# kristi700/ViT-SSL

Measured on AMD Instinct MI355X. Metric: images_per_sec, higher is better.
Workload: dtype bf16; 1 GPU; ViT-B/16 SimMIM 224x224 mask 0.6 dropout 0.1 AdamW, batch 256/GPU; global_batch=256, parallelism=dp1

## Files before the change

__graft_entry__.py:

```python
import os
import subprocess
import sys
from concurrent.futures import ThreadPoolExecutor

ROOT = os.path.dirname(os.path.abspath(__file__))
PKG = os.path.join(ROOT, "vit-ssl_amd")
CSRC = os.path.join(PKG, "csrc")
OUT_DIR = os.path.join(PKG, "vitssl_hip")
LIB = os.path.join(OUT_DIR, "libvitssl_hip.so")
SOURCES = ["error.cpp", "device_state.hip", "gemm_nt.hip", "gemm_tn.hip", "layernorm.hip", "attention.hip", "attention_hd.hip", "elementwise.hip", "patch.hip", "dino.hip", "augment.hip", "transforms.hip", "metrics.hip", "classify.hip", "mixup.hip", "fp8.hip", "optim.hip", "droppath.hip", "layerscale.hip", "lamb.hip", "mae.hip"]
HIPCC = os.environ.get("HIPCC", "/opt/rocm/bin/hipcc")
PER_FILE_FLAGS = {"augment.hip": ["-ffp-contract=off"], "transforms.hip": ["-ffp-contract=off"]}
FLAGS = ["--offload-arch=gfx950", "-O3", "-fPIC", "-std=c++17", "-Wno-unused-result"] + os.environ.get("VITSSL_HIPCC_FLAGS", "").split()


def _needs_rebuild(target, deps):
    if not os.path.exists(target):
        return True
    t = os.path.getmtime(target)
    return any(os.path.getmtime(d) > t for d in deps if os.path.exists(d))


def build(force: bool = False, verbose: bool = False) -> None:
    srcs = [os.path.join(CSRC, s) for s in SOURCES if os.path.exists(os.path.join(CSRC, s))]
    hdrs = [os.path.join(CSRC, "common.h"), os.path.join(CSRC, "attention_tiles.h"), os.path.join(CSRC, "attention_bwd.h"),
            os.path.join(CSRC, "resample_taps.h"), os.path.join(CSRC, "nt_epilogue.h"),
            os.path.join(ROOT, "include", "vitssl_hip.h"), os.path.join(ROOT, "include", "vitssl_transforms.h"),
            os.path.join(ROOT, "include", "vitssl_metrics.h"), os.path.join(ROOT, "include", "vitssl_classify.h"),
            os.path.join(ROOT, "include", "vitssl_attention_hd.h"), os.path.join(ROOT, "include", "vitssl_patch.h"),
            os.path.join(ROOT, "include", "vitssl_optim.h"), os.path.join(ROOT, "include", "vitssl_mixup.h"),
            os.path.join(ROOT, "include", "vitssl_droppath.h"), os.path.join(ROOT, "include", "vitssl_layerscale.h"),
            os.path.join(ROOT, "include", "vitssl_lamb.h"), os.path.join(ROOT, "include", "vitssl_bce.h"),
            os.path.join(ROOT, "include_ext", "vitssl_mae.h")]
    objdir = os.path.join(CSRC, "build")
    os.makedirs(objdir, exist_ok=True)

    def compile_one(src):
        obj = os.path.join(objdir, os.path.basename(src) + ".o")
        if force or _needs_rebuild(obj, [src] + hdrs + [os.path.abspath(__file__)]):
            cmd = [HIPCC] + FLAGS + PER_FILE_FLAGS.get(os.path.basename(src), []) + ["-x", "hip", "-c", src, "-o", obj]
            r = subprocess.run(cmd, capture_output=True, text=True)
            if r.returncode != 0:
                raise RuntimeError(f"hipcc failed for {src}:\n{r.stderr[-4000:]}")
            if verbose and r.stderr.strip():
                print(r.stderr, file=sys.stderr)
        return obj

    with ThreadPoolExecutor(max_workers=4) as ex:
        objs = list(ex.map(compile_one, srcs))
    if force or _needs_rebuild(LIB, objs):
        cmd = [HIPCC, "--offload-arch=gfx950", "-shared", "-fPIC", "-o", LIB] + objs
        r = subprocess.run(cmd, capture_output=True, text=True)
        if r.returncode != 0:
            raise RuntimeError(f"link failed:\n{r.stderr[-4000:]}")
    if PKG not in sys.path:
        sys.path.insert(0, PKG)
    import vitssl_hip
    vitssl_hip.lib()


def smoke() -> None:
    for p in (ROOT, PKG):
        if p not in sys.path:
            sys.path.insert(0, p)
    import torch
    from vitssl_hip import smoke_check
    smoke_check.run(torch.device("cuda:0"))
    print("smoke OK")


if __name__ == "__main__":
    build(force="--force" in sys.argv, verbose=True)
    print("built", LIB)
```

vit-ssl_amd/csrc/gemm_nt.hip:

```cpp
#include "nt_epilogue.h"

namespace {

template <int BK_, int WM_, int WN_, int MI_ = 8>
struct NtCfg {
  static constexpr int BK = BK_, WM = WM_, WN = WN_;
  static constexpr int MI = MI_;
  static constexpr int WROWS = 16 * MI_;
  static constexpr int BM = WROWS * WM_, BN = 64 * WN_;
  static constexpr int WAVES = WM_ * WN_, THREADS = 64 * WM_ * WN_;
  static constexpr int ROWB = BK_ * 2;
  static constexpr int A_BYTES = BM * ROWB, B_BYTES = BN * ROWB;
  static constexpr int BUF_BYTES = A_BYTES + B_BYTES;
  static constexpr int LDS_BYTES = 2 * BUF_BYTES;
  static constexpr int MIN_WAVES_PER_SIMD = 2;
  static constexpr int WG_PER_CU = (WAVES == 8) ? 1 : 2;
};
using NtBig = NtCfg<64, 2, 4>;
using NtSmall = NtCfg<32, 2, 2>;
using NtBig224 = NtCfg<64, 2, 4, 7>;
using NtBig192 = NtCfg<64, 2, 4, 6>;

template <int BK_>
__device__ __forceinline__ int nt_swz(int r) {
  return BK_ == 64 ? ((r >> 1) & 7) : 3 * ((r >> 3) & 1);
}

template <int BK_, int ROWS, int WAVES>
__device__ __forceinline__ void stage_tile(__amdgpu_buffer_rsrc_t rsrc, char* lds_tile, long long row0, int k0,
                                           int K, int wave, int lane) {
  constexpr int ROWB = BK_ * 2;
  constexpr int RPI = 1024 / ROWB;
  constexpr int LPR = ROWB / 16;
  constexpr int SLOTS = ROWS / RPI;
  constexpr int PER = (SLOTS + WAVES - 1) / WAVES;
#pragma unroll
  for (int j = 0; j < PER; ++j) {
    const int i = wave * PER + j;
    if (SLOTS % WAVES != 0 && i >= SLOTS) break;
    const int r = i * RPI + lane / LPR;
    const int c = lane % LPR;
    const int sc = c ^ nt_swz<BK_>(r);
    const unsigned voff = (unsigned)(((row0 + r) * (long long)K + k0) * 2 + sc * 16);
    dma16_to_lds(rsrc, lds_tile + i * 1024, voff);
  }
}

template <int N>
__device__ __forceinline__ void wait_vmcnt_round_down() {
  if constexpr (N >= 16) asm volatile("s_waitcnt vmcnt(16)" ::: "memory");
  else if constexpr (N >= 8) asm volatile("s_waitcnt vmcnt(8)" ::: "memory");
  else asm volatile("s_waitcnt vmcnt(0)" ::: "memory");
}

template <int BM, int BN>
__device__ __forceinline__ bool nt_tile_of(const NtParams& p, const int ntiles, const int G, const int bid, int r, long long& m0, int& n0) {
  const int base = r * G;
  const int cnt = min(G, ntiles - base);
  if (bid >= cnt) return false;
  const int wgid = base + xcd_remap(bid, cnt);
  const int full = p.tiles_m * p.group_n;
  const int cg = wgid / full;
  const int rem = wgid - cg * full;
  const int gw = min(p.group_n, p.tiles_n - cg * p.group_n);
  const int tile_m = rem / gw;
  m0 = (long long)tile_m * BM;
  n0 = (cg * p.group_n + (rem - tile_m * gw)) * BN;
  return true;
}

template <int EPI, typename CFG>
__global__ __launch_bounds__(CFG::THREADS, CFG::MIN_WAVES_PER_SIMD) void gemm_nt_kernel(NtParams p) {
  extern __shared__ __attribute__((aligned(16))) char smem[];
  constexpr int BM = CFG::BM, BN = CFG::BN, BK = CFG::BK;

  const int lane = threadIdx.x & 63;
  const int wave = __builtin_amdgcn_readfirstlane(threadIdx.x >> 6);
  const int wm = wave / CFG::WN, wn = wave % CFG::WN;

  const int ntiles = p.tiles_m * p.tiles_n;
  const int G = gridDim.x;
  const int bid = blockIdx.x;
  auto tile_of = [&](int r, long long& m0, int& n0) { return nt_tile_of<BM, BN>(p, ntiles, G, bid, r, m0, n0); };

  const unsigned long long a_bytes = (unsigned long long)p.M * p.K * 2ull;
  const unsigned long long b_bytes = (unsigned long long)p.N * p.K * 2ull;
  __amdgpu_buffer_rsrc_t rsA = __builtin_amdgcn_make_buffer_rsrc((void*)p.A, 0, (int)a_bytes, 0x00020000);
  __amdgpu_buffer_rsrc_t rsB = __builtin_amdgcn_make_buffer_rsrc((void*)p.B, 0, (int)b_bytes, 0x00020000);

  const int kb = p.k_chunk ? (int)blockIdx.y * p.k_chunk : 0;
  const int nk = (p.k_chunk ? min(p.K - kb, p.k_chunk) : p.K) / BK;
  const int swz = nt_swz<BK>(lane & 15);
  const int frag_row = lane & 15;
  const int kq = lane >> 4;

  constexpr int MI = CFG::MI;
  f32x4 acc[4][MI];

  auto compute_half = [&](const char* bufA, const char* bufB, auto kk_c) {
    constexpr int kk = decltype(kk_c)::value;
    const int coff = ((kk * 4 + kq) ^ swz) << 4;
    bf16x8 fb[4], fa[MI];
#pragma unroll
    for (int j = 0; j < 4; ++j)
      fb[j] = *(const bf16x8*)(bufB + (wn * 64 + j * 16 + frag_row) * CFG::ROWB + coff);
#pragma unroll
    for (int i = 0; i < MI; ++i)
      fa[i] = *(const bf16x8*)(bufA + (wm * CFG::WROWS + i * 16 + frag_row) * CFG::ROWB + coff);
    if constexpr (BK == 64) __builtin_amdgcn_s_setprio(1);
#pragma unroll
    for (int j = 0; j < 4; ++j)
#pragma unroll
      for (int i = 0; i < MI; ++i)
        acc[j][i] = __builtin_amdgcn_mfma_f32_16x16x32_bf16(fb[j], fa[i], acc[j][i], 0, 0, 0);
    if constexpr (BK == 64) __builtin_amdgcn_s_setprio(0);
  };

  long long m0 = 0, m0n = 0;
  int n0 = 0, n0n = 0;
  if (!tile_of(0, m0, n0)) return;
  int par = 0;
  stage_tile<BK, BM, CFG::WAVES>(rsA, smem, m0, kb, p.K, wave, lane);
  stage_tile<BK, BN, CFG::WAVES>(rsB, smem + CFG::A_BYTES, n0, kb, p.K, wave, lane);
  asm volatile("s_waitcnt vmcnt(0)" ::: "memory");

  for (int round = 0;; ++round) {
    const bool has_next = tile_of(round + 1, m0n, n0n);
    __syncthreads();
#pragma unroll
    for (int j = 0; j < 4; ++j)
#pragma unroll
      for (int i = 0; i < MI; ++i) acc[j][i] = f32x4{0.f, 0.f, 0.f, 0.f};

    for (int t = 0; t < nk; ++t) {
      char* bufA = smem + par * CFG::BUF_BYTES;
      char* nA = smem + (par ^ 1) * CFG::BUF_BYTES;
      const bool more = t + 1 < nk;
      const bool fetch = more || has_next;
      const long long sm = more ? m0 : m0n;
      const int sn = more ? n0 : n0n;
      const int sk = kb + (more ? (t + 1) * BK : 0);
      if constexpr (BK == 64) {
        if (fetch) stage_tile<BK, BM, CFG::WAVES>(rsA, nA, sm, sk, p.K, wave, lane);
        compute_half(bufA, bufA + CFG::A_BYTES, IC<0>{});
        if (fetch) stage_tile<BK, BN, CFG::WAVES>(rsB, nA + CFG::A_BYTES, sn, sk, p.K, wave, lane);
        compute_half(bufA, bufA + CFG::A_BYTES, IC<1>{});
      } else {
        if (fetch) {
          stage_tile<BK, BM, CFG::WAVES>(rsA, nA, sm, sk, p.K, wave, lane);
          stage_tile<BK, BN, CFG::WAVES>(rsB, nA + CFG::A_BYTES, sn, sk, p.K, wave, lane);
        }
        compute_half(bufA, bufA + CFG::A_BYTES, IC<0>{});
      }
      par ^= 1;
      if (more) {
        asm volatile("s_waitcnt vmcnt(0)" ::: "memory");
        __syncthreads();
      }
    }

    nt_epilogue<EPI, CFG>(p, acc, m0, n0, wm, wn, lane);

    if (!has_next) break;
    constexpr int TAIL = nt_epi_tail_stores<EPI>();
    static_assert(TAIL <= nt_epi_row_ops<EPI, false>(true) * MI, "more than this epilogue is certain to store");
    wait_vmcnt_round_down<TAIL>();
    m0 = m0n;
    n0 = n0n;
  }
}

__device__ __forceinline__ i32x8 join_frags(const bf16x8& lo, const bf16x8& hi) {
  const u32x4 a = __builtin_bit_cast(u32x4, lo), b = __builtin_bit_cast(u32x4, hi);
  return i32x8{(int)a[0], (int)a[1], (int)a[2], (int)a[3], (int)b[0], (int)b[1], (int)b[2], (int)b[3]};
}

template <int EPI, typename CFG, bool F8 = false>
__global__ __launch_bounds__(CFG::THREADS, 2) void gemm_nt_pp_kernel(NtParams p) {
  extern __shared__ __attribute__((aligned(16))) char smem[];
  static_assert(CFG::BK == 64 && CFG::WM == 2 && CFG::WN == 4, "ping-pong loop is written for 8 waves, BK = 64");
  constexpr int BM = CFG::BM, BN = CFG::BN, MI = CFG::MI;
  constexpr int MH1 = MI - 4;
  constexpr int BUF = CFG::BUF_BYTES;
  constexpr int DUMMY = 2 * BUF;
  constexpr unsigned OOBV = 0x80000000u;
  constexpr bool USE_GLUT = EPI == VITSSL_EPI_GELU;
  constexpr int GLUT_BASE = 2 * BUF + 1024;
  constexpr int GLUT_IMM = USE_GLUT ? GLUT_BASE - (int)GLUT_LO8 : -1;
  static_assert(!USE_GLUT || (GLUT_IMM >= 0 && GLUT_IMM < 65536), "the table's offset must fit the ds_read immediate");

  const int lane = threadIdx.x & 63;
  const int wave = __builtin_amdgcn_readfirstlane(threadIdx.x >> 6);
  const int wm = wave >> 2, wn = wave & 3;
  const int ntiles = p.tiles_m * p.tiles_n;
  const int G = gridDim.x;
  const int bid = blockIdx.x;

  auto tile_of = [&](int r, long long& m0, int& n0) { return nt_tile_of<BM, BN>(p, ntiles, G, bid, r, m0, n0); };

  long long m0 = 0;
  int n0 = 0;
  if (!tile_of(0, m0, n0)) return;

  if (p.stagger > 0) {
    const int rem = ntiles % G;
    if (rem != 0 && bid >= rem && wave == 0) {
      const unsigned long long delay = (unsigned long long)p.stagger * (unsigned)(bid - rem) / (unsigned)(G - rem);
      const unsigned long long t0 = __builtin_amdgcn_s_memrealtime();
      while (__builtin_amdgcn_s_memrealtime() - t0 < delay) __builtin_amdgcn_s_sleep(8);
    }
  }

  constexpr unsigned ESZ = F8 ? 1u : 2u;
  const unsigned long long a_bytes = (unsigned long long)p.M * p.K * ESZ;
  const unsigned long long b_bytes = (unsigned long long)p.N * p.K * ESZ;
  const int nk = F8 ? p.K / 128 : p.K / 64;
  const unsigned rowb = (unsigned)p.K * ESZ;

  unsigned voffA[2][2], voffB[2][2];
  int ldsA[2][2], ldsB[2][2];
#pragma unroll
  for (int h = 0; h < 2; ++h)
#pragma unroll
    for (int e = 0; e < 2; ++e) {
      const int s = 2 * wave + e;
      {
        const int per_g = h == 0 ? 8 : 2 * MH1;
        const bool ok = s < 2 * per_g;
        const int g = s / per_g, q = s - g * per_g;
        const int r = g * CFG::WROWS + 64 * h + 8 * q;
        const int rl = r + (lane >> 3);
        const int sc = (lane & 7) ^ ((rl >> 1) & 7);
        voffA[h][e] = ok ? (unsigned)rl * rowb + (unsigned)sc * 16u : OOBV;
        ldsA[h][e] = ok ? r * 128 : DUMMY;
      }
      {
        const int c = s >> 2, q = s & 3;
        const int r = 64 * c + 32 * h + 8 * q;
        const int rl = r + (lane >> 3);
        const int sc = (lane & 7) ^ ((rl >> 1) & 7);
        voffB[h][e] = (unsigned)rl * rowb + (unsigned)sc * 16u;
        ldsB[h][e] = CFG::A_BYTES + r * 128;
      }
    }

  struct Cur {
    int round, kt;
    unsigned a, b;
  };
  auto cur_at = [&](int round) {
    Cur c;
    c.round = round;
    c.kt = 0;
    long long mm;
    int nn;
    if (tile_of(round, mm, nn)) {
      c.a = (unsigned)((unsigned long long)mm * rowb);
      c.b = (unsigned)((unsigned long long)nn * rowb);
    } else {
      c.a = c.b = OOBV;
    }
    return c;
  };
  auto cur_next = [&](const Cur& c) {
    if (c.a == OOBV) return c;
    if (c.kt + 1 < nk) {
      Cur n = c;
      n.kt += 1;
      n.a += 128u;
      n.b += 128u;
      return n;
    }
    return cur_at(c.round + 1);
  };
  auto stage_a = [&](const Cur& c, int bufsel, auto h_c) {
    constexpr int h = decltype(h_c)::value;
    __amdgpu_buffer_rsrc_t rs =
        __builtin_amdgcn_make_buffer_rsrc((void*)((const char*)p.A + c.a), 0, c.a == OOBV ? 0 : (int)(a_bytes - c.a), 0x00020000);
#pragma unroll
    for (int e = 0; e < 2; ++e) {
      const bool live = ldsA[h][e] != DUMMY;
      dma16_to_lds(rs, smem + (live ? bufsel * BUF : 0) + ldsA[h][e], voffA[h][e]);
    }
  };
  auto stage_b = [&](const Cur& c, int bufsel, auto h_c) {
    constexpr int h = decltype(h_c)::value;
    __amdgpu_buffer_rsrc_t rs =
        __builtin_amdgcn_make_buffer_rsrc((void*)((const char*)p.B + c.b), 0, c.b == OOBV ? 0 : (int)(b_bytes - c.b), 0x00020000);
#pragma unroll
    for (int e = 0; e < 2; ++e)
      dma16_to_lds(rs, smem + bufsel * BUF + ldsB[h][e], voffB[h][e]);
  };

  const int frag_row = lane & 15;
  const int kq = lane >> 4;
  const int swz = nt_swz<64>(frag_row);
  const int offA0 = (wm * CFG::WROWS + frag_row) * 128 + (((0 + kq) ^ swz) << 4);
  const int offA1 = (wm * CFG::WROWS + frag_row) * 128 + (((4 + kq) ^ swz) << 4);
  const int offB0 = CFG::A_BYTES + (wn * 64 + frag_row) * 128 + (((0 + kq) ^ swz) << 4);
  const int offB1 = CFG::A_BYTES + (wn * 64 + frag_row) * 128 + (((4 + kq) ^ swz) << 4);

  f32x4 acc[4][MI];
  bf16x8 fa[2][4];
  bf16x8 fb[2][2][2];

  auto read_a = [&](const char* buf, auto mh_c) {
    constexpr int mh = decltype(mh_c)::value;
    constexpr int cnt = mh == 0 ? 4 : MH1;
#pragma unroll
    for (int ii = 0; ii < cnt; ++ii) {
      fa[0][ii] = *(const bf16x8*)(buf + offA0 + (4 * mh + ii) * 2048);
      fa[1][ii] = *(const bf16x8*)(buf + offA1 + (4 * mh + ii) * 2048);
    }
  };
  auto read_b = [&](const char* buf, auto nh_c) {
    constexpr int nh = decltype(nh_c)::value;
#pragma unroll
    for (int jj = 0; jj < 2; ++jj) {
      fb[nh][0][jj] = *(const bf16x8*)(buf + offB0 + (2 * nh + jj) * 2048);
      fb[nh][1][jj] = *(const bf16x8*)(buf + offB1 + (2 * nh + jj) * 2048);
    }
  };
  auto mma_quad = [&](auto mh_c, auto nh_c) {
    constexpr int mh = decltype(mh_c)::value, nh = decltype(nh_c)::value;
    constexpr int cnt = mh == 0 ? 4 : MH1;
    if constexpr (F8) {
#pragma unroll
      for (int jj = 0; jj < 2; ++jj) {
        const i32x8 bq = join_frags(fb[nh][0][jj], fb[nh][1][jj]);
#pragma unroll
        for (int ii = 0; ii < cnt; ++ii)
          acc[2 * nh + jj][4 * mh + ii] = __builtin_amdgcn_mfma_scale_f32_16x16x128_f8f6f4(
              bq, join_frags(fa[0][ii], fa[1][ii]), acc[2 * nh + jj][4 * mh + ii], 0, 0, 0, 0, 0, 0);
      }
    } else {
#pragma unroll
      for (int kk = 0; kk < 2; ++kk)
#pragma unroll
        for (int jj = 0; jj < 2; ++jj)
#pragma unroll
          for (int ii = 0; ii < cnt; ++ii)
            acc[2 * nh + jj][4 * mh + ii] =
                __builtin_amdgcn_mfma_f32_16x16x32_bf16(fb[nh][kk][jj], fa[kk][ii], acc[2 * nh + jj][4 * mh + ii], 0, 0, 0);
    }
  };
  auto ktile = [&](int buf, const Cur& c1, const Cur& c2, bool last_of_round, auto nw_c) {
    constexpr int NW = decltype(nw_c)::value;
    const char* cur = smem + buf * BUF;
    read_b(cur, IC<0>{});
    read_a(cur, IC<0>{});
    stage_b(c1, buf ^ 1, IC<1>{});
    wait_vmcnt<NW>();
    raw_barrier();
    mma_quad(IC<0>{}, IC<0>{});
    raw_barrier();
    read_b(cur, IC<1>{});
    stage_a(c1, buf ^ 1, IC<1>{});
    wait_vmcnt<NW>();
    raw_barrier();
    mma_quad(IC<0>{}, IC<1>{});
    raw_barrier();
    read_a(cur, IC<1>{});
    stage_b(c2, buf, IC<0>{});
    raw_barrier();
    mma_quad(IC<1>{}, IC<1>{});
    raw_barrier();
    stage_a(c2, buf, IC<0>{});
    wait_vmcnt<NW>();
    raw_barrier();
    mma_quad(IC<1>{}, IC<0>{});
    if (!(last_of_round && wm == 1)) raw_barrier();
  };

  Cur c0 = cur_at(0);
  Cur c1 = cur_next(c0);
  stage_b(c0, 0, IC<0>{});
  stage_a(c0, 0, IC<0>{});
  stage_b(c0, 0, IC<1>{});
  stage_a(c0, 0, IC<1>{});
  stage_b(c1, 1, IC<0>{});
  stage_a(c1, 1, IC<0>{});
  Cur c2 = cur_next(c1);
  if constexpr (USE_GLUT) {
    if ((unsigned)(unsigned long long)LDS_PTR(smem) != 0u) __builtin_trap();
    const float hs = p.drop_on ? 0.5f * p.dk.scale : 0.5f;
    const float cs = p.drop_on ? 0.3989422804014327f * p.dk.scale : 0.3989422804014327f;
    unsigned* tab = (unsigned*)(smem + GLUT_BASE);
    for (int e = threadIdx.x; e < GLUT_ENTRIES; e += CFG::THREADS) {
      const unsigned h = (unsigned)((e >> 1) + (GLUT_E_LO << 7)) | ((unsigned)(e & 1) << 15);
      float y, dy;
      gelu_both_scaled(bf2f((bf16_t)h), hs, cs, y, dy);
      if constexpr (F8) {
        const float qs = p.qscale ? *p.qscale : 1.0f;
        tab[e] = (unsigned)f2bf(dy) | ((pack_fp8x4(y * qs, 0.f, 0.f, 0.f) & 0xffu) << 16);
      } else {
        tab[e] = (unsigned)f2bf(y) | ((unsigned)f2bf(dy) << 16);
      }
    }
    asm volatile("s_waitcnt lgkmcnt(0)" ::: "memory");
  }
  wait_vmcnt<8>();
  raw_barrier();

  constexpr int S = nt_epi_vmem_ops<EPI, MI, F8>();
  constexpr int NW = 8;
  constexpr int NW_POST = (NW + S) > 63 ? 63 : (NW + S);
  int buf = 0;
#ifdef VITSSL_NT_STAMPS
  auto stamp = [&](int round, int which) {
    if (!(p.stamps && (wave & 3) == 0 && lane == 0 && round < 16)) return;
    p.stamps[(((size_t)bid * 2 + wm) * 16 + round) * 4 + which] = __builtin_amdgcn_s_memrealtime();
    p.stamps[(size_t)256 * 2 * 16 * 4 + (((size_t)bid * 2 + wm) * 16 + round) * 4 + which] = __builtin_amdgcn_s_memtime();
  };
#else
  auto stamp = [&](int, int) {};
#endif
  for (int round = 0;; ++round) {
    stamp(round, 0);
    if (wm == 1) raw_barrier();
#pragma unroll
    for (int j = 0; j < 4; ++j)
#pragma unroll
      for (int i = 0; i < MI; ++i) acc[j][i] = f32x4{0.f, 0.f, 0.f, 0.f};
    for (int t = 0; t < nk; ++t) {
      const bool last = t + 1 == nk;
      if (t == 0 && round > 0) ktile(buf, c1, c2, last, IC<NW_POST>{});
      else ktile(buf, c1, c2, last, IC<NW>{});
      c1 = c2;
      c2 = cur_next(c2);
      buf ^= 1;
    }
    stamp(round, 1);
    if constexpr (F8) {
      if (p.alpha || p.alpha2) {
        const float al = (p.alpha ? *p.alpha : 1.0f) * (p.alpha2 ? *p.alpha2 : 1.0f);
#pragma unroll
        for (int j = 0; j < 4; ++j)
#pragma unroll
          for (int i = 0; i < MI; ++i) acc[j][i] *= al;
      }
    }
    nt_epilogue<EPI, CFG, F8, GLUT_IMM, true>(p, acc, m0, n0, wm, wn, lane, smem, smem + (buf ^ 1) * BUF + ldsB[1][0]);
    stamp(round, 2);
#ifdef VITSSL_NT_STAMPS
    if (p.stamps) {
      asm volatile("s_waitcnt vmcnt(0)" ::: "memory");
      stamp(round, 3);
    }
#endif
    if (!tile_of(round + 1, m0, n0)) break;
  }
  asm volatile("s_waitcnt vmcnt(0)" ::: "memory");
}

int cu_count() { return vitssl_persistent_cus(); }

template <int EPI, typename CFG, bool F8 = false>
int launch_pp(NtParams p, hipStream_t s) {
  constexpr int LDS = 2 * CFG::BUF_BYTES + 1024 + (EPI == VITSSL_EPI_GELU ? GLUT_BYTES : 0);
  static VsOnce attr_done{false};
  if (int rc = ensure_lds(gemm_nt_pp_kernel<EPI, CFG, F8>, LDS, attr_done, "gemm_nt")) return rc;
  const long long ntiles = (long long)p.tiles_m * p.tiles_n;
  const long long slots = cu_count();
  const long long grid = ntiles < slots ? ntiles : slots;
  constexpr float STAGGER_SCALE = 1.0f;
  static VsEnvMilli stagger_knob;
  const float stagger_scale = stagger_knob.get("VITSSL_NT_STAGGER", STAGGER_SCALE);
  constexpr int STAGGER_EPIS = (1 << VITSSL_EPI_RESID) | (1 << VITSSL_EPI_DGELU);
  static VsEnvInt stagger_mask_knob;
  const int stagger_mask = stagger_mask_knob.get("VITSSL_NT_STAGGER_EPIS", STAGGER_EPIS);
  const float tile_us = (float)(p.K * p.esz / 128) * 1.45f * (float)CFG::MI / 8.f + nt_epi(EPI).epi_us;
  p.stagger = ((stagger_mask >> nt_epi(EPI).stagger_bit) & 1) ? (int)(stagger_scale * tile_us * 100.f) : 0;
  vitssl_note_nt_grid((int)grid);
  hipLaunchKernelGGL((gemm_nt_pp_kernel<EPI, CFG, F8>), dim3((unsigned)grid), dim3(CFG::THREADS), LDS, s, p);
  VS_CHECK_LAUNCH("gemm_nt_pp");
  return VITSSL_OK;
}

template <int EPI, typename CFG>
int launch_cfg_parts(NtParams p, hipStream_t s) {
  if constexpr (CFG::LDS_BYTES > 48 * 1024) {
    static VsOnce attr_done{false};
    if (int rc = ensure_lds(gemm_nt_kernel<EPI, CFG>, CFG::LDS_BYTES, attr_done, "gemm_nt")) return rc;
  }
  p.tiles_m = (int)ceil_div64(p.M, CFG::BM);
  p.tiles_n = (int)ceil_div64(p.N, CFG::BN);
  const int want = (int)((2 * 1024 * 1024) / ((long long)CFG::BN * p.K * p.esz));
  static VsEnvInt group_env;
  const int group_knob = group_env.get("VITSSL_NT_GROUPN", 0);
  if (group_knob > 0) p.group_n = group_knob < p.tiles_n ? group_knob : p.tiles_n;
  else if (p.tiles_n <= 4) p.group_n = p.tiles_n;
  else if (want <= 2) p.group_n = 2;
  else if (p.tiles_n % 6 == 0 && want >= 6) p.group_n = 6;
  else if (p.tiles_n % 4 == 0) p.group_n = 4;
  else if (p.tiles_n % 3 == 0) p.group_n = 3;
  else p.group_n = want < 4 ? want : 4;
  if (p.esz == 1) {
    if ((p.N & 7) != 0) {
      vitssl_set_error("gemm_fp8_nt: N=%d must be a multiple of 8", p.N);
      return VITSSL_ERR_ARG;
    }
    if constexpr (CFG::WAVES == 8 && CFG::BK == 64 && nt_epi(EPI).fp8) {
      return launch_pp<EPI, CFG, true>(p, s);
    } else {
      vitssl_set_error("gemm_fp8_nt: epilogue %d / tile configuration not built for fp8 operands", EPI);
      return VITSSL_ERR_ARG;
    }
  }
  if constexpr (CFG::WAVES == 8 && CFG::BK == 64 && EPI != EPI_F32_SPLITK) {
    if (p.k_chunk == 0 && (p.N & 7) == 0) return launch_pp<EPI, CFG>(p, s);
  }
  static VsEnvInt persist_env;
  const int knob = persist_env.get("VITSSL_NT_PERSIST", -1);
  const bool persist = knob >= 0 ? knob != 0 : p.K <= 512;
  const long long ntiles = (long long)p.tiles_m * p.tiles_n;
  long long grid = ntiles;
  if (persist) {
    const long long slots = (long long)cu_count() * CFG::WG_PER_CU;
    if (grid > slots) grid = slots;
  }
  const unsigned slices = p.k_chunk ? (unsigned)ceil_div64(p.K, p.k_chunk) : 1u;
  hipLaunchKernelGGL((gemm_nt_kernel<EPI, CFG>), dim3((unsigned)grid, slices), dim3(CFG::THREADS), CFG::LDS_BYTES, s, p);
  VS_CHECK_LAUNCH("gemm_nt");
  return VITSSL_OK;
}

int nt_tile_override() {
  static VsEnvInt knob;
  return knob.get("VITSSL_NT_TILE", 0);
}

int launch_splitk_f32(NtParams p, hipStream_t s, bool* done) {
  *done = false;
  const long long tiles = ceil_div64(p.M, NtSmall::BM) * ceil_div64(p.N, NtSmall::BN);
  if (tiles >= 64 || p.K < 4096) return VITSSL_OK;
  long long slices = (cu_count() / 2 + tiles - 1) / tiles;
  const long long max_slices = p.K / 512;
  if (slices > max_slices) slices = max_slices;
  if (slices < 2) return VITSSL_OK;
  long long chunk = ceil_div64(ceil_div64(p.K, slices), 64) * 64;
  p.k_chunk = (int)chunk;
  hipError_t e = hipMemsetAsync(p.out0, 0, (size_t)p.M * p.N * sizeof(float), s);
  if (e != hipSuccess) {
    vitssl_set_error("gemm_nt: split-K memset failed: %s", hipGetErrorString(e));
    return VITSSL_ERR_LAUNCH;
  }
  *done = true;
  return launch_cfg_parts<EPI_F32_SPLITK, NtSmall>(p, s);
}


template <int EPI, typename CFG>
int launch_cfg(NtParams p, hipStream_t s) {
  float* colsum = p.colsum;
  if (!colsum) return launch_cfg_parts<EPI, CFG>(p, s);
  const int groups = (int)ceil_div64(p.M, CFG::BM) * (CFG::BM / CFG::WROWS);
  p.colsum = vs_sum_parts(p.workspace, p.workspace_floats, (long long)groups * p.N, p.M, p.N, "gemm_nt column sums");
  if (!p.colsum) return VITSSL_ERR_ARG;
  const int rc = launch_cfg_parts<EPI, CFG>(p, s);
  if (rc != VITSSL_OK) return rc;
  return vs_reduce_parts(colsum, p.colsum, groups, p.N, p.N, s);
}

template <int EPI>
int launch_nt(const NtParams& p, hipStream_t s) {
  if constexpr (EPI == VITSSL_EPI_F32) {
    if (!p.colsum && p.esz == 2) {
      bool done = false;
      const int rc = launch_splitk_f32(p, s, &done);
      if (rc != VITSSL_OK || done) return rc;
    }
  }
  const int mode = p.esz == 1 ? 0 : nt_tile_override();
  if (mode == 1) return launch_cfg<EPI, NtBig>(p, s);
  if (mode == 2) return launch_cfg<EPI, NtSmall>(p, s);
  if (mode == 3) return launch_cfg<EPI, NtBig192>(p, s);
  if (mode == 4) return launch_cfg<EPI, NtBig224>(p, s);
  const long long big_tiles = ceil_div64(p.M, 256) * ceil_div64(p.N, 256);
  if (big_tiles < 64 && p.esz == 2) return launch_cfg<EPI, NtSmall>(p, s);
  const long long slots = cu_count();
  const long long tn = ceil_div64(p.N, 256);
  const double c256 = (double)ceil_div64(ceil_div64(p.M, 256) * tn, slots);
  const double c224 = 0.90 * (double)ceil_div64(ceil_div64(p.M, 224) * tn, slots);
  const double c192 = 0.78 * (double)ceil_div64(ceil_div64(p.M, 192) * tn, slots);
  double best = c256;
  if (c192 < 0.9 * c256 && c192 <= c224) best = c192;
  else if (c224 < 0.95 * c256) best = c224;
  if (best == c192 && best != c256) return launch_cfg<EPI, NtBig192>(p, s);
  if (best == c224 && best != c256) return launch_cfg<EPI, NtBig224>(p, s);
  return launch_cfg<EPI, NtBig>(p, s);
}

}

#ifdef VITSSL_NT_STAMPS
static unsigned long long* g_nt_stamps = nullptr;
extern "C" void vitssl_debug_nt_stamps(void* buf) { g_nt_stamps = (unsigned long long*)buf; }
#endif

static NtEpiFacts caller_epi(int epi) { return nt_epi(epi >= EPI_F32_SPLITK ? -1 : epi); }

static int check_rowscale(const char* who, const vitssl_rowscale_t* rows, int64_t M) {
  VS_CHECK_ARG(rows->scale && rows->groups > 0 && rows->rows_per_group > 0, "%s: row scales need scale, groups > 0 and rows_per_group > 0", who);
  VS_CHECK_ARG(rows->groups * (int64_t)rows->rows_per_group == M, "%s: groups (%lld) * rows_per_group (%d) must equal M (%lld)", who,
               (long long)rows->groups, rows->rows_per_group, (long long)M);
  return VITSSL_OK;
}

static int gemm_nt_entry(const vitssl_gemm_t* g, int esz, const vitssl_fp8_gemm_t* q, void* stream, const vitssl_rowscale_t* rows = nullptr,
                         const vitssl_colscale_t* cols = nullptr, void* branch = nullptr) {
  const char* who = cols ? "gemm_nt_ls" : rows ? "gemm_nt_rows" : esz == 1 ? "gemm_fp8_nt" : "gemm_nt";
  VS_CHECK_ARG(g && g->A && g->B && (g->out0 || (esz == 1 && caller_epi(g->epilogue).q8_of == 0 && q && q->out_fp8)), "%s: null operand", who);
  VS_CHECK_ARG(g->M > 0 && g->N > 0 && g->K > 0, "%s: empty problem M=%lld N=%d K=%d", who, (long long)g->M, g->N, g->K);
  VS_CHECK_ARG(g->K % (128 / esz) == 0, "%s: K=%d must be a multiple of %d", who, g->K, 128 / esz);
  VS_CHECK_ARG(g->N % 4 == 0, "%s: N=%d must be a multiple of 4", who, g->N);
  VS_CHECK_ARG(g->N <= (1 << 20), "%s: N=%d exceeds 2^20 (epilogue windows use 32-bit byte offsets)", who, g->N);
  VS_CHECK_ARG((unsigned long long)g->M * g->K * (unsigned)esz < (1ull << 31) && (unsigned long long)g->N * g->K * (unsigned)esz < (1ull << 31),
               "%s: operand larger than 2 GiB (M=%lld N=%d K=%d)", who, (long long)g->M, g->N, g->K);
  NtParams p{(const bf16_t*)g->A, (const bf16_t*)g->B, g->M, g->N, g->K, g->bias, g->aux, g->out0, g->out1, g->colsum, g->workspace,
             g->workspace_floats, make_drop_key(g->drop)};
  p.drop_on = p.dk.thr != 0;
  p.embed = g->embed;
  p.esz = esz;
  if (q) {
    p.alpha = q->alpha;
    p.alpha2 = q->alpha2;
    p.out2 = q->out_fp8;
    p.qscale = q->out_scale;
    p.qamax = q->out_amax;
  }
  p.rows_per_group = 1;
#ifdef VITSSL_NT_STAMPS
  p.stamps = g_nt_stamps;
#endif
  hipStream_t s = (hipStream_t)stream;
  VS_CHECK_ARG(!g->colsum || caller_epi(g->epilogue).colsum, "%s: column sums are built for the BF16 / F32 / DGELU epilogues only", who);
  VS_CHECK_ARG(!p.drop_on || (unsigned long long)g->M * (unsigned long long)g->N < (1ull << 34),
               "%s: dropout over %lld x %d elements: the stream's group counter is 32 bits (M * N < 2^34)", who, (long long)g->M, g->N);
  if (rows || cols) {
    VS_CHECK_ARG(g->epilogue == VITSSL_EPI_RESID, "%s: %s scales are built for VITSSL_EPI_RESID only, got epilogue %d", who,
                 cols ? "column" : "row", g->epilogue);
    VS_CHECK_ARG(g->aux, "%s: EPI_RESID needs aux (residual)", who);
    if (cols) {
      VS_CHECK_ARG(cols->gamma, "%s: null gamma", who);
      VS_CHECK_ARG(cols->cols == g->N, "%s: cols (%d) must equal N (%d)", who, cols->cols, g->N);
    }
    if (rows) {
      if (int rc = check_rowscale(who, rows, g->M)) return rc;
      p.rowscale = rows->scale;
      p.rows_per_group = (unsigned)rows->rows_per_group;
    }
    if (!cols) return launch_nt<EPI_RESID_ROWS>(p, s);
    p.colscale = cols->gamma;
    p.out1 = branch;
    return launch_nt<EPI_RESID_LS>(p, s);
  }
  switch (g->epilogue) {
    case VITSSL_EPI_BF16: return launch_nt<VITSSL_EPI_BF16>(p, s);
    case VITSSL_EPI_F32: return launch_nt<VITSSL_EPI_F32>(p, s);
    case VITSSL_EPI_GELU:
      VS_CHECK_ARG(g->out1 || p.out2, "%s: EPI_GELU needs out1 (or, with fp8 operands, out_fp8)", who);
      return launch_nt<VITSSL_EPI_GELU>(p, s);
    case VITSSL_EPI_RESID:
      VS_CHECK_ARG(g->aux, "%s: EPI_RESID needs aux (residual)", who);
      return launch_nt<VITSSL_EPI_RESID>(p, s);
    case VITSSL_EPI_DGELU:
      VS_CHECK_ARG(g->aux, "%s: EPI_DGELU needs aux (pre-activation)", who);
      return launch_nt<VITSSL_EPI_DGELU>(p, s);
    case VITSSL_EPI_EMBED:
      VS_CHECK_ARG(g->embed.pos && g->embed.tokens > 0 && g->embed.out_tokens >= g->embed.tokens + g->embed.tok_offset,
                   "%s: EPI_EMBED needs pos/tokens", who);
      VS_CHECK_ARG(!g->embed.mask || g->embed.mask_token, "%s: EPI_EMBED mask without mask_token", who);
      return launch_nt<VITSSL_EPI_EMBED>(p, s);
    default:
      vitssl_set_error("%s: unknown epilogue %d", who, g->epilogue);
      return VITSSL_ERR_ARG;
  }
}

extern "C" int vitssl_gemm_bf16_nt(const vitssl_gemm_t* g, void* stream) { return gemm_nt_entry(g, 2, nullptr, stream); }

extern "C" int vitssl_gemm_bf16_nt_rows(const vitssl_gemm_t* g, const vitssl_rowscale_t* rows, void* stream) {
  VS_CHECK_ARG(rows, "gemm_nt_rows: null row scales (vitssl_gemm_bf16_nt is the launch without them)");
  return gemm_nt_entry(g, 2, nullptr, stream, rows);
}

extern "C" int vitssl_gemm_bf16_nt_ls(const vitssl_gemm_t* g, const vitssl_colscale_t* cols, const vitssl_rowscale_t* rows,
                                      void* branch_bf16, void* stream) {
  VS_CHECK_ARG(cols, "gemm_nt_ls: null column scales (vitssl_gemm_bf16_nt / vitssl_gemm_bf16_nt_rows are the launches without them)");
  return gemm_nt_entry(g, 2, nullptr, stream, rows, cols, branch_bf16);
}

extern "C" int vitssl_gemm_fp8_nt(const vitssl_gemm_t* g, const vitssl_fp8_gemm_t* q, void* stream) {
  VS_CHECK_ARG(g && caller_epi(g->epilogue).fp8, "gemm_fp8_nt: fp8 operands are built for the BF16 / F32 / GELU / RESID / DGELU epilogues");
  VS_CHECK_ARG(!(q && q->out_fp8) || caller_epi(g->epilogue).q8_of >= 0, "gemm_fp8_nt: out_fp8 belongs to EPI_GELU / EPI_DGELU");
  return gemm_nt_entry(g, 1, q, stream);
}
```

vit-ssl_amd/csrc/nt_epilogue.h:

```cpp
#pragma once
#include "../../include/vitssl_droppath.h"
#include "../../include/vitssl_layerscale.h"
#include "common.h"

namespace {

struct NtParams {
  const bf16_t* A;
  const bf16_t* B;
  long long M;
  int N, K;
  const float* bias;
  const void* aux;
  void* out0;
  void* out1;
  float* colsum;
  float* workspace;
  int64_t workspace_floats;
  DropKey dk;
  int drop_on;
  vitssl_embed_t embed;
  int tiles_m, tiles_n;
  int group_n;
  int k_chunk;
  int stagger;
  int esz;
  const float* alpha;
  void* out2;
  const float* alpha2;
  const float* qscale;
  float* qamax;
  const float* rowscale;
  unsigned rows_per_group;
  const float* colscale;
#ifdef VITSSL_NT_STAMPS
  unsigned long long* stamps;
#endif
};

constexpr int EPI_F32_SPLITK = 100;
constexpr int EPI_RESID_ROWS = 101;
constexpr int EPI_RESID_LS = 102;

enum NtOut1 { OUT1_NONE, OUT1_REQUIRED, OUT1_OPTIONAL };
struct NtEpiFacts {
  int out0_esz;
  bool windowed;
  NtOut1 out1;
  int aux_esz;
  bool colsum, fp8;
  int q8_of;
  bool drops, resid;
  int stagger_bit;
  float epi_us;
};
constexpr NtEpiFacts nt_epi(int epi) {
  switch (epi) {
    case VITSSL_EPI_BF16:  return NtEpiFacts{2, true,  OUT1_NONE,     0, true,  true,  -1, false, false, VITSSL_EPI_BF16,  2.f};
    case VITSSL_EPI_F32:   return NtEpiFacts{4, true,  OUT1_NONE,     0, true,  true,  -1, false, false, VITSSL_EPI_F32,   4.f};
    case VITSSL_EPI_GELU:  return NtEpiFacts{2, true,  OUT1_REQUIRED, 0, false, true,   1, true,  false, VITSSL_EPI_GELU,  7.f};
    case VITSSL_EPI_RESID: return NtEpiFacts{4, true,  OUT1_NONE,     4, false, true,  -1, true,  true,  VITSSL_EPI_RESID, 8.f};
    case VITSSL_EPI_DGELU: return NtEpiFacts{2, true,  OUT1_NONE,     2, true,  true,   0, false, false, VITSSL_EPI_DGELU, 5.f};
    case VITSSL_EPI_EMBED: return NtEpiFacts{4, false, OUT1_NONE,     0, false, false, -1, false, false, VITSSL_EPI_EMBED, 4.f};
    case EPI_F32_SPLITK:   return NtEpiFacts{4, false, OUT1_NONE,     0, false, false, -1, false, false, -1,               4.f};
    case EPI_RESID_ROWS:   return NtEpiFacts{4, true,  OUT1_NONE,     4, false, false, -1, true,  true,  VITSSL_EPI_RESID, 8.f};
    case EPI_RESID_LS:     return NtEpiFacts{4, true,  OUT1_OPTIONAL, 4, false, false, -1, true,  true,  VITSSL_EPI_RESID, 8.f};
    default:               return NtEpiFacts{0, false, OUT1_NONE,     0, false, false, -1, false, false, -1,               0.f};
  }
}

template <int EPI, int MI, bool PREF>
constexpr int nt_row_group() {
  return nt_epi(EPI).resid ? (PREF ? 1 : (MI % 2 == 0 ? 2 : 1)) : EPI == VITSSL_EPI_DGELU ? (PREF ? 2 : (MI % 4 == 0 ? 4 : 2)) : 4;
}

template <int EPI, bool F8>
constexpr int nt_epi_row_ops(bool stores_only) {
  constexpr NtEpiFacts E = nt_epi(EPI);
  if (!E.windowed) return 0;
  const int out0 = (F8 && E.q8_of == 0) ? 1 : E.out0_esz;
  const int out1 = E.out1 != OUT1_REQUIRED ? 0 : (F8 && E.q8_of == 1) ? 1 : 2;
  return (stores_only ? 0 : E.aux_esz) + out0 + out1;
}
template <int EPI, int MI, bool F8>
constexpr int nt_epi_vmem_ops() { return nt_epi_row_ops<EPI, F8>(false) * MI; }
template <int EPI>
constexpr int nt_epi_tail_stores() { return nt_epi_row_ops<EPI, false>(true) * nt_row_group<EPI, 8, false>(); }
template <int EPI, int MI>
constexpr bool nt_counts_are(int bf, int f8, int tail) {
  return nt_epi_vmem_ops<EPI, MI, false>() == bf * MI && (!nt_epi(EPI).fp8 || nt_epi_vmem_ops<EPI, MI, true>() == f8 * MI) &&
         nt_epi_tail_stores<EPI>() == tail;
}
template <int MI>
constexpr bool nt_counts_are_as_written() {
  return nt_counts_are<VITSSL_EPI_BF16, MI>(2, 2, 8) && nt_counts_are<VITSSL_EPI_GELU, MI>(4, 3, 16) && nt_counts_are<VITSSL_EPI_DGELU, MI>(4, 3, 8) &&
         nt_counts_are<VITSSL_EPI_F32, MI>(4, 4, 16) && nt_counts_are<VITSSL_EPI_RESID, MI>(8, 8, 8) && nt_counts_are<EPI_RESID_ROWS, MI>(8, 8, 8) &&
         nt_counts_are<EPI_RESID_LS, MI>(8, 8, 8) && nt_counts_are<VITSSL_EPI_EMBED, MI>(0, 0, 0) && nt_counts_are<EPI_F32_SPLITK, MI>(0, 0, 0);
}
static_assert(nt_counts_are_as_written<6>() && nt_counts_are_as_written<7>() && nt_counts_are_as_written<8>(), "epilogue vmem counts");


constexpr int GLUT_E_LO = 127 - 14;
constexpr int GLUT_BINADES = 18;
constexpr int GLUT_ENTRIES = GLUT_BINADES * 128 * 2;
constexpr int GLUT_BYTES = GLUT_ENTRIES * 4;
constexpr unsigned GLUT_LO8 = (unsigned)GLUT_E_LO << 10;
constexpr unsigned GLUT_HI8 = (unsigned)(GLUT_E_LO + GLUT_BINADES) << 10;

__device__ __forceinline__ unsigned glut_rot2(unsigned w) {
  unsigned t, r;
  asm("v_pk_lshrrev_b16 %0, 15, %1 op_sel_hi:[0,1]" : "=v"(t) : "v"(w));
  asm("v_pk_mad_u16 %0, %1, 2, %2 op_sel_hi:[1,0,1]" : "=v"(r) : "v"(w), "v"(t));
  return r;
}
__device__ __forceinline__ void glut_addr2(unsigned r, unsigned& a0, unsigned& a1) {
  asm("v_lshlrev_b32_sdwa %0, 2, %1 dst_sel:DWORD dst_unused:UNUSED_PAD src0_sel:DWORD src1_sel:WORD_0" : "=v"(a0) : "v"(r));
  asm("v_lshlrev_b32_sdwa %0, 2, %1 dst_sel:DWORD dst_unused:UNUSED_PAD src0_sel:DWORD src1_sel:WORD_1" : "=v"(a1) : "v"(r));
}
__device__ __forceinline__ bool glut_out_of_range(unsigned r01, unsigned r23) {
  const unsigned lo2 = ((unsigned)GLUT_E_LO << 8) * 0x10001u, span = ((unsigned)(GLUT_BINADES << 8) - 1u) * 0x10001u;
  unsigned d01, d23, dm, e;
  asm("v_pk_sub_u16 %0, %1, %2" : "=v"(d01) : "v"(r01), "s"(lo2));
  asm("v_pk_sub_u16 %0, %1, %2" : "=v"(d23) : "v"(r23), "s"(lo2));
  asm("v_pk_max_u16 %0, %1, %2" : "=v"(dm) : "v"(d01), "v"(d23));
  asm("v_pk_sub_u16 %0, %1, %2 clamp" : "=v"(e) : "v"(dm), "s"(span));
  return e != 0;
}
template <int OFF>
__device__ __forceinline__ unsigned glut_read(const char* smem, unsigned a) {
  (void)smem;
  return *(const __attribute__((address_space(3))) unsigned*)(unsigned long long)(a + (unsigned)OFF);
}

struct NtWindow {
  char* xs;
  unsigned tw16, tr16a, tw32, tr32a;
  __device__ __forceinline__ void lines_of_bf16(const u32x2 (&w)[2][2], u32x4& s1, u32x4& s2) const {
#pragma unroll
    for (int j = 0; j < 4; ++j) *(u32x2*)(xs + (tw16 ^ (unsigned)(32 * j))) = w[j >> 1][j & 1];
    s1 = *(const u32x4*)(xs + tr16a);
    s2 = *(const u32x4*)(xs + ((tr16a + 1024u) ^ 64u));
  }
  __device__ __forceinline__ void put_lines_bf16(const u32x4& s1, const u32x4& s2) const {
    *(u32x4*)(xs + tr16a) = s1;
    *(u32x4*)(xs + ((tr16a + 1024u) ^ 64u)) = s2;
  }
  __device__ __forceinline__ u32x2 bf16_of_lines(int j) const { return *(const u32x2*)(xs + (tw16 ^ (unsigned)(32 * j))); }
  __device__ __forceinline__ void lines_of_f32(const f32x4& v0, const f32x4& v1, u32x4& s1, u32x4& s2) const {
    *(f32x4*)(xs + tw32) = v0;
    *(f32x4*)(xs + (tw32 ^ 64u)) = v1;
    s1 = *(const u32x4*)(xs + tr32a);
    s2 = *(const u32x4*)(xs + tr32a + 1024);
  }
  __device__ __forceinline__ void f32_of_lines(f32x4& v0, f32x4& v1) const {
    *(f32x4*)(xs + tr32a) = v0;
    *(f32x4*)(xs + tr32a + 1024) = v1;
    v0 = *(const f32x4*)(xs + tw32);
    v1 = *(const f32x4*)(xs + (tw32 ^ 64u));
  }
};

__device__ __forceinline__ float amax4(float a, float b, float c, float d) { return fmaxf(fmaxf(fabsf(a), fabsf(b)), fmaxf(fabsf(c), fabsf(d))); }

template <int EPI, typename CFG, bool Q8 = false, int GLUT_OFF = -1, bool TLS = false>
__device__ __forceinline__ void nt_epilogue(const NtParams& p, f32x4 (&acc)[4][CFG::MI], const long long m0, const int n0,
                                            const int wm, const int wn, const int lane_in, const char* lds = nullptr, char* xs = nullptr) {
  constexpr int MI = CFG::MI;
  constexpr NtEpiFacts E = nt_epi(EPI);
  constexpr bool LS = EPI == EPI_RESID_LS;
  int lane = lane_in;
  if (TLS) asm volatile("" : "+v"(lane));
  constexpr bool GLUT = EPI == VITSSL_EPI_GELU && GLUT_OFF >= 0;
  const bool glut_on = GLUT && (!Q8 || (p.out1 == nullptr && p.qamax == nullptr));
  constexpr bool CS = E.colsum, DROPS = E.drops;
  float csum[4][4];
  if (CS && p.colsum) {
#pragma unroll
    for (int j = 0; j < 4; ++j)
#pragma unroll
      for (int r = 0; r < 4; ++r) csum[j][r] = 0.f;
  }
  const int g4 = lane >> 4;
  const bool wide = TLS || (p.N & 7) == 0;
  constexpr unsigned OOB = 0x80000000u;
  const long long rows_left = p.M - m0;
  auto window = [&](const void* base, int elt) {
    const unsigned long long bytes = (unsigned long long)rows_left * (unsigned long long)p.N * (unsigned)elt;
    const unsigned rec = bytes > 0x80000000ull ? 0x80000000u : (unsigned)bytes;
    return __builtin_amdgcn_make_buffer_rsrc((void*)((const char*)base + m0 * p.N * elt), 0, (int)rec, 0x00020000);
  };
  const unsigned row_l = (unsigned)(wm * CFG::WROWS + (lane & 15));
  const unsigned un = (unsigned)p.N;
  const int odd = g4 & 1;

  auto off_bf16_wide = [&](int i, int jp) -> unsigned {
    const int n = n0 + wn * 64 + (2 * jp + odd) * 16 + 4 * (g4 - odd);
    return n < p.N ? ((row_l + 16u * i) * un + (unsigned)n) * 2u : OOB;
  };
  auto off_elem = [&](int i, int n, unsigned elt) -> unsigned { return n < p.N ? ((row_l + 16u * i) * un + (unsigned)n) * elt : OOB; };
  constexpr bool tls = TLS;
  const int tm = lane & 15, trho = lane >> 3, tkap = lane & 7;
  const unsigned tw16 = (unsigned)(tm * 128 + ((g4 ^ (2 * (tm >> 1))) << 3));
  const unsigned tr16a = (unsigned)(trho * 128 + ((tkap ^ (trho >> 1)) << 4));
  const unsigned tw32 = (unsigned)(tm * 128 + ((g4 ^ (tm & 7)) << 4));
  const unsigned tr32a = (unsigned)(trho * 128 + ((tkap ^ trho) << 4));
  const NtWindow win{xs, tw16, tr16a, tw32, tr32a};
  const unsigned trow = (unsigned)(wm * CFG::WROWS + trho);
  const int tn16 = n0 + wn * 64 + 8 * tkap;
  const unsigned tb16 = tn16 < p.N ? (trow * un + (unsigned)tn16) * 2u : OOB;
  auto off_line16 = [&](int i, int half) -> unsigned { return tb16 + (unsigned)(16 * i + 8 * half) * (un * 2u); };
  auto off_line32 = [&](int i, int jp, int half) -> unsigned {
    const int n = n0 + wn * 64 + 32 * jp + 4 * tkap;
    const unsigned b = n < p.N ? (trow * un + (unsigned)n) * 4u : OOB;
    return b + (unsigned)(16 * i + 8 * half) * (un * 4u);
  };
  int nn[2][2];
  bool okn[2][2];
  auto pack_pair = [&](const u32x2& w0, const u32x2& w1) -> u32x4 {
    auto lo = __builtin_amdgcn_permlane16_swap(w0[0], w1[0], false, false);
    auto hi = __builtin_amdgcn_permlane16_swap(w0[1], w1[1], false, false);
    return u32x4{lo[0], hi[0], lo[1], hi[1]};
  };
  auto store_bf16_row = [&](__amdgpu_buffer_rsrc_t rs, int i, const u32x2 (&w)[2][2], auto aux_c) {
    constexpr int AUXV = decltype(aux_c)::value;
    if (tls) {
      u32x4 s1, s2;
      win.lines_of_bf16(w, s1, s2);
      __builtin_amdgcn_raw_buffer_store_b128(s1, rs, off_line16(i, 0), 0, AUXV);
      __builtin_amdgcn_raw_buffer_store_b128(s2, rs, off_line16(i, 1), 0, AUXV);
    } else if (wide) {
      const u32x4 a = pack_pair(w[0][0], w[0][1]), b = pack_pair(w[1][0], w[1][1]);
      __builtin_amdgcn_raw_buffer_store_b128(a, rs, off_bf16_wide(i, 0), 0, AUXV);
      __builtin_amdgcn_raw_buffer_store_b128(b, rs, off_bf16_wide(i, 1), 0, AUXV);
    } else {
#pragma unroll
      for (int jp = 0; jp < 2; ++jp) {
        const int na = n0 + wn * 64 + (2 * jp) * 16 + 4 * g4;
        __builtin_amdgcn_raw_buffer_store_b64(w[jp][0], rs, off_elem(i, na, 2u), 0, AUXV);
        __builtin_amdgcn_raw_buffer_store_b64(w[jp][1], rs, off_elem(i, na + 16, 2u), 0, AUXV);
      }
    }
  };
  constexpr int F32_AUX = E.resid ? 2 : 0;
  auto store_f32_pair = [&](__amdgpu_buffer_rsrc_t rs, int i, int jp, const f32x4& v0, const f32x4& v1, const int (&nnp)[2]) {
    if (tls) {
      u32x4 s1, s2;
      win.lines_of_f32(v0, v1, s1, s2);
      __builtin_amdgcn_raw_buffer_store_b128(s1, rs, off_line32(i, jp, 0), 0, F32_AUX);
      __builtin_amdgcn_raw_buffer_store_b128(s2, rs, off_line32(i, jp, 1), 0, F32_AUX);
    } else {
      __builtin_amdgcn_raw_buffer_store_b128(__builtin_bit_cast(u32x4, v0), rs, off_elem(i, nnp[0], 4u), 0, F32_AUX);
      __builtin_amdgcn_raw_buffer_store_b128(__builtin_bit_cast(u32x4, v1), rs, off_elem(i, nnp[1], 4u), 0, F32_AUX);
    }
  };
  auto store_fp8_row = [&](__amdgpu_buffer_rsrc_t rs, int i, const unsigned (&out_q)[2][2]) {
    if ((p.N & 15) == 0) {
      auto s02 = __builtin_amdgcn_permlane32_swap(out_q[0][0], out_q[1][0], false, false);
      auto s13 = __builtin_amdgcn_permlane32_swap(out_q[0][1], out_q[1][1], false, false);
      auto e = __builtin_amdgcn_permlane16_swap(s02[0], s13[0], false, false);
      auto f = __builtin_amdgcn_permlane16_swap(s02[1], s13[1], false, false);
      if (tls) {
        *(u32x4*)(xs + tm * 64 + ((g4 ^ ((tm >> 1) & 3)) << 4)) = u32x4{e[0], e[1], f[0], f[1]};
        const int rho4 = lane >> 2, kap4 = lane & 3;
        const u32x4 s8 = *(const u32x4*)(xs + rho4 * 64 + ((kap4 ^ ((rho4 >> 1) & 3)) << 4));
        const int n8 = n0 + wn * 64 + 16 * kap4;
        const unsigned o8 = n8 < p.N ? ((unsigned)(wm * CFG::WROWS + 16 * i + rho4) * un + (unsigned)n8) : OOB;
        __builtin_amdgcn_raw_buffer_store_b128(s8, rs, o8, 0, 0);
      } else {
        const int n = n0 + wn * 64 + 16 * g4;
        __builtin_amdgcn_raw_buffer_store_b128(u32x4{e[0], e[1], f[0], f[1]}, rs, off_elem(i, n, 1u), 0, 0);
      }
    } else {
#pragma unroll
      for (int jp = 0; jp < 2; ++jp)
#pragma unroll
        for (int h = 0; h < 2; ++h) __builtin_amdgcn_raw_buffer_store_b32(out_q[jp][h], rs, off_elem(i, nn[jp][h], 1u), 0, 0);
    }
  };

  __amdgpu_buffer_rsrc_t rsOut0, rsOut1, rsOut2, rsAux;
  constexpr bool Q8EPI = Q8 && E.q8_of >= 0;
  const bool q8 = Q8EPI && p.out2 != nullptr;
  if (q8) rsOut2 = window(p.out2, 1);
  const float qs = (Q8EPI && p.qscale) ? *p.qscale : 1.0f;
  float qmax = 0.f;
  if constexpr (E.windowed) rsOut0 = window(p.out0, E.out0_esz);
  if constexpr (E.out1 != OUT1_NONE) {
    if (E.out1 == OUT1_REQUIRED || p.out1) rsOut1 = window(p.out1, 2);
  }
  if constexpr (E.aux_esz != 0) rsAux = window(p.aux, E.aux_esz);

  f32x4 bias4[2][2];
  f32x4 gam4[2][2];
  unsigned a0col[2][2];
  const unsigned a0rowstep = 16u * (unsigned)(p.N >> 2) * DROP_C0;
  unsigned a0row = 0;
  if (DROPS && p.drop_on)
    a0row = drop_a0(p.dk, (unsigned)(m0 + wm * CFG::WROWS + (lane & 15)) * (unsigned)(p.N >> 2));
  const float gelu_hs = (DROPS && p.drop_on) ? 0.5f * p.dk.scale : 0.5f;
  const float gelu_cs = (DROPS && p.drop_on) ? 0.3989422804014327f * p.dk.scale : 0.3989422804014327f;
#pragma unroll
  for (int jp = 0; jp < 2; ++jp)
#pragma unroll
    for (int h = 0; h < 2; ++h) {
      nn[jp][h] = n0 + wn * 64 + (2 * jp + h) * 16 + 4 * g4;
      a0col[jp][h] = (unsigned)(nn[jp][h] >> 2) * DROP_C0;
      okn[jp][h] = nn[jp][h] < p.N;
      bias4[jp][h] = f32x4{0.f, 0.f, 0.f, 0.f};
      if (p.bias && (EPI != EPI_F32_SPLITK || blockIdx.y == 0) && okn[jp][h]) bias4[jp][h] = *(const f32x4*)(p.bias + nn[jp][h]);
      if constexpr (LS) {
        gam4[jp][h] = f32x4{0.f, 0.f, 0.f, 0.f};
        if (okn[jp][h]) gam4[jp][h] = *(const f32x4*)(p.colscale + nn[jp][h]);
      }
    }

  constexpr bool PREF = TLS && E.aux_esz != 0;
  constexpr int RG = nt_row_group<EPI, MI, PREF>();
  constexpr int NB = PREF ? 2 : 1;
  f32x4 res[NB][RG][2][2];
  u32x4 raw[NB][RG][2];
  float rsc[NB][RG];
  auto load_group = [&](const int ig, const int b) {
    const int cnt = MI - ig < RG ? MI - ig : RG;
    if constexpr (EPI == EPI_RESID_ROWS || LS) {
#pragma unroll
      for (int ii = 0; ii < RG; ++ii) {
        if (ii >= cnt) continue;
        if constexpr (LS) rsc[b][ii] = 1.0f;
        if (EPI == EPI_RESID_ROWS || p.rowscale) {
          const long long mr = m0 + wm * CFG::WROWS + (ig + ii) * 16 + (lane & 15);
          rsc[b][ii] = p.rowscale[mr < p.M ? (unsigned)mr / p.rows_per_group : 0u];
        }
      }
    }
    if constexpr (E.resid) {
#pragma unroll
      for (int ii = 0; ii < RG; ++ii)
#pragma unroll
        for (int jp = 0; jp < 2; ++jp) {
          if (ii >= cnt) continue;
          if (tls) {
            res[b][ii][jp][0] = __builtin_bit_cast(f32x4, __builtin_amdgcn_raw_buffer_load_b128(rsAux, off_line32(ig + ii, jp, 0), 0, 0));
            res[b][ii][jp][1] = __builtin_bit_cast(f32x4, __builtin_amdgcn_raw_buffer_load_b128(rsAux, off_line32(ig + ii, jp, 1), 0, 0));
          } else {
#pragma unroll
            for (int h = 0; h < 2; ++h)
              res[b][ii][jp][h] = __builtin_bit_cast(f32x4, __builtin_amdgcn_raw_buffer_load_b128(rsAux, off_elem(ig + ii, nn[jp][h], 4u), 0, 0));
          }
        }
    }
    if constexpr (EPI == VITSSL_EPI_DGELU) {
      if (wide) {
#pragma unroll
        for (int ii = 0; ii < RG; ++ii) {
          if (ii >= cnt) continue;
          if (tls) {
            raw[b][ii][0] = __builtin_amdgcn_raw_buffer_load_b128(rsAux, off_line16(ig + ii, 0), 0, 0);
            raw[b][ii][1] = __builtin_amdgcn_raw_buffer_load_b128(rsAux, off_line16(ig + ii, 1), 0, 0);
          } else {
#pragma unroll
            for (int jp = 0; jp < 2; ++jp) raw[b][ii][jp] = __builtin_amdgcn_raw_buffer_load_b128(rsAux, off_bf16_wide(ig + ii, jp), 0, 0);
          }
        }
      }
    }
  };
  if constexpr (PREF) load_group(0, 0);
#pragma unroll
  for (int ig = 0; ig < MI; ig += RG) {
    const int cnt = MI - ig < RG ? MI - ig : RG;
    const int gb = PREF ? (ig / RG) & 1 : 0;
    if constexpr (!PREF) load_group(ig, 0);
    else if (ig + RG < MI) load_group(ig + RG, gb ^ 1);
    u32x2 gpre[RG][2][2];
    if constexpr (EPI == VITSSL_EPI_DGELU) {
      if (wide) {
#pragma unroll
        for (int ii = 0; ii < RG; ++ii)
#pragma unroll
          for (int jp = 0; jp < 2; ++jp) {
            if (ii >= cnt) continue;
            if (tls) {
              if (jp == 0) {
                win.put_lines_bf16(raw[gb][ii][0], raw[gb][ii][1]);
#pragma unroll
                for (int j = 0; j < 4; ++j) gpre[ii][j >> 1][j & 1] = win.bf16_of_lines(j);
              }
              continue;
            }
            auto sa = __builtin_amdgcn_permlane16_swap(raw[gb][ii][jp][0], raw[gb][ii][jp][2], false, false);
            auto sb = __builtin_amdgcn_permlane16_swap(raw[gb][ii][jp][1], raw[gb][ii][jp][3], false, false);
            gpre[ii][jp][0] = u32x2{sa[0], sb[0]};
            gpre[ii][jp][1] = u32x2{sa[1], sb[1]};
          }
      } else {
#pragma unroll
        for (int ii = 0; ii < RG; ++ii)
#pragma unroll
          for (int jp = 0; jp < 2; ++jp)
#pragma unroll
            for (int h = 0; h < 2; ++h)
              if (ii < cnt) gpre[ii][jp][h] = __builtin_amdgcn_raw_buffer_load_b64(rsAux, off_elem(ig + ii, nn[jp][h], 2u), 0, 0);
      }
    }

#pragma unroll
    for (int ii = 0; ii < RG; ++ii) {
      if (ii >= cnt) continue;
      const int i = ig + ii;
      const long long m = m0 + wm * CFG::WROWS + i * 16 + (lane & 15);
      const bool okm = m < p.M;
      u32x2 out_a[2][2], out_b[2][2];
      unsigned out_q[2][2];
      unsigned gl[16];
      bool gslow[2][2];
      if (GLUT && glut_on) {
#pragma unroll
        for (int jp = 0; jp < 2; ++jp)
#pragma unroll
          for (int h = 0; h < 2; ++h) {
            const f32x4 vv = acc[2 * jp + h][i] + bias4[jp][h];
            const unsigned w0 = pack_bf2(vv[0], vv[1]), w1 = pack_bf2(vv[2], vv[3]);
            const unsigned r01 = glut_rot2(w0), r23 = glut_rot2(w1);
            gslow[jp][h] = __builtin_amdgcn_ballot_w64(glut_out_of_range(r01, r23)) != 0;
            unsigned ad[4];
            glut_addr2(r01, ad[0], ad[1]);
            glut_addr2(r23, ad[2], ad[3]);
            const int q = 8 * jp + 4 * h;
#pragma unroll
            for (int r = 0; r < 4; ++r) gl[q + r] = glut_read<GLUT_OFF>(lds, ad[r]);
          }
      }
#pragma unroll
      for (int jp = 0; jp < 2; ++jp) {
        f32x4 v[2] = {acc[2 * jp][i] + bias4[jp][0], acc[2 * jp + 1][i] + bias4[jp][1]};

        if constexpr (EPI == VITSSL_EPI_BF16) {
          out_a[jp][0] = u32x2{pack_bf2(v[0][0], v[0][1]), pack_bf2(v[0][2], v[0][3])};
          out_a[jp][1] = u32x2{pack_bf2(v[1][0], v[1][1]), pack_bf2(v[1][2], v[1][3])};
        } else if constexpr (EPI == VITSSL_EPI_GELU) {
          unsigned km[2][2] = {{0xffffffffu, 0xffffffffu}, {0xffffffffu, 0xffffffffu}};
          u32x2 dw[2] = {u32x2{0u, 0u}, u32x2{0u, 0u}};
          const bool dropping = p.drop_on;
          if (dropping) {
#pragma unroll
            for (int h = 0; h < 2; ++h) {
              dw[h] = drop_words_a0(p.dk, a0row + (unsigned)i * a0rowstep + a0col[jp][h]);
              km[h][0] = drop_keep_pair(p.dk, dw[h][0]);
              km[h][1] = drop_keep_pair(p.dk, dw[h][1]);
            }
          }
#pragma unroll
          for (int h = 0; h < 2; ++h) {
            if (GLUT && glut_on && !gslow[jp][h]) {
              const int q = 8 * jp + 4 * h;
              const u32x2 lo = u32x2{__builtin_amdgcn_perm(gl[q + 1], gl[q], 0x05040100u) & km[h][0],
                                     __builtin_amdgcn_perm(gl[q + 3], gl[q + 2], 0x05040100u) & km[h][1]};
              if constexpr (!Q8) {
                out_b[jp][h] = lo;
                out_a[jp][h] = u32x2{__builtin_amdgcn_perm(gl[q + 1], gl[q], 0x07060302u) & km[h][0],
                                     __builtin_amdgcn_perm(gl[q + 3], gl[q + 2], 0x07060302u) & km[h][1]};
              } else {
                out_a[jp][h] = lo;
                const unsigned b01 = __builtin_amdgcn_perm(gl[q + 1], gl[q], 0x0c0c0602u), b23 = __builtin_amdgcn_perm(gl[q + 3], gl[q + 2], 0x06020c0cu);
                out_q[jp][h] = (b01 | b23) & __builtin_amdgcn_perm(km[h][1], km[h][0], 0x06040200u);
              }
              continue;
            }
            float y[4], d[4];
#pragma unroll
            for (int r = 0; r < 4; ++r) gelu_both_scaled(round_bf(v[h][r]), gelu_hs, gelu_cs, y[r], d[r]);
            out_b[jp][h] = u32x2{pack_bf2(y[0], y[1]) & km[h][0], pack_bf2(y[2], y[3]) & km[h][1]};
            out_a[jp][h] = u32x2{pack_bf2(d[0], d[1]) & km[h][0], pack_bf2(d[2], d[3]) & km[h][1]};
            if constexpr (Q8) {
              if (dropping) {
                bool keep[4];
                drop_keep4(p.dk, dw[h], keep);
#pragma unroll
                for (int r = 0; r < 4; ++r) y[r] = keep[r] ? y[r] : 0.f;
              }
              out_q[jp][h] = pack_fp8x4(y[0] * qs, y[1] * qs, y[2] * qs, y[3] * qs);
              if (okm && okn[jp][h]) qmax = fmaxf(qmax, amax4(y[0], y[1], y[2], y[3]));
            }
          }
        } else if constexpr (EPI == VITSSL_EPI_DGELU) {
#pragma unroll
          for (int h = 0; h < 2; ++h) {
            const u32x2 gpv = gpre[ii][jp][h];
            v[h][0] *= bf_lo(gpv[0]);
            v[h][1] *= bf_hi(gpv[0]);
            v[h][2] *= bf_lo(gpv[1]);
            v[h][3] *= bf_hi(gpv[1]);
            out_a[jp][h] = u32x2{pack_bf2(v[h][0], v[h][1]), pack_bf2(v[h][2], v[h][3])};
            if constexpr (Q8) {
              out_q[jp][h] = pack_fp8x4(v[h][0] * qs, v[h][1] * qs, v[h][2] * qs, v[h][3] * qs);
              if (okm && okn[jp][h]) qmax = fmaxf(qmax, amax4(v[h][0], v[h][1], v[h][2], v[h][3]));
            }
          }
        } else if constexpr (EPI == EPI_F32_SPLITK) {
#pragma unroll
          for (int h = 0; h < 2; ++h) {
            if (!(okm && okn[jp][h])) continue;
            float* o = (float*)p.out0 + m * p.N + nn[jp][h];
#pragma unroll
            for (int r = 0; r < 4; ++r) unsafeAtomicAdd(o + r, v[h][r]);
          }
        } else if constexpr (EPI == VITSSL_EPI_F32) {
          store_f32_pair(rsOut0, i, jp, v[0], v[1], nn[jp]);
        } else if constexpr (E.resid) {
          if (tls) win.f32_of_lines(res[gb][ii][jp][0], res[gb][ii][jp][1]);
          if constexpr (EPI == EPI_RESID_ROWS || LS) {
            const float rs = rsc[gb][ii];
            const float cs = p.drop_on ? rs * p.dk.scale : rs;
#pragma unroll
            for (int h = 0; h < 2; ++h) {
              bool keep[4] = {true, true, true, true};
              if (p.drop_on) drop_keep4(p.dk, drop_words_a0(p.dk, a0row + (unsigned)i * a0rowstep + a0col[jp][h]), keep);
              float u[4];
#pragma unroll
              for (int r = 0; r < 4; ++r) {
                const float kv = keep[r] ? v[h][r] : 0.f;
                float sc = cs;
                if constexpr (LS) {
                  u[r] = p.drop_on ? kv * p.dk.scale : kv;
                  sc = cs * gam4[jp][h][r];
                }
                const float t = fmaf(kv, sc, res[gb][ii][jp][h][r]);
                v[h][r] = rs == 0.f ? res[gb][ii][jp][h][r] : t;
              }
              if constexpr (LS) out_a[jp][h] = u32x2{pack_bf2(u[0], u[1]), pack_bf2(u[2], u[3])};
            }
          } else {
#pragma unroll
            for (int h = 0; h < 2; ++h) {
              if (p.drop_on) {
                bool keep[4];
                drop_keep4(p.dk, drop_words_a0(p.dk, a0row + (unsigned)i * a0rowstep + a0col[jp][h]), keep);
#pragma unroll
                for (int r = 0; r < 4; ++r) v[h][r] = fmaf(keep[r] ? v[h][r] : 0.f, p.dk.scale, res[gb][ii][jp][h][r]);
              } else {
                v[h] += res[gb][ii][jp][h];
              }
            }
          }
          store_f32_pair(rsOut0, i, jp, v[0], v[1], nn[jp]);
        } else {
#pragma unroll
          for (int h = 0; h < 2; ++h) {
            if (!(okm && okn[jp][h])) continue;
            const long long img = m / p.embed.tokens;
            const int rin = (int)(m - img * p.embed.tokens);
            if (p.embed.mask && p.embed.mask[m]) v[h] = *(const f32x4*)(p.embed.mask_token + nn[jp][h]);
            v[h] += *(const f32x4*)(p.embed.pos + (long long)(p.embed.tok_offset + rin) * p.N + nn[jp][h]);
            const long long orow = img * p.embed.out_tokens + p.embed.tok_offset + rin;
            *(f32x4*)((float*)p.out0 + orow * p.N + nn[jp][h]) = v[h];
          }
        }
        if (CS && p.colsum) {
#pragma unroll
          for (int h = 0; h < 2; ++h)
            if (okm && okn[jp][h]) {
#pragma unroll
              for (int r = 0; r < 4; ++r) csum[2 * jp + h][r] += v[h][r];
            }
        }
      }
      if constexpr (E.windowed && E.out0_esz == 2) {
        if (!(Q8 && E.q8_of == 0) || p.out0) store_bf16_row(rsOut0, i, out_a, IC<EPI == VITSSL_EPI_GELU ? 2 : 0>{});
      }
      if constexpr (E.out1 == OUT1_REQUIRED) {
        if (!(Q8 && E.q8_of == 1) || p.out1) store_bf16_row(rsOut1, i, out_b, IC<0>{});
      }
      if constexpr (E.out1 == OUT1_OPTIONAL) {
        if (p.out1) store_bf16_row(rsOut1, i, out_a, IC<2>{});
      }
      if constexpr (Q8EPI) {
        if (q8) store_fp8_row(rsOut2, i, out_q);
      }
    }
  }

  if (CS && p.colsum) {
    f32x4 red[4];
#pragma unroll
    for (int j = 0; j < 4; ++j) {
#pragma unroll
      for (int r = 0; r < 4; ++r) {
        float s = csum[j][r];
        s += __shfl_xor(s, 1, 64);
        s += __shfl_xor(s, 2, 64);
        s += __shfl_xor(s, 4, 64);
        s += __shfl_xor(s, 8, 64);
        red[j][r] = s;
      }
    }
    if (tls) {
      if ((lane & 15) == 0) {
#pragma unroll
        for (int j = 0; j < 4; ++j) *(f32x4*)(xs + (16 * j + 4 * g4) * 4) = red[j];
      }
      asm volatile("" ::: "memory");
      const float v = *(const volatile float*)(xs + lane * 4);
      const int n = n0 + wn * 64 + lane;
      if (n < p.N) p.colsum[(m0 / CFG::WROWS + wm) * p.N + n] = v;
    } else {
#pragma unroll
      for (int j = 0; j < 4; ++j)
#pragma unroll
        for (int r = 0; r < 4; ++r) {
          const int n = n0 + wn * 64 + j * 16 + 4 * (lane >> 4) + r;
          if ((lane & 15) == 0 && n < p.N) p.colsum[(m0 / CFG::WROWS + wm) * p.N + n] = red[j][r];
        }
    }
  }
  if constexpr (Q8EPI) {
    if (p.qamax) {
      qmax = wave_max(qmax);
      unsigned* slot = (unsigned*)p.qamax;
      if (lane == 0 && __float_as_uint(qmax) > __builtin_nontemporal_load(slot)) atomicMax(slot, __float_as_uint(qmax));
    }
  }
}

}
```

vit-ssl_amd/vitssl_hip/_lib.py:

```python
import ctypes as C
import os
import re

_HERE = os.path.dirname(os.path.abspath(__file__))
LIB_PATH = os.environ.get("VITSSL_LIB") or os.path.join(_HERE, "libvitssl_hip.so")
_INCLUDE = os.path.normpath(os.path.join(_HERE, "..", "..", "include"))
HEADERS = {key: os.path.join(_INCLUDE, f"vitssl_{key}.h")
           for key in ("hip", "transforms", "metrics", "classify", "attention_hd", "patch", "optim", "mixup", "droppath", "layerscale",
                       "lamb", "bce")}
_INCLUDE_EXT = os.path.normpath(os.path.join(_HERE, "..", "..", "include_ext"))
EXT_HEADERS = {"mae": os.path.join(_INCLUDE_EXT, "vitssl_mae.h")}


class VitsslError(RuntimeError):
    pass


class Dropout(C.Structure):
    _fields_ = [("p", C.c_float), ("site", C.c_uint32), ("seed", C.c_uint64)]


class Embed(C.Structure):
    _fields_ = [("mask", C.c_void_p), ("mask_token", C.c_void_p), ("pos", C.c_void_p),
                ("tokens", C.c_int), ("out_tokens", C.c_int), ("tok_offset", C.c_int)]


class TnJob(C.Structure):
    _fields_ = [("A", C.c_void_p), ("B", C.c_void_p), ("C", C.c_void_p), ("N1", C.c_int), ("N2", C.c_int)]


class Fp8TnJob(C.Structure):
    _fields_ = [("A8", C.c_void_p), ("B8", C.c_void_p), ("C", C.c_void_p), ("N1", C.c_int), ("N2", C.c_int),
                ("alpha", C.c_void_p), ("alpha2", C.c_void_p)]


class OptimSegment(C.Structure):
    _fields_ = [("offset", C.c_int64), ("n", C.c_int64), ("lr_scale", C.c_float), ("weight_decay", C.c_float)]


class RowScale(C.Structure):
    _fields_ = [("scale", C.c_void_p), ("groups", C.c_int64), ("rows_per_group", C.c_int)]


class ColScale(C.Structure):
    _fields_ = [("gamma", C.c_void_p), ("cols", C.c_int)]


class Gemm(C.Structure):
    _fields_ = [("A", C.c_void_p), ("B", C.c_void_p), ("M", C.c_int64), ("N", C.c_int), ("K", C.c_int),
                ("epilogue", C.c_int), ("bias", C.c_void_p), ("aux", C.c_void_p), ("out0", C.c_void_p),
                ("out1", C.c_void_p), ("colsum", C.c_void_p), ("drop", Dropout), ("embed", Embed),
                ("workspace", C.c_void_p), ("workspace_floats", C.c_int64)]


class Fp8Gemm(C.Structure):
    _fields_ = [("alpha", C.c_void_p), ("alpha2", C.c_void_p), ("out_fp8", C.c_void_p), ("out_scale", C.c_void_p),
                ("out_amax", C.c_void_p)]


class CastJob(C.Structure):
    _fields_ = [("src", C.c_void_p), ("dst", C.c_void_p), ("dst_t", C.c_void_p), ("R", C.c_int), ("C", C.c_int)]


class CastLdJob(C.Structure):
    _fields_ = CastJob._fields_ + [("ld_dst", C.c_int), ("ld_dst_t", C.c_int)]


class Fp8WeightJob(C.Structure):
    _fields_ = [("src", C.c_void_p), ("dst_fp8", C.c_void_p), ("dst_t_fp8", C.c_void_p), ("R", C.c_int), ("C", C.c_int)]


STRUCTS = {"vitssl_dropout_t": Dropout, "vitssl_embed_t": Embed, "vitssl_gemm_t": Gemm, "vitssl_fp8_gemm_t": Fp8Gemm,
           "vitssl_fp8_weight_job_t": Fp8WeightJob, "vitssl_tn_job_t": TnJob, "vitssl_fp8_tn_job_t": Fp8TnJob,
           "vitssl_cast_job_t": CastJob, "vitssl_cast_ld_job_t": CastLdJob, "vitssl_optim_segment_t": OptimSegment,
           "vitssl_rowscale_t": RowScale, "vitssl_colscale_t": ColScale}

EPI_BF16, EPI_F32, EPI_GELU, EPI_RESID, EPI_DGELU, EPI_EMBED = range(6)

ABI_VERSION = 3
_vp, _i, _i64, _f, _d = C.c_void_p, C.c_int, C.c_int64, C.c_float, C.c_double
_pGemm, _pRows, _pCols = C.POINTER(Gemm), C.POINTER(RowScale), C.POINTER(ColScale)


def _returns(restype, *argtypes):
    return restype, list(argtypes)


_ABI = {
    "hip": {
        "vitssl_last_error": _returns(C.c_char_p),
        "vitssl_version": _returns(_i),
        "vitssl_set_reserved_cus": [_i],
        "vitssl_get_reserved_cus": _returns(_i),
        "vitssl_debug_last_nt_grid": _returns(_i),
        "vitssl_debug_last_attn_fwd_grid": _returns(_i),
        "vitssl_dropout_mask": [_vp, _i64, _i64, Dropout, _vp],
        "vitssl_layernorm_fwd": [_vp, _vp, _vp, _vp, _vp, _vp, _i64, _i, _f, _vp],
        "vitssl_layernorm_bwd": [_vp, _vp, _vp, _vp, _vp, _vp, _vp, _vp, _vp, _vp, _vp, Dropout, _i64, _i, _vp, _i64, _vp],
        "vitssl_grad_mask_cast": [_vp, _vp, _vp, Dropout, _i64, _i, _vp, _i64, _vp],
        "vitssl_gemm_bf16_nt": [_pGemm, _vp],
        "vitssl_gemm_fp8_nt": [_pGemm, C.POINTER(Fp8Gemm), _vp],
        "vitssl_attn_fwd_fp8": [_vp, _vp, _vp, _vp, _vp, _i, _i, _i, _i, _vp],
        "vitssl_gemm_fp8_tn_workspace_floats": _returns(_i64, _i64, _i, _i),
        "vitssl_gemm_fp8_tn": [_vp, _vp, _vp, _i64, _i, _i, _vp, _vp, _vp, _i64, _vp],
        "vitssl_attn_bwd_fp8": [_vp, _vp, _vp, _vp, _vp, _vp, _vp, _vp, _i, _i, _i, _i, _vp],
        "vitssl_quantize_fp8": [_vp, _vp, _i64, _vp],
        "vitssl_quantize_fp8_scaled": [_vp, _vp, _i64, _vp, _vp, _vp],
        "vitssl_layernorm_fwd_fp8": [_vp, _vp, _vp, _vp, _vp, _vp, _vp, _i64, _i, _f, _vp],
        "vitssl_layernorm_bwd_fp8": [_vp, _vp, _vp, _vp, _vp, _vp, _vp, _vp, _vp, _vp, _vp, _vp, _vp, _vp, Dropout, _i64, _i, _vp,
                                     _i64, _vp],
        "vitssl_grad_mask_cast_fp8": [_vp, _vp, _vp, _vp, _vp, _vp, Dropout, _i64, _i, _vp, _i64, _vp],
        "vitssl_fp8_quantize_weights": [_vp, _vp, _i, _i, _vp, _vp, _vp],
        "vitssl_gemm_tn_workspace_floats": _returns(_i64, _i64, _i, _i),
        "vitssl_gemm_bf16_tn": [_vp, _vp, _vp, _i64, _i, _i, _vp, _i64, _vp],
        "vitssl_gemm_tn_batch_workspace_floats": _returns(_i64, C.POINTER(TnJob), _i, _i64),
        "vitssl_gemm_bf16_tn_batch": [C.POINTER(TnJob), _i, _i64, _vp, _i64, _vp],
        "vitssl_gemm_fp8_tn_batch_workspace_floats": _returns(_i64, C.POINTER(Fp8TnJob), _i, _i64),
        "vitssl_gemm_fp8_tn_batch": [C.POINTER(Fp8TnJob), _i, _i64, _vp, _i64, _vp],
        "vitssl_attn_fwd": [_vp, _vp, _vp, _vp, _i, _i, _i, _i, _vp],
        "vitssl_attn_bwd": [_vp, _vp, _vp, _vp, _vp, _vp, _i, _i, _i, _i, _vp],
        "vitssl_patchify_bf16": [_vp, _vp, _i, _i, _i, _i, _i, _vp],
        "vitssl_gather_patches_f32": [_vp, _vp, _vp, _i, _i, _i, _i, _i, _vp],
        "vitssl_gather_rows_bf16": [_vp, _vp, _vp, _i, _i, _vp],
        "vitssl_scatter_rows_f32": [_vp, _vp, _vp, _i64, _i, _vp],
        "vitssl_gather_cls_f32": [_vp, _vp, _i, _i, _i, _vp],
        "vitssl_scatter_cls_f32": [_vp, _vp, _i, _i, _i, _vp],
        "vitssl_embed_bwd_workspace_floats": _returns(_i64, _i, _i, _i, _i),
        "vitssl_embed_bwd": [_vp, _vp, _vp, _vp, _vp, _vp, _vp, _i, _i, _i, _i, _vp, _i64, _vp],
        "vitssl_l1_loss": [_vp, _vp, _vp, _vp, _f, _i64, _vp, _i64, _vp],
        "vitssl_cross_entropy": [_vp, _vp, _vp, _vp, _f, _i, _i, _vp],
        "vitssl_colsum_bf16": [_vp, _vp, _i64, _i, _vp, _i64, _vp],
        "vitssl_sum_workspace_floats": _returns(_i64, _i64, _i),
        "vitssl_cast_bf16": [_vp, _vp, _i64, _vp],
        "vitssl_cast_transpose_bf16": [_vp, _vp, _vp, _i, _i, _vp],
        "vitssl_cast_transpose_batch": [_vp, _vp, _i, _i, _vp],
        "vitssl_adamw": [_vp, _vp, _vp, _vp, _i64, _f, _f, _f, _f, _f, _i, _f, _vp],
        "vitssl_ema": [_vp, _vp, _i64, _f, _vp],
        "vitssl_rownorm_fwd": [_vp, _vp, _vp, _i64, _i, _vp],
        "vitssl_rownorm_bwd": [_vp, _vp, _vp, _vp, _i64, _i, _vp],
        "vitssl_weightnorm_fold": [_vp, _vp, _vp, _vp, _i, _i, _vp],
        "vitssl_weightnorm_bwd": [_vp, _vp, _vp, _vp, _vp, _vp, _i, _i, _vp],
        "vitssl_dino_loss_workspace_floats": _returns(_i64, _i, _i, _i),
        "vitssl_dino_loss": [_vp, _vp, _vp, _vp, _i64, _vp, _vp, _i, _i, _i, _i, _f, _f, _f, _vp],
        "vitssl_colsum_f32": [_vp, _vp, _i64, _i, _vp],
        "vitssl_center_ema": [_vp, _vp, _i, _f, _f, _vp],
        "vitssl_bicubic_resize_fwd": [_vp, _vp, _i, _i, _i, _i, _i, _vp],
        "vitssl_bicubic_resize_bwd": [_vp, _vp, _i, _i, _i, _i, _i, _vp],
        "vitssl_aug_resized_crop_u8": [_vp, _vp, _vp, _vp, _i, _i, _i, _i, _vp],
        "vitssl_aug_color_u8": [_vp, _vp, _vp, _i, _i, _vp],
        "vitssl_aug_blur_to_tensor": [_vp, _vp, _vp, _i, _i, _i, _vp],
    },
    "transforms": {
        "vitssl_tf_resized_crop_to_tensor": [_vp, _vp, _vp, _i, _i, _i, _i, _i, _vp],
        "vitssl_debug_tf_tile_rows": _returns(_i, _i, _i, _i, _i),
    },
    "metrics": {
        "vitssl_recon_metrics_workspace_floats": _returns(_i64, _i64, _i, _i),
        "vitssl_recon_metrics": [_vp, _vp, _vp, _i64, _i, _i, _vp, _i64, _vp],
        "vitssl_dino_stats_workspace_floats": _returns(_i64, _i, _i, _i, _i),
        "vitssl_dino_stats": [_vp, _vp, _vp, _vp, _i, _i, _i, _i, _vp, _i64, _vp],
    },
    "classify": {
        "vitssl_classify_loss_workspace_floats": _returns(_i64, _i, _i),
        "vitssl_classify_loss": [_vp, _vp, _i, _i, _i, _d, _i64, _f, _vp, _vp, _i, _vp, _vp, _vp, _vp, _vp, _i64, _vp],
    },
    "attention_hd": {
        "vitssl_attn_hd_fwd": [_vp, _vp, _vp, _vp, _i, _i, _i, _i, _vp],
        "vitssl_attn_hd_bwd": [_vp, _vp, _vp, _vp, _vp, _vp, _i, _i, _i, _i, _vp],
    },
    "patch": {
        "vitssl_patchify_ld_bf16": [_vp, _vp, _i, _i, _i, _i, _i, _i, _vp],
        "vitssl_gather_patches_any_f32": [_vp, _vp, _vp, _i, _i, _i, _i, _i, _vp],
        "vitssl_l1_loss_ld": [_vp, _i64, _vp, _i64, _vp, _vp, _i64, _f, _i64, _i, _vp, _i64, _vp],
        "vitssl_accumulate_ld_f32": [_vp, _vp, _i64, _i, _i64, _vp],
        "vitssl_cast_transpose_batch_ld": [_vp, _vp, _i, _i, _vp],
    },
    "optim": {
        "vitssl_optim_table_bytes": _returns(_i64, _i),
        "vitssl_optim_table_build": [C.POINTER(OptimSegment), _i, _i64, _vp, _i64],
        "vitssl_grad_sumsq_workspace_bytes": _returns(_i64, _i),
        "vitssl_grad_sumsq": [_vp, _vp, _i, _vp, _vp, _i64, _vp],
        "vitssl_adamw_segments": [_vp, _vp, _vp, _vp, _vp, _i, _f, _f, _f, _f, _i, _f, _vp, _f, _vp],
    },
    "mixup": {
        "vitssl_mix_batch": [_vp, _vp, _vp, _vp, _i, _i, _i, _i, _vp],
        "vitssl_classify_loss_mix_workspace_floats": _returns(_i64, _i, _i),
        "vitssl_classify_loss_mix": [_vp, _vp, _vp, _vp, _i, _i, _i, _d, _i64, _f, _vp, _vp, _i, _vp, _vp, _vp, _vp, _vp, _i64, _vp],
    },
    "droppath": {
        "vitssl_droppath_table": [_vp, C.POINTER(C.c_float), C.POINTER(C.c_uint32), _i, _i, C.c_uint64, _vp],
        "vitssl_gemm_bf16_nt_rows": [_pGemm, _pRows, _vp],
        "vitssl_layernorm_bwd_rows": [_vp, _vp, _vp, _vp, _vp, _vp, _vp, _vp, _vp, _vp, _vp, Dropout, _pRows, _i64, _i, _vp, _i64, _vp],
        "vitssl_grad_mask_cast_rows": [_vp, _vp, _vp, Dropout, _pRows, _i64, _i, _vp, _i64, _vp],
    },
    "layerscale": {
        "vitssl_gemm_bf16_nt_ls": [_pGemm, _pCols, _pRows, _vp, _vp],
        "vitssl_layerscale_workspace_floats": _returns(_i64, _i64, _i),
        "vitssl_layernorm_bwd_ls": [_vp, _vp, _vp, _vp, _vp, _vp, _vp, _vp, _vp, _vp, _vp, Dropout, _pRows, _pCols, _vp, _vp, _i64, _i,
                                    _vp, _i64, _vp],
        "vitssl_grad_mask_cast_ls": [_vp, _vp, _vp, Dropout, _pRows, _pCols, _vp, _vp, _i64, _i, _vp, _i64, _vp],
    },
    "lamb": {
        "vitssl_lamb_workspace_bytes": _returns(_i64, C.POINTER(OptimSegment), _i),
        "vitssl_lamb_segments": [_vp, _vp, _vp, _vp, _vp, _i, _f, _f, _f, _f, _i, _f, _vp, _f, _i, _vp, _vp, _i64, _vp],
    },
    "bce": {
        "vitssl_classify_bce_workspace_floats": _returns(_i64, _i, _i),
        "vitssl_classify_bce": [_vp, _vp, _vp, _vp, _i, _i, _i, _d, _d, _i, _i64, _f, _vp, _vp, _i, _vp, _vp, _vp, _vp, _vp, _i64, _vp],
    },
}
REGISTRY = {key: {name: p if isinstance(p, tuple) else (C.c_int, p) for name, p in table.items()} for key, table in _ABI.items()}

_EXT_ABI = {
    "mae": {
        "vitssl_mae_tokens_fwd": [_vp, _vp, _vp, _vp, _vp, _i, _i, _i, _i, _vp],
        "vitssl_mae_tokens_bwd": [_vp, _vp, _vp, _vp, _i, _i, _i, _i, _vp, _i64, _vp],
        "vitssl_mae_unshuffle_fwd": [_vp, _vp, _vp, _vp, _vp, _i, _i, _i, _i, _vp],
        "vitssl_mae_unshuffle_bwd": [_vp, _vp, _vp, _vp, _vp, _i, _i, _i, _i, _vp, _i64, _vp],
        "vitssl_mae_loss": [_vp, _i64, _vp, _vp, _vp, _i64, _i, _i, _i, _f, _vp, _i64, _vp],
        "vitssl_mae_gather_rows_bf16": [_vp, _vp, _vp, _i64, _i, _vp],
        "vitssl_mae_gather_rows_f32": [_vp, _vp, _vp, _i64, _i, _vp],
        "vitssl_mae_scatter_rows_f32": [_vp, _vp, _vp, _i64, _i, _vp],
    },
}
EXT_REGISTRY = {key: {name: p if isinstance(p, tuple) else (C.c_int, p) for name, p in table.items()} for key, table in _EXT_ABI.items()}

DROPPATH_SITE_BIT = 0x80000000
DROPPATH_MAX_SITES = 128
LAMB_ALWAYS_ADAPT, LAMB_TRUST_CLIP = 1, 2

_lib = None


def header_path(key):
    return HEADERS[key] if key in HEADERS else EXT_HEADERS[key]


def header_text(key):
    with open(header_path(key)) as f:
        txt = re.sub(r"/\*.*?\*/", "", f.read(), flags=re.S)
    return re.sub(r"//.*$|^\s*#.*$", "", txt, flags=re.M)


def declarations(key="hip"):
    def ctype(s):
        return re.sub(r"\s*\*", "*", " ".join(s.split()))
    decls = {}
    for ret, name, params in re.findall(r"(?<=[;{}])\s*([A-Za-z_][\w\s*]*?)\b(vitssl_[a-z0-9_]+)\s*\(([^()]*)\)\s*;", header_text(key)):
        params = [] if params.strip() == "void" else [ctype(re.sub(r"\w+\s*$", "", p)) for p in params.split(",")]
        decls[name] = (ctype(ret), params)
    return decls


def header_symbols(key="hip"):
    return sorted(declarations(key))


def lib():
    global _lib
    if _lib is not None:
        return _lib
    if not os.path.exists(LIB_PATH):
        raise VitsslError(
            f"{LIB_PATH} not found: the HIP library is not built. Run `python __graft_entry__.py` "
            "(or __graft_entry__.build()). There is no CPU fallback for the vit_core hot path.")
    import torch
    l = C.CDLL(LIB_PATH)
    if l.vitssl_version() != ABI_VERSION:
        raise VitsslError(f"{LIB_PATH} implements C-ABI version {l.vitssl_version()}, these bindings expect {ABI_VERSION}: "
                          "rebuild it (python __graft_entry__.py)")
    for table in list(REGISTRY.values()) + list(EXT_REGISTRY.values()):
        for name, (restype, argtypes) in table.items():
            fn = getattr(l, name)
            fn.restype, fn.argtypes = restype, argtypes
    _lib = l
    return l


def call(name, *args):
    l = lib()
    rc = getattr(l, name)(*args)
    if rc != 0:
        raise VitsslError(f"{name} failed ({rc}): {l.vitssl_last_error().decode()}")
```

vit-ssl_amd/vitssl_hip/engine.py:

```python
from __future__ import annotations

import re
from typing import Callable, Dict, List, NamedTuple, Optional, Tuple

import numpy as np
import torch
from torch import nn

from . import _lib as L
from . import ops

BF16 = torch.bfloat16
F32 = torch.float32
FP8 = ops.FP8
ALIGN = 64
MAX_TOKENS = 2048
FP8_MAX_TOKENS = 256

import os as _os

_LINEAR_OPERANDS = _os.environ.get("VITSSL_LINEAR_OPERANDS", "bf16")


def set_linear_operands(kind: str):
    global _LINEAR_OPERANDS
    if kind not in ("bf16", "fp8"):
        raise L.VitsslError(f"linear operands must be 'bf16' or 'fp8', got {kind!r}")
    _LINEAR_OPERANDS = kind


def linear_operands() -> str:
    if _LINEAR_OPERANDS not in ("bf16", "fp8"):
        raise L.VitsslError(f"VITSSL_LINEAR_OPERANDS must be 'bf16' or 'fp8', got {_LINEAR_OPERANDS!r}")
    return _LINEAR_OPERANDS


def _round_up(n: int, a: int) -> int:
    return (n + a - 1) // a * a


def as_f32(x: torch.Tensor) -> torch.Tensor:
    if x.dtype != F32:
        x = x.float()
    return x.contiguous()


class PatchGeometry:

    def __init__(self, C: int, P: int):
        self.C, self.P = int(C), int(P)
        self.Pd = self.C * self.P * self.P
        self.native = self.P % 4 == 0 and self.Pd % 64 == 0
        self.Pdp = self.Pd if self.native else _round_up(self.Pd, 64)
        if self.C < 1 or self.P < 1:
            raise L.VitsslError(f"patch_size={P} and the channel count {C} of input_shape must be positive")
        if not self.native and self.C * self.P * (self.P + 31) > 16000:
            raise L.VitsslError(f"patch_size={P} with {C} channels: the channel rows of one patch do not fit the patchify kernel's "
                                f"LDS tile (C * P * (P + 31) = {self.C * self.P * (self.P + 31)} > 16000); a patch size that is a multiple "
                                "of 4 with C * P * P a multiple of 64 has no such limit")
        self.Np = self.Pd if self.Pd % 4 == 0 else self.Pdp

    def patchify(self, x, patches):
        (ops.patchify_bf16 if self.native else ops.patchify_ld_bf16)(x, patches, self.P)

    def register_proj(self, store: "FlatStore", key: str, src: Callable[[], torch.Tensor], D: int):
        if self.native:
            store.register_weight(key, src, transposed_too=False)
        else:
            store.register_padded_weight(key, src, D, self.Pdp, transposed_too=False)

    def proj_image(self, w):
        if self.native:
            wb = torch.empty(w.shape, dtype=BF16, device=w.device)
            ops.cast_transpose_bf16(w, wb, None)
        else:
            wb = torch.zeros(w.shape[0], self.Pdp, dtype=BF16, device=w.device)
            ops.CastPlanLd().run([(w, wb, None)])
        return wb

    def proj_wgrad(self, dproj, patches, gw, ws: "Workspace"):
        if self.native:
            ops.gemm_tn(dproj, patches, gw)
            return
        tmp = ws.get("pad.proj_wgrad", (gw.shape[0], self.Pdp), F32, gw.device)
        tmp.zero_()
        ops.gemm_tn(dproj, patches, tmp)
        ops.accumulate_ld_f32(gw, tmp)

    def gather_targets(self, x, idx, out):
        (ops.gather_patches_f32 if self.native else ops.gather_patches_any_f32)(x, idx, out, self.P)

    def l1_loss(self, pred, targets, loss_sum, dpred, gscale):
        (ops.l1_loss if self.native else ops.l1_loss_ld)(pred, targets, loss_sum, dpred, gscale=gscale)

    def widen_grad(self, dpred):
        dp = as_f32(dpred)
        if dp.numel() == 0:
            return torch.empty(0, self.Pdp, dtype=BF16, device=dp.device)
        dpb = torch.empty(dp.shape, dtype=BF16, device=dp.device)
        ops.cast_bf16(dp, dpb)
        if self.Pdp != self.Pd:
            wide = torch.zeros(dp.shape[0], self.Pdp, dtype=BF16, device=dp.device)
            wide[:, :self.Pd] = dpb
            dpb = wide
        return dpb


class Workspace:

    def __init__(self):
        self._bufs: Dict[str, torch.Tensor] = {}

    def get(self, name: str, shape, dtype, device) -> torch.Tensor:
        t = self._bufs.get(name)
        shape = tuple(int(s) for s in shape)
        if t is None or t.shape != shape or t.dtype != dtype or t.device != device:
            t = torch.empty(shape, dtype=dtype, device=device)
            self._bufs[name] = t
        return t

    def clear(self):
        self._bufs.clear()


class PatchHead:

    def __init__(self, store: "FlatStore", geo: PatchGeometry, key: str, weight_name: str, bias_name: str, D: int, ws: Workspace):
        self.store, self.geo, self.key, self.wname, self.bname, self.D, self.ws = store, geo, key, weight_name, bias_name, int(D), ws
        src = lambda: store.view(weight_name, (geo.Pd, self.D))
        if geo.native:
            store.register_weight(key, src)
        else:
            store.register_padded_weight(key, src, geo.Pdp, self.D)

    def forward(self, h):
        st, Pd, Np = self.store, self.geo.Pd, self.geo.Np
        if Np == Pd:
            pred = torch.empty(h.shape[0], Pd, dtype=F32, device=h.device)
            ops.gemm_nt(h, st.w(self.key)[:Pd], pred, L.EPI_F32, bias=st.view(self.bname))
            return pred
        bias = self.ws.get(f"pad.{self.key}_bias", (Np,), F32, h.device)
        bias.zero_()
        bias[:Pd].copy_(st.view(self.bname))
        wide = torch.empty(h.shape[0], Np, dtype=F32, device=h.device)
        ops.gemm_nt(h, st.w(self.key), wide, L.EPI_F32, bias=bias)
        return wide[:, :Pd]

    def wgrad(self, dpred, h):
        Pd, Pdp = self.geo.Pd, self.geo.Pdp
        gb, gw = self.store.gview(self.bname, (1, Pd)), self.store.gview(self.wname, (Pd, self.D))
        if self.geo.native:
            ops.colsum_bf16(dpred, gb.view(Pd))
            ops.gemm_tn(dpred, h, gw)
            return
        hb = self.ws.get(f"pad.{self.key}_bgrad", (1, Pdp), F32, h.device)
        hw = self.ws.get(f"pad.{self.key}_wgrad", (Pdp, self.D), F32, h.device)
        hb.zero_()
        hw.zero_()
        ops.colsum_bf16(dpred, hb.view(Pdp))
        ops.gemm_tn(dpred, h, hw)
        ops.accumulate_ld_f32(gb, hb)
        ops.accumulate_ld_f32(gw, hw[:Pd])

    def dgrad(self, dpred, out):
        ops.gemm_nt(dpred, self.store.w(self.key + ".T"), out, L.EPI_BF16)


class HostStage:

    def __init__(self, slots: int = 4):
        self.slots, self._ring, self._key, self._pos = int(slots), [], None, 0

    def upload(self, arrays, dev) -> List[torch.Tensor]:
        offs, total = [], 0
        for a in arrays:
            offs.append(total)
            total = _round_up(total + a.nbytes, 256)
        if self._key != (total, str(dev)):
            self._ring = [[torch.empty(total, dtype=torch.uint8).pin_memory(), torch.empty(total, dtype=torch.uint8, device=dev), None]
                          for _ in range(self.slots)]
            self._key, self._pos = (total, str(dev)), 0
        slot = self._ring[self._pos % self.slots]
        self._pos += 1
        host, d, ev = slot
        if ev is not None:
            ev.synchronize()
        staged = host.numpy()
        for o, a in zip(offs, arrays):
            staged[o:o + a.nbytes] = a.view(np.uint8)
        d.copy_(host, non_blocking=True)
        slot[2] = torch.cuda.Event()
        slot[2].record(torch.cuda.current_stream())
        return [d[o:o + a.nbytes].view(torch.from_numpy(a[:0]).dtype) for o, a in zip(offs, arrays)]


_BLOCK_NAME = re.compile(r"(?:^|\.)encoder_blocks\.(\d+)\.")
_TOKEN_NAMES = ("cls_token", "positional_embedding", "mask_token")


def num_layers(names) -> int:
    ids = [int(m.group(1)) for m in map(_BLOCK_NAME.search, names) if m]
    return max(ids) + 1 if ids else 0


def layer_id(name: str, layers: int) -> int:
    m = _BLOCK_NAME.search(name)
    if m:
        return int(m.group(1)) + 1
    parts = name.split(".")
    if "patch_embedding" in parts or parts[0] == "projection" or parts[-1] in _TOKEN_NAMES:
        return 0
    return layers + 1


def exempt_from_weight_decay(name: str, ndim: int) -> bool:
    return ndim <= 1 or name.split(".")[-1] in _TOKEN_NAMES


class FlatStore:

    def __init__(self, module: nn.Module, device: torch.device, only: Optional[Callable[[str], bool]] = None,
                 forward_only: bool = False):
        self.module = module
        self.device = device
        self.forward_only = bool(forward_only)
        self.names: List[str] = []
        self.params: List[nn.Parameter] = []
        self.offsets: Dict[str, Tuple[int, int]] = {}
        off = 0
        for name, p in module.named_parameters():
            if only is not None and not only(name):
                continue
            n = p.numel()
            self.names.append(name)
            self.params.append(p)
            self.offsets[name] = (off, n)
            off = _round_up(off + n, ALIGN)
        self.numel = off
        self.flat = torch.zeros(off, dtype=F32, device=device)
        self.gflat = torch.zeros(off, dtype=F32, device=device)
        with torch.no_grad():
            for name, p in zip(self.names, self.params):
                o, n = self.offsets[name]
                view = self.flat[o:o + n].view(p.shape)
                view.copy_(p.data)
                p.data = view
        self._bf16: Dict[str, torch.Tensor] = {}
        self._bf16_key = None
        self.generation = 0
        self._cast_jobs: List[Tuple[str, Callable[[], torch.Tensor], bool, bool]] = []
        self._cast_pad: Dict[str, Tuple[int, int]] = {}
        self._fp8: Dict[str, torch.Tensor] = {}
        self._fp8_jobs: List[Tuple[str, Callable[[], torch.Tensor]]] = []
        self._fp8_plan = None
        self._fp8_index: Dict[str, int] = {}

    def is_attached(self) -> bool:
        base = self.flat.data_ptr()
        for name, p in zip(self.names, self.params):
            o, _ = self.offsets[name]
            if p.data_ptr() != base + 4 * o:
                return False
        return True

    def view(self, name: str, shape=None) -> torch.Tensor:
        o, n = self.offsets[name]
        v = self.flat[o:o + n]
        return v.view(shape) if shape is not None else v

    def gview(self, name: str, shape=None) -> torch.Tensor:
        o, n = self.offsets[name]
        v = self.gflat[o:o + n]
        return v.view(shape) if shape is not None else v

    def span(self, first: str, last: str) -> Tuple[int, int]:
        lo = self.offsets[first][0]
        o, n = self.offsets[last]
        return lo, o + n

    def prefix_span(self, prefix: str) -> Tuple[int, int]:
        names = [n for n in self.names if n.startswith(prefix)]
        return self.span(names[0], names[-1])

    def span_view(self, first: str, last: str, shape, grad=False) -> torch.Tensor:
        lo, hi = self.span(first, last)
        buf = self.gflat if grad else self.flat
        v = buf[lo:hi]
        if v.numel() != int(torch.Size(shape).numel()):
            raise L.VitsslError(f"parameters {first}..{last} are not contiguous in the flat store")
        return v.view(shape)

    def attach_grads(self):
        for name, p in zip(self.names, self.params):
            p.grad = self.gview(name, p.shape)

    def mark_dirty(self):
        self.generation += 1

    def weights_key(self):
        pv = 0
        for p in self.params:
            pv += p._version
        return (self.generation, self.flat._version, pv)

    def register_weight(self, key: str, src: Callable[[], torch.Tensor], transposed_too: bool = True, plain: bool = True):
        self._cast_jobs.append((key, src, transposed_too and not self.forward_only, plain))

    def register_padded_weight(self, key: str, src: Callable[[], torch.Tensor], rows: int, cols: int, transposed_too: bool = True):
        self._cast_pad[key] = (int(rows), int(cols))
        self.register_weight(key, src, transposed_too)

    def register_fp8_weight(self, key: str, src: Callable[[], torch.Tensor]):
        self._fp8_index[key] = len(self._fp8_jobs)
        self._fp8_jobs.append((key, src))

    def refresh_weights(self):
        key = self.weights_key()
        if key == self._bf16_key and (self._bf16 or self._fp8):
            return
        jobs = []
        for wname, src, tr, plain in self._cast_jobs:
            w = src()
            R, Cn = w.shape
            alloc = torch.empty
            if wname in self._cast_pad:
                R, Cn = self._cast_pad[wname]
                alloc = torch.zeros
            dst = self._bf16.get(wname) if plain else None
            if plain and (dst is None or dst.shape != (R, Cn)):
                dst = alloc(R, Cn, dtype=BF16, device=self.device)
                self._bf16[wname] = dst
            dst_t = None
            if tr:
                dst_t = self._bf16.get(wname + ".T")
                if dst_t is None or dst_t.shape != (Cn, R):
                    dst_t = alloc(Cn, R, dtype=BF16, device=self.device)
                    self._bf16[wname + ".T"] = dst_t
            jobs.append((w.contiguous(), dst, dst_t))
        if jobs:
            if getattr(self, "_cast_plan", None) is None:
                self._cast_plan = ops.CastPlanLd() if self._cast_pad else ops.CastPlan()
            self._cast_plan.run(jobs)
        if self._fp8_jobs:
            jobs8 = []
            for k8, src in self._fp8_jobs:
                w = src()
                R, Cn = w.shape
                dst, dst_t = self._fp8.get(k8), self._fp8.get(k8 + ".T")
                if dst is None or dst.shape != (R, Cn):
                    dst = torch.empty(R, Cn, dtype=FP8, device=self.device)
                    dst_t = torch.empty(Cn, R, dtype=FP8, device=self.device)
                    self._fp8[k8], self._fp8[k8 + ".T"] = dst, dst_t
                jobs8.append((w.contiguous(), dst, dst_t))
            if self._fp8_plan is None:
                self._fp8_plan = ops.Fp8WeightPlan()
            self._fp8_plan.run(jobs8)
        self._bf16_key = key

    def w(self, key: str) -> torch.Tensor:
        return self._bf16[key]

    def w8(self, key: str) -> Tuple[torch.Tensor, torch.Tensor]:
        j = self._fp8_index[key]
        return self._fp8[key], self._fp8_plan.alpha[j:j + 1]

    def w8t(self, key: str) -> Tuple[torch.Tensor, torch.Tensor]:
        j = self._fp8_index[key]
        return self._fp8[key + ".T"], self._fp8_plan.alpha[j:j + 1]


RESERVED_CUS_DEFAULT = 8


def configure_collectives(reserve_cus: int = RESERVED_CUS_DEFAULT):
    if "NCCL_MAX_NCHANNELS" not in _os.environ:
        _os.environ["NCCL_MAX_NCHANNELS"] = str(max(1, int(reserve_cus)))
    if "NCCL_MIN_NCHANNELS" not in _os.environ:
        _os.environ["NCCL_MIN_NCHANNELS"] = str(min(int(_os.environ["NCCL_MAX_NCHANNELS"]), max(1, int(reserve_cus))))
    return {k: _os.environ.get(k) for k in ("NCCL_MAX_NCHANNELS", "NCCL_MIN_NCHANNELS")}


class GradReducer:

    def __init__(self, gflat: torch.Tensor, group=None, bucket_mb: float = 32.0, expect=None,
                 reserve_cus: int = RESERVED_CUS_DEFAULT):
        import torch.distributed as dist
        self.dist = dist
        self.gflat = gflat
        self.group = group
        self.world = dist.get_world_size(group) if dist.is_available() and dist.is_initialized() else 1
        if self.world > 1 and gflat.is_cuda:
            if "VITSSL_RESERVE_CUS" not in _os.environ:
                L.call("vitssl_set_reserved_cus", int(reserve_cus))
        self.bucket_elems = int(bucket_mb * 1024 * 1024 / 4)
        self.pending: List[Tuple[int, int]] = []
        self.pending_elems = 0
        self.handles = []
        self.cuda = gflat.is_cuda
        self.comm_stream = torch.cuda.Stream(device=gflat.device, priority=-1) if self.cuda else None
        self.launched: List[Tuple[int, int]] = []
        self.expect = expect if expect is not None else (0, gflat.numel())
        self.check_coverage = True
        self.timing = False
        self._t0 = None
        self._bucket_events = []

    def _flush(self):
        if not self.pending:
            return
        rng = sorted(self.pending)
        merged = [list(rng[0])]
        for lo, hi in rng[1:]:
            if lo <= merged[-1][1]:
                merged[-1][1] = max(merged[-1][1], hi)
            else:
                merged.append([lo, hi])
        self.pending, self.pending_elems = [], 0
        for lo, hi in merged:
            self.launched.append((lo, hi))
            if self.world == 1:
                continue
            chunk = self.gflat[lo:hi]
            if self.cuda:
                self.comm_stream.wait_stream(torch.cuda.current_stream())
                with torch.cuda.stream(self.comm_stream):
                    if self.timing:
                        e0, e1 = torch.cuda.Event(enable_timing=True), torch.cuda.Event(enable_timing=True)
                        e0.record(self.comm_stream)
                    self.dist.all_reduce(chunk, group=self.group)
                    if self.timing:
                        e1.record(self.comm_stream)
                        self._bucket_events.append((4 * (hi - lo), e0, e1))
            else:
                self.handles.append(self.dist.all_reduce(chunk, group=self.group, async_op=True))

    def begin(self):
        self.pending, self.pending_elems, self.handles, self.launched = [], 0, [], []
        if self.timing and self.cuda:
            self._bucket_events = []
            self._t0 = torch.cuda.Event(enable_timing=True)
            self._t0.record(torch.cuda.current_stream())

    def bucket_times(self):
        if not self._bucket_events:
            return []
        torch.cuda.synchronize()
        return [(nbytes, round(self._t0.elapsed_time(e0), 3), round(e0.elapsed_time(e1), 3)) for nbytes, e0, e1 in self._bucket_events]

    def ready(self, lo: int, hi: int):
        self.pending.append((lo, hi))
        self.pending_elems += hi - lo
        if self.pending_elems >= self.bucket_elems:
            self._flush()

    def finish(self):
        self._flush()
        for h in self.handles:
            h.wait()
        self.handles = []
        if self.cuda and self.world > 1:
            torch.cuda.current_stream().wait_stream(self.comm_stream)
        if self.check_coverage:
            self._assert_covered()

    def _assert_covered(self):
        if isinstance(self.expect, list):
            return self._assert_covered_ranges()
        pos = self.expect[0]
        for lo, hi in sorted(self.launched):
            if lo < pos:
                raise L.VitsslError(f"GradReducer: gradient range [{lo}, {hi}) was reduced twice (previous range ended at {pos})")
            if lo - pos >= ALIGN:
                raise L.VitsslError(f"GradReducer: gradient range [{pos}, {lo}) was never handed to the reducer")
            pos = hi
        if self.expect[1] - pos >= ALIGN:
            raise L.VitsslError(f"GradReducer: gradient range [{pos}, {self.expect[1]}) was never handed to the reducer")

    @staticmethod
    def _minus(a, b):
        out = []
        for lo, hi in sorted(a):
            pos = lo
            for blo, bhi in b:
                if bhi <= pos or blo >= hi:
                    continue
                if blo - pos >= ALIGN:
                    out.append((pos, blo))
                pos = max(pos, bhi)
            if hi - pos >= ALIGN:
                out.append((pos, hi))
        return out

    def _assert_covered_ranges(self):
        got, want = sorted(self.launched), sorted(self.expect)
        pos = None
        for lo, hi in got:
            if pos is not None and lo < pos:
                raise L.VitsslError(f"GradReducer: gradient range [{lo}, {hi}) was reduced twice (previous range ended at {pos})")
            pos = hi
        for lo, hi in self._minus(want, got):
            raise L.VitsslError(f"GradReducer: gradient range [{lo}, {hi}) was never handed to the reducer")
        for lo, hi in self._minus(got, want):
            raise L.VitsslError(f"GradReducer: gradient range [{lo}, {hi}) is outside the expected ranges {want}")

    def stats(self):
        return len(self.launched), 4 * sum(hi - lo for lo, hi in self.launched)

    @property
    def grad_scale(self) -> float:
        return 1.0 / self.world


def drop_path_rates(rate: float, layers: int) -> List[float]:
    rate = float(rate)
    if not 0.0 <= rate < 1.0:
        raise ValueError(f"drop_path_rate must lie in [0, 1), got {rate}")
    if layers <= 1:
        return [0.0] * max(layers, 0)
    return [rate * i / (layers - 1) for i in range(layers)]


class _GradOperand(NamedTuple):
    x: Optional[torch.Tensor]
    x8: Optional[torch.Tensor] = None
    scale: Optional[torch.Tensor] = None
    amax: Optional[torch.Tensor] = None
    inv: Optional[torch.Tensor] = None


class EncoderStack:

    def __init__(self, store: FlatStore, block_prefixes: List[str], D: int, H: int, F: int, p_drop: float,
                 site_base: int = 0, drop_path: Optional[List[float]] = None, layer_scale: bool = False):
        if D % H != 0:
            raise AssertionError(f"d_model({D}) must be cleanly divisible by num_heads({H})!")
        self.store = store
        self.bp = list(block_prefixes)
        self._spans = [store.prefix_span(b) for b in self.bp]
        self.L, self.D, self.H, self.F = len(self.bp), D, H, F
        self.dh = D // H
        self.p = float(p_drop)
        self.site_base = site_base
        self.ws = Workspace()
        self._saved = {}
        self.fp8 = linear_operands() == "fp8"
        rates = [float(r) for r in drop_path] if drop_path is not None else []
        if rates and len(rates) != self.L:
            raise ValueError(f"drop_path holds {len(rates)} rates for {self.L} blocks")
        if any(not 0.0 <= r < 1.0 for r in rates):
            raise ValueError(f"drop_path rates must lie in [0, 1), got {rates}")
        self.drop_path = rates if any(r > 0.0 for r in rates) else None
        if self.drop_path is not None and self.fp8:
            raise L.VitsslError("drop path (drop_path_rate > 0) is built for bf16 linear operands only: use bf16 operands "
                                "(set_linear_operands('bf16') or VITSSL_LINEAR_OPERANDS=bf16) or drop_path_rate = 0")
        if self.drop_path is not None and 2 * self.L > L.DROPPATH_MAX_SITES:
            raise L.VitsslError(f"drop path covers up to {L.DROPPATH_MAX_SITES // 2} blocks a stack, got {self.L}")
        self.layer_scale = bool(layer_scale)
        if self.layer_scale:
            if self.fp8:
                raise L.VitsslError("LayerScale (layer_scale_init) is built for bf16 linear operands only: use bf16 operands "
                                    "(set_linear_operands('bf16') or VITSSL_LINEAR_OPERANDS=bf16) or leave layer_scale_init out")
            for b in self.bp:
                for leaf in ("layer_scale1.gamma", "layer_scale2.gamma"):
                    if b + leaf not in store.offsets:
                        raise L.VitsslError(f"LayerScale: the store holds no parameter {b + leaf!r}")
                    if store.offsets[b + leaf][1] != D:
                        raise L.VitsslError(f"LayerScale: {b + leaf!r} holds {store.offsets[b + leaf][1]} values, expected embed_dim = {D}")
        if self.fp8 and (D % 128 != 0 or F % 128 != 0):
            raise L.VitsslError(f"fp8 linear operands need embed_dim ({D}) and mlp_dim ({F}) to be multiples of 128")
        for b in self.bp:
            a = b + "self_attention."
            srcs = {
                "wqkv": lambda a=a, D=D: store.span_view(a + "w_query.weight", a + "w_value.weight", (3 * D, D)),
                "wo": lambda a=a: store.view(a + "final_linear.weight", (D, D)),
                "w1": lambda b=b: store.view(b + "feed_forward.linear_in.weight", (F, D)),
                "w2": lambda b=b: store.view(b + "feed_forward.linear_out.weight", (D, F)),
            }
            for leaf, src in srcs.items():
                if self.fp8:
                    store.register_fp8_weight(b + leaf, src)
                else:
                    store.register_weight(b + leaf, src)
        self._gs_by_slot: Dict[str, dict] = {}
        self._gs = None

    def _n(self, i, leaf):
        return self.bp[i] + leaf

    def block_span(self, i) -> Tuple[int, int]:
        return self._spans[i]

    def _drop(self, i, which, seed, training):
        if not training or self.p <= 0.0:
            return ops.NO_DROP
        return ops.make_dropout(self.p, seed, self.site_base + 3 * i + which)

    def needs_seed(self, training: bool) -> bool:
        return bool(training) and (self.p > 0.0 or self.drop_path is not None)

    def drop_path_sites(self) -> List[Tuple[float, int]]:
        return [(r, L.DROPPATH_SITE_BIT | ((self.site_base + 2 * i + br) & 0x7FFFFFFF)) for i, r in enumerate(self.drop_path or [])
                for br in (0, 1)]

    def drop_path_table(self, slot: str = "a") -> Optional[torch.Tensor]:
        return self._saved[slot].get("dp")

    def check_tokens(self, T: int):
        if self.fp8 and self.dh != 64:
            raise L.VitsslError(f"fp8 linear operands support head dim 64 only, got embed_dim / num_heads = {self.D} / {self.H} = "
                                f"{self.dh}: use bf16 operands (set_linear_operands('bf16') or VITSSL_LINEAR_OPERANDS=bf16), which "
                                f"cover {ops.HD_SUPPORTED}")
        ops.attn_family(self.dh)
        if self.fp8 and T > FP8_MAX_TOKENS:
            raise L.VitsslError(f"fp8 linear operands support sequences of up to {FP8_MAX_TOKENS} tokens, got {T}: use bf16 "
                                f"operands (set_linear_operands('bf16') or VITSSL_LINEAR_OPERANDS=bf16), which cover up to "
                                f"{MAX_TOKENS} tokens")
        if T > MAX_TOKENS:
            raise L.VitsslError(f"sequence length {T} > {MAX_TOKENS} unsupported by the attention kernels")

    def _scaled(self, dp, T, i, k, branch=None, dls=False):
        kw = {}
        if dp is not None and self.drop_path[i] > 0.0:
            kw["rows"] = (dp[2 * i + k - 1], T)
        if self.layer_scale:
            name = self._n(i, f"layer_scale{k}.gamma")
            kw["cols"] = self.store.view(name)
            if branch is not None:
                kw["branch"] = branch
            if dls:
                kw["dls"] = self.store.gview(name)
        return kw

    def _ln_fwd(self, x, i, leaf, y, mean, rstd):
        gamma, beta = self.store.view(self._n(i, leaf + ".weight")), self.store.view(self._n(i, leaf + ".bias"))
        if self.fp8:
            ops.layernorm_fwd_fp8(x, gamma, beta, None, y, mean, rstd)
        else:
            ops.layernorm_fwd(x, gamma, beta, y, mean, rstd)

    def _gemm(self, A, i, leaf, out, epilogue, dgrad=False, image=None, **kw):
        name = self._n(i, leaf)
        if self.fp8:
            w, alpha = (self.store.w8t if dgrad else self.store.w8)(name)
            ops.gemm_fp8_nt(A, w, out, epilogue, alpha=alpha, out_fp8=image, **kw)
        else:
            ops.gemm_nt(A, self.store.w(name + ".T" if dgrad else name), out, epilogue, out1=image, **kw)

    def _attn_fwd(self, qkv, att, att_op, lse, B, T, probs):
        if self.fp8:
            ops.attn_fwd(qkv, att, lse, B, T, self.H, self.dh, probs=probs, out_fp8=att_op)
        else:
            ops.attn_fwd_any(qkv, att, lse, B, T, self.H, self.dh, probs=probs)

    def _attn_bwd(self, s, dout, q, delta, B, T):
        if self.fp8:
            ops.attn_bwd(s["qkv"], s["att"], dout, s["lse"], q.x, delta, B, T, self.H, self.dh, dqkv_fp8=q.x8, scale=q.scale, amax=q.amax)
            self._settle(q)
        else:
            ops.attn_bwd_any(s["qkv"], s["att"], dout, s["lse"], q.x, delta, B, T, self.H, self.dh)

    def _dgrad(self, q, i, leaf, out, epilogue=L.EPI_BF16, emits=None, **kw):
        if self.fp8:
            kw["alpha2"] = q.inv
            if emits is not None:
                kw.update(image=emits.x8, out_scale=emits.scale, out_amax=emits.amax)
        self._gemm(q.x8 if self.fp8 else q.x, i, leaf, out, epilogue, dgrad=True, **kw)
        if self.fp8 and emits is not None:
            self._settle(emits)

    def _ln_bwd(self, ln, g, q, gm_colsum, drop, **scaled):
        f8 = (q.x8, q.scale, q.amax) if self.fp8 else ()
        if ln is None:
            (ops.grad_mask_cast_fp8 if self.fp8 else ops.grad_mask_cast)(g, q.x, *f8, gm_colsum, drop, **scaled)
        else:
            *head, i, leaf = ln
            w, b = self._n(i, leaf + ".weight"), self._n(i, leaf + ".bias")
            (ops.layernorm_bwd_fp8 if self.fp8 else ops.layernorm_bwd)(*head, self.store.view(w), g, g, q.x, *f8, self.store.gview(w),
                                                                       self.store.gview(b), gm_colsum, drop, **scaled)
        if self.fp8:
            self._settle(q)

    def forward(self, x: torch.Tensor, B: int, T: int, training: bool, seed: int, save: bool, slot: str = "a",
                return_attn: bool = False):
        st, D, H, F = self.store, self.D, self.H, self.F
        self.check_tokens(T)
        M = B * T
        dev = x.device
        g = self.ws.get
        probs = None
        rec = {"B": B, "T": T, "seed": seed, "training": training, "blocks": []}
        dp = None
        if training and self.drop_path is not None:
            dp = ops.droppath_table(self.drop_path_sites(), B, seed, g(f"{slot}.dp" if save else f"{slot}.tmp.dp", (2 * self.L, B), F32, dev))
        rec["dp"] = dp
        cur = x
        for i in range(self.L):
            tag = f"{slot}.{i}." if save else f"{slot}.tmp."
            img = lambda n, n8, cols: g(tag + (n8 if self.fp8 else n), (M, cols), FP8 if self.fp8 else BF16, dev)
            h1, h2, a = img("h1", "h1_8", D), img("h2", "h2_8", D), img("a", "a8", F)
            att = g(tag + "att", (M, D), BF16, dev)
            att_op = img("att", "att8", D) if self.fp8 else att
            ls1 = g(tag + "ls1", (M, D), BF16, dev) if self.layer_scale and save else None
            ls2 = g(tag + "ls2", (M, D), BF16, dev) if self.layer_scale and save else None
            mean1, rstd1 = g(tag + "mean1", (M,), F32, dev), g(tag + "rstd1", (M,), F32, dev)
            mean2, rstd2 = g(tag + "mean2", (M,), F32, dev), g(tag + "rstd2", (M,), F32, dev)
            qkv = g(tag + "qkv", (M, 3 * D), BF16, dev)
            lse = g(tag + "lse", (B, H, T), F32, dev)
            xmid = g(tag + "xmid", (M, D), F32, dev)
            u = g(tag + "u", (M, F), BF16, dev)
            xout = g(f"{slot}.{i}.xout" if save else f"{slot}.tmp.xout{i & 1}", (M, D), F32, dev)

            if return_attn and i == self.L - 1:
                probs = torch.empty(B, H, T, T, dtype=F32, device=dev)
            b1, b2 = st.view(self._n(i, "feed_forward.linear_in.bias")), st.view(self._n(i, "feed_forward.linear_out.bias"))
            self._ln_fwd(cur, i, "layer_norm1", h1, mean1, rstd1)
            self._gemm(h1, i, "wqkv", qkv, L.EPI_BF16)
            self._attn_fwd(qkv, att, att_op, lse, B, T, probs if i == self.L - 1 else None)
            self._gemm(att_op, i, "wo", xmid, L.EPI_RESID, aux=cur, drop=self._drop(i, 0, seed, training), **self._scaled(dp, T, i, 1, branch=ls1))
            self._ln_fwd(xmid, i, "layer_norm2", h2, mean2, rstd2)
            self._gemm(h2, i, "w1", u, L.EPI_GELU, bias=b1, image=a, drop=self._drop(i, 1, seed, training))
            self._gemm(a, i, "w2", xout, L.EPI_RESID, bias=b2, aux=xmid, drop=self._drop(i, 2, seed, training), **self._scaled(dp, T, i, 2, branch=ls2))
            if save:
                rec["blocks"].append(dict(xin=cur, h1=h1, mean1=mean1, rstd1=rstd1, qkv=qkv, att=att, att_op=att_op, lse=lse, xmid=xmid,
                                          h2=h2, mean2=mean2, rstd2=rstd2, u=u, a=a, ls1=ls1, ls2=ls2))
            cur = xout
        if save:
            self._saved[slot] = rec
        return cur, probs

    def backward(self, g: torch.Tensor, slot: str = "a", reducer: Optional[GradReducer] = None,
                 scale_key: Optional[str] = None, input_grad_only: bool = False) -> torch.Tensor:
        st, D, H, F = self.store, self.D, self.H, self.F
        rec = self._saved[slot]
        B, T, seed, training, dp = rec["B"], rec["T"], rec["seed"], rec["training"], rec.get("dp")
        M = B * T
        dev = g.device
        w = self.ws.get
        bw = f"bwd{M}."
        gv = st.gview
        last = self.L - 1
        wgrad = self.fp8 or not input_grad_only
        gs = self._grad_scale_state(dev, scale_key or slot) if self.fp8 else None
        jit = self.fp8 and not gs["valid"]
        kinds = (("gm", "gm8", D), ("du", "du8", F), ("gm2" if wgrad and not self.fp8 else "gm", "gm8b", D), ("dqkv", "dq8", 3 * D))
        x = [w(bw + n, (M, cols), BF16, dev) if not self.fp8 or jit else None for n, _, cols in kinds]
        x8 = [w(bw + n8, (M, cols), FP8, dev) if self.fp8 else None for _, n8, cols in kinds]
        dh_ = w(bw + "dh", (M, D), BF16, dev)
        delta = w(bw + "delta", (B, H, T), F32, dev)

        plain = [_GradOperand(t) for t in x]

        def grad(i, t):
            if not self.fp8:
                return plain[t]
            return _GradOperand(x[t], x8[t], gs["scale"][i, t:t + 1], gs["amax"][i, t:t + 1], gs["inv"][i, t:t + 1])

        def scaled(i, k):
            return self._scaled(dp, T, i, k, branch=rec["blocks"][i][f"ls{k}"] if wgrad else None, dls=wgrad)

        gm = grad(last, 0)
        self._ln_bwd(None, g, gm, gv(self._n(last, "feed_forward.linear_out.bias")), self._drop(last, 2, seed, training), **scaled(last, 2))
        for i in range(last, -1, -1):
            s = rec["blocks"][i]
            a_ = self.bp[i] + "self_attention."
            du, gm2, dqkv = grad(i, 1), grad(i, 2), grad(i, 3)
            self._dgrad(gm, i, "w2", du.x, L.EPI_DGELU, emits=du, aux=s["u"],
                        colsum=gv(self._n(i, "feed_forward.linear_in.bias")))
            self._dgrad(du, i, "w1", dh_)
            self._ln_bwd((dh_, s["xmid"], s["mean2"], s["rstd2"], i, "layer_norm2"), g, gm2, None, self._drop(i, 0, seed, training),
                         **scaled(i, 1))
            self._dgrad(gm2, i, "wo", dh_)
            self._attn_bwd(s, dh_, dqkv, delta, B, T)
            self._dgrad(dqkv, i, "wqkv", dh_)
            if wgrad:
                jobs = [(gm, s["a"], gv(self._n(i, "feed_forward.linear_out.weight"), (D, F))),
                        (du, s["h2"], gv(self._n(i, "feed_forward.linear_in.weight"), (F, D))),
                        (gm2, s["att_op"], gv(a_ + "final_linear.weight", (D, D))),
                        (dqkv, s["h1"], st.span_view(a_ + "w_query.weight", a_ + "w_value.weight", (3 * D, D), grad=True))]
                if self.fp8:
                    ops.gemm_fp8_tn_batch([(q.x8, act, dw, None, q.inv) for q, act, dw in jobs])
                else:
                    ops.gemm_tn_batch([(q.x, act, dw) for q, act, dw in jobs])
            ln1 = (dh_, s["xin"], s["mean1"], s["rstd1"])
            if i > 0:
                gm = grad(i - 1, 0)
                self._ln_bwd(ln1 + (i, "layer_norm1"), g, gm, gv(self._n(i - 1, "feed_forward.linear_out.bias")),
                             self._drop(i - 1, 2, seed, training), **scaled(i - 1, 2))
            else:
                ops.layernorm_bwd(*ln1, st.view(self._n(i, "layer_norm1.weight")), g, g, None,
                                  gv(self._n(i, "layer_norm1.weight")), gv(self._n(i, "layer_norm1.bias")), None, ops.NO_DROP)
            if reducer is not None and wgrad:
                lo, hi = self.block_span(i)
                reducer.ready(lo, hi)
        if self.fp8:
            gs["used"].copy_(gs["scale"])
            self._rescale(gs["scale"], gs["inv"], gs["amax"], margin=1)
            gs["amax"].zero_()
            gs["valid"] = True
        return g

    @staticmethod
    def _scale_from_amax(amax: torch.Tensor, margin: int) -> torch.Tensor:
        mant, e = torch.frexp(amax)
        k = (9 - e - (mant > 0.875).to(e.dtype) - margin).clamp(-120, 120)
        return torch.bitwise_left_shift(k.to(torch.int32) + 127, 23).view(torch.float32)

    def _grad_scale_state(self, dev, slot: str = "a"):
        gs = self._gs_by_slot.get(slot)
        if gs is None or gs["scale"].device != dev:
            mk = lambda v: torch.full((self.L, 4), v, dtype=F32, device=dev)
            gs = {"scale": mk(1.0), "inv": mk(1.0), "amax": mk(0.0), "used": mk(1.0), "valid": False}
            self._gs_by_slot[slot] = gs
        self._gs = gs
        return gs

    def _rescale(self, scale, inv, amax, margin: int):
        ok = (amax > 0) & torch.isfinite(amax)
        new = torch.where(ok, self._scale_from_amax(torch.where(ok, amax, torch.ones_like(amax)), margin), scale)
        scale.copy_(new)
        inv.copy_(1.0 / new)

    def _settle(self, q):
        if q.x is not None and q.x8 is not None:
            self._rescale(q.scale, q.inv, q.amax, margin=0)
            ops.quantize_fp8(q.x, q.x8, scale=q.scale)

    def fp8_grad_scales(self, slot: Optional[str] = None) -> torch.Tensor:
        gs = self._gs if slot is None else self._gs_by_slot[slot]
        return gs["used"].clone()

    def recalibrate_fp8(self):
        for gs in self._gs_by_slot.values():
            gs["valid"] = False
```

vit-ssl_amd/vitssl_hip/ops.py:

```python
import collections
import ctypes as C
import operator

import torch

from . import _lib as L
from ._lib import Dropout, Embed, Fp8Gemm, Gemm, call

BF16 = torch.bfloat16
F32 = torch.float32
FP8 = torch.float8_e4m3fn


def _stream():
    return C.c_void_p(torch.cuda.current_stream().cuda_stream)


def _chk(t, dtype, name, shape=None):
    if t is None:
        raise L.VitsslError(f"{name}: tensor is None")
    if not t.is_cuda:
        raise L.VitsslError(f"{name}: expected a CUDA (HIP) tensor, got {t.device}; there is no CPU fallback")
    if t.device.index != torch.cuda.current_device():
        raise L.VitsslError(f"{name}: tensor lives on {t.device} but the current device is cuda:{torch.cuda.current_device()}; "
                            "call torch.cuda.set_device (one process per GPU) before using the engine")
    if t.dtype != dtype:
        raise L.VitsslError(f"{name}: expected dtype {dtype}, got {t.dtype}")
    if not t.is_contiguous():
        raise L.VitsslError(f"{name}: tensor must be contiguous")
    if shape is not None and tuple(t.shape) != tuple(shape):
        raise L.VitsslError(f"{name}: expected shape {tuple(shape)}, got {tuple(t.shape)}")
    return C.c_void_p(t.data_ptr())


def _opt(t, dtype, name, shape=None):
    return C.c_void_p(0) if t is None else _chk(t, dtype, name, shape)


def make_dropout(p=0.0, seed=0, site=0):
    return Dropout(float(p), int(site) & 0xFFFFFFFF, int(seed) & 0xFFFFFFFFFFFFFFFF)


NO_DROP = make_dropout()

PROFILE = None


def _prof_begin():
    if PROFILE is None:
        return None
    ev = torch.cuda.Event(enable_timing=True)
    ev.record(torch.cuda.current_stream())
    return ev


def _prof_end(ev0, label, flops, nbytes=0):
    if ev0 is None:
        return
    ev1 = torch.cuda.Event(enable_timing=True)
    ev1.record(torch.cuda.current_stream())
    PROFILE.append((label, flops, ev0, ev1, nbytes))


def dropout_mask(rows, cols, drop, device):
    keep = torch.empty(rows, cols, dtype=torch.uint8, device=device)
    call("vitssl_dropout_mask", _chk(keep, torch.uint8, "keep"), rows, cols, drop, _stream())
    return keep


def layernorm_fwd(x, gamma, beta, y, mean, rstd, eps=1e-5):
    rows, cols = x.shape
    ev = _prof_begin()
    call("vitssl_layernorm_fwd", _chk(x, F32, "x"), _chk(gamma, F32, "gamma", (cols,)), _chk(beta, F32, "beta", (cols,)),
         _chk(y, BF16, "y", (rows, cols)), _chk(mean, F32, "mean", (rows,)), _chk(rstd, F32, "rstd", (rows,)),
         rows, cols, float(eps), _stream())
    _prof_end(ev, "ln_fwd", 0.0, rows * (6 * cols + 8))


def layernorm_fwd_fp8(x, gamma, beta, y, y8, mean, rstd, eps=1e-5):
    rows, cols = x.shape
    ev = _prof_begin()
    call("vitssl_layernorm_fwd_fp8", _chk(x, F32, "x"), _chk(gamma, F32, "gamma", (cols,)), _chk(beta, F32, "beta", (cols,)),
         _opt(y, BF16, "y", (rows, cols)), _chk(y8, FP8, "y8", (rows, cols)), _chk(mean, F32, "mean", (rows,)),
         _chk(rstd, F32, "rstd", (rows,)), rows, cols, float(eps), _stream())
    _prof_end(ev, "ln_fwd", 0.0, rows * ((7 if y is not None else 5) * cols + 8))


def _scalar(t, name):
    if t is None:
        return C.c_void_p(0)
    if t.numel() != 1:
        raise L.VitsslError(f"{name}: expected a 1-element fp32 device tensor")
    return _chk(t, F32, name)


def quantize_fp8(x, y8, scale=None, amax=None):
    call("vitssl_quantize_fp8_scaled", _chk(x, BF16, "x"), _chk(y8, FP8, "y8", x.shape), x.numel(), _scalar(scale, "scale"),
         _scalar(amax, "amax"), _stream())


def droppath_table(pairs, B, seed, out):
    n = len(pairs)
    if not 1 <= n <= L.DROPPATH_MAX_SITES:
        raise L.VitsslError(f"droppath_table: {n} (rate, site) pairs outside [1, {L.DROPPATH_MAX_SITES}]")
    rates = (C.c_float * n)(*[float(r) for r, _ in pairs])
    sites = (C.c_uint32 * n)(*[int(s) & 0xFFFFFFFF for _, s in pairs])
    call("vitssl_droppath_table", _chk(out, F32, "scale", (n, B)), rates, sites, n, int(B), C.c_uint64(int(seed) & 0xFFFFFFFFFFFFFFFF),
         _stream())
    return out


def _rowscale(rows, M, name):
    scale, rpg = rows
    rpg = int(rpg)
    if rpg <= 0 or M % rpg != 0:
        raise L.VitsslError(f"{name}: rows_per_group {rpg} does not divide the {M} rows")
    r = L.RowScale()
    r.scale = _chk(scale, F32, name + " rows.scale", (M // rpg,))
    r.groups, r.rows_per_group = M // rpg, rpg
    return r


def _colscale(cols, N, name):
    c = L.ColScale()
    c.gamma = _chk(cols, F32, name + " cols(gamma)", (N,))
    c.cols = N
    return c


_LnForm = collections.namedtuple("_LnForm", "sfx query")
_LN_PLAIN = _LnForm("", "vitssl_sum_workspace_floats")
_LN_FP8 = _LnForm("_fp8", "vitssl_sum_workspace_floats")
_LN_ROWS = _LnForm("_rows", "vitssl_sum_workspace_floats")
_LN_LS = _LnForm("_ls", "vitssl_layerscale_workspace_floats")


def _ln_bwd(who, ln, g_res, gm, gm_colsum, drop, fp8=None, rows=None, cols=None, branch=None, dls=None):
    M, N = (ln[1] if ln else g_res).shape
    if cols is not None:
        if (branch is None) != (dls is None):
            raise L.VitsslError(f"{who}: branch= and dls= are given together (gamma's gradient) or both left out")
        form = _LN_LS
        extra = (C.byref(_rowscale(rows, M, who)) if rows is not None else None, C.byref(_colscale(cols, N, who)),
                 _opt(branch, BF16, who + " branch", (M, N)), _opt(dls, F32, who + " dls", (N,)))
    else:
        if branch is not None or dls is not None:
            raise L.VitsslError(f"{who}: branch= / dls= belong to cols= (LayerScale)")
        form = _LN_FP8 if fp8 else (_LN_PLAIN if rows is None else _LN_ROWS)
        extra = () if rows is None else (C.byref(_rowscale(rows, M, who)),)
    if ln:
        dy, x, mean, rstd, gamma, g_out, dgamma, dbeta = ln
        head = (_chk(dy, BF16, "dy", (M, N)), _chk(x, F32, "x"), _chk(mean, F32, "mean", (M,)), _chk(rstd, F32, "rstd", (M,)),
                _chk(gamma, F32, "gamma", (N,)), _opt(g_res, F32, "g_res", (M, N)), _chk(g_out, F32, "g_out", (M, N)))
    else:
        head = (_chk(g_res, F32, "g"),)
    gm_p = (_opt if fp8 or (ln and form is not _LN_LS) else _chk)(gm, BF16, "gm", (M, N))
    q8 = (_chk(fp8[0], FP8, "gm8", (M, N)), _scalar(fp8[1], "scale"), _scalar(fp8[2], "amax")) if fp8 else ()
    sums = (_chk(dgamma, F32, "dgamma", (N,)), _chk(dbeta, F32, "dbeta", (N,))) if ln else ()
    ws = _tn_workspace((ln[1] if ln else g_res).device, int(getattr(L.lib(), form.query)(M, N)))
    ev = _prof_begin() if ln else None
    call("vitssl_" + ("layernorm_bwd" if ln else "grad_mask_cast") + form.sfx, *head, gm_p, *q8, *sums,
         _opt(gm_colsum, F32, "gm_colsum", (N,)), drop, *extra, M, N, C.c_void_p(ws.data_ptr()), ws.numel(), _stream())
    _prof_end(ev, "ln_bwd", 0.0, M * (N * (2 + 4 + (4 if g_res is not None else 0) + 4 + (2 if gm is not None else 0) + (1 if fp8 else 0)
                                           + (2 if branch is not None else 0)) + 8))


def layernorm_bwd(dy, x, mean, rstd, gamma, g_res, g_out, gm, dgamma, dbeta, gm_colsum=None, drop=NO_DROP, rows=None, cols=None,
                  branch=None, dls=None):
    _ln_bwd("layernorm_bwd", (dy, x, mean, rstd, gamma, g_out, dgamma, dbeta), g_res, gm, gm_colsum, drop, rows=rows, cols=cols,
            branch=branch, dls=dls)


def layernorm_bwd_fp8(dy, x, mean, rstd, gamma, g_res, g_out, gm, gm8, scale, amax, dgamma, dbeta, gm_colsum=None, drop=NO_DROP):
    _ln_bwd("layernorm_bwd_fp8", (dy, x, mean, rstd, gamma, g_out, dgamma, dbeta), g_res, gm, gm_colsum, drop, fp8=(gm8, scale, amax))


def grad_mask_cast(g, gm, gm_colsum=None, drop=NO_DROP, rows=None, cols=None, branch=None, dls=None):
    _ln_bwd("grad_mask_cast", None, g, gm, gm_colsum, drop, rows=rows, cols=cols, branch=branch, dls=dls)


def grad_mask_cast_fp8(g, gm, gm8, scale, amax, gm_colsum=None, drop=NO_DROP):
    _ln_bwd("grad_mask_cast_fp8", None, g, gm, gm_colsum, drop, fp8=(gm8, scale, amax))


_OUT0_DTYPE = {L.EPI_BF16: BF16, L.EPI_F32: F32, L.EPI_GELU: BF16, L.EPI_RESID: F32, L.EPI_DGELU: BF16, L.EPI_EMBED: F32}


def _nt_desc(who, sfx, dtype, A, B, epilogue, bias, set_out0, aux, dgelu_aux, out1, colsum, drop, epilogues=None):
    M, K = A.shape
    N, K2 = B.shape
    if K != K2:
        raise L.VitsslError(f"{who}: K mismatch {K} vs {K2}")
    if epilogues is not None and epilogue not in epilogues:
        raise L.VitsslError(f"{who}: epilogue {epilogue} has no fp8-operand form")
    g = Gemm()
    g.A = _chk(A, dtype, "A" + sfx)
    g.B = _chk(B, dtype, "B" + sfx)
    g.M, g.N, g.K = M, N, K
    g.epilogue = epilogue
    g.bias = _opt(bias, F32, "bias", (N,))
    set_out0(g, M, N)
    if epilogue == L.EPI_RESID:
        g.aux = _chk(aux, F32, "aux(residual)", (M, N))
    elif epilogue == L.EPI_DGELU:
        g.aux = _chk(aux, BF16, dgelu_aux, (M, N))
    g.out1 = _opt(out1, BF16, "out1", (M, N))
    g.colsum = _opt(colsum, F32, "colsum", (N,))
    if colsum is not None:
        g.workspace, g.workspace_floats = _sum_ws(colsum.device, M, N)
    g.drop = drop
    return g, M, N, K


def gemm_nt(A, B, out0, epilogue, bias=None, aux=None, out1=None, colsum=None, drop=NO_DROP, embed=None, rows=None, cols=None,
            branch=None):
    def set_out0(g, M, N):
        if epilogue != L.EPI_EMBED:
            g.out0 = _chk(out0, _OUT0_DTYPE[epilogue], "out0", (M, N))
            return
        if embed is None:
            raise L.VitsslError("gemm_nt: EPI_EMBED needs embed=(mask, mask_token, pos, tokens, out_tokens, tok_offset)")
        mask, mask_token, pos, tokens, out_tokens, tok_offset = embed
        if M % tokens != 0:
            raise L.VitsslError("gemm_nt: M must be a multiple of tokens")
        e = Embed()
        e.mask = _opt(mask, torch.uint8, "mask", (M,))
        e.mask_token = _opt(mask_token, F32, "mask_token", (N,))
        e.pos = _chk(pos, F32, "pos", (out_tokens, N))
        e.tokens, e.out_tokens, e.tok_offset = tokens, out_tokens, tok_offset
        g.embed = e
        g.out0 = _chk(out0, F32, "out0", ((M // tokens) * out_tokens, N))

    g, M, N, K = _nt_desc("gemm_nt", "", BF16, A, B, epilogue, bias, set_out0, aux, "aux(u)", out1, colsum, drop)
    ev = _prof_begin()
    if cols is not None:
        if epilogue != L.EPI_RESID:
            raise L.VitsslError(f"gemm_nt: cols= belongs to EPI_RESID, got epilogue {epilogue}")
        call("vitssl_gemm_bf16_nt_ls", C.byref(g), C.byref(_colscale(cols, N, "gemm_nt")),
             C.byref(_rowscale(rows, M, "gemm_nt")) if rows is not None else None, _opt(branch, BF16, "branch", (M, N)), _stream())
    elif branch is not None:
        raise L.VitsslError("gemm_nt: branch= belongs to cols= (LayerScale)")
    elif rows is not None:
        if epilogue != L.EPI_RESID:
            raise L.VitsslError(f"gemm_nt: rows= belongs to EPI_RESID, got epilogue {epilogue}")
        call("vitssl_gemm_bf16_nt_rows", C.byref(g), C.byref(_rowscale(rows, M, "gemm_nt")), _stream())
    else:
        call("vitssl_gemm_bf16_nt", C.byref(g), _stream())
    _prof_end(ev, f"gemm_nt[epi{epilogue}] {M}x{N}x{K}", 2.0 * M * N * K)


def gemm_fp8_nt(A8, B8, out0, epilogue, alpha=None, bias=None, aux=None, out1=None, out_fp8=None, drop=NO_DROP,
                alpha2=None, colsum=None, out_scale=None, out_amax=None):
    def set_out0(g, M, N):
        if out0 is None and not (epilogue == L.EPI_DGELU and out_fp8 is not None):
            raise L.VitsslError("gemm_fp8_nt: out0 may only be omitted for EPI_DGELU with out_fp8")
        g.out0 = _opt(out0, _OUT0_DTYPE[epilogue], "out0", (M, N))

    g, M, N, K = _nt_desc("gemm_fp8_nt", "8", FP8, A8, B8, epilogue, bias, set_out0, aux, "aux(g')", out1, colsum, drop,
                          epilogues=(L.EPI_BF16, L.EPI_F32, L.EPI_GELU, L.EPI_RESID, L.EPI_DGELU))
    q = Fp8Gemm()
    q.alpha = _scalar(alpha, "alpha")
    q.alpha2 = _scalar(alpha2, "alpha2")
    q.out_fp8 = _opt(out_fp8, FP8, "out_fp8", (M, N))
    q.out_scale = _scalar(out_scale, "out_scale")
    q.out_amax = _scalar(out_amax, "out_amax")
    if out_fp8 is not None and epilogue not in (L.EPI_GELU, L.EPI_DGELU):
        raise L.VitsslError("gemm_fp8_nt: out_fp8 belongs to EPI_GELU / EPI_DGELU")
    ev = _prof_begin()
    call("vitssl_gemm_fp8_nt", C.byref(g), C.byref(q), _stream())
    _prof_end(ev, f"gemm_fp8_nt[epi{epilogue}] {M}x{N}x{K}", 2.0 * M * N * K)


_TN_WS = {}


def _tn_workspace(device, floats):
    key = (device, torch.cuda.current_stream().cuda_stream)
    ws = _TN_WS.get(key)
    if ws is None or ws.numel() < floats:
        ws = torch.empty(max(floats, 1 << 20), dtype=F32, device=device)
        _TN_WS[key] = ws
    return ws


def _sum_ws(device, rows, cols):
    ws = _tn_workspace(device, int(L.lib().vitssl_sum_workspace_floats(rows, cols)))
    return C.c_void_p(ws.data_ptr()), ws.numel()


_TnKind = collections.namedtuple("_TnKind", "label dtype sfx scalars entry query batch_entry batch_query Job")
_TN_BF16 = _TnKind("gemm_tn", BF16, "", (), "vitssl_gemm_bf16_tn", "vitssl_gemm_tn_workspace_floats",
                   "vitssl_gemm_bf16_tn_batch", "vitssl_gemm_tn_batch_workspace_floats", L.TnJob)
_TN_FP8 = _TnKind("gemm_fp8_tn", FP8, "8", ("alpha", "alpha2"), "vitssl_gemm_fp8_tn", "vitssl_gemm_fp8_tn_workspace_floats",
                  "vitssl_gemm_fp8_tn_batch", "vitssl_gemm_fp8_tn_batch_workspace_floats", L.Fp8TnJob)


def _tn_single(k, A, B, Cacc, scalars, atomic):
    M, N1 = A.shape
    M2, N2 = B.shape
    if M != M2:
        raise L.VitsslError(f"{k.label}: M mismatch {M} vs {M2}")
    a, b, c = _chk(A, k.dtype, "A" + k.sfx), _chk(B, k.dtype, "B" + k.sfx), _chk(Cacc, F32, "C", (N1, N2))
    if atomic:
        wsp, wsn = C.c_void_p(0), 0
    else:
        ws = _tn_workspace(A.device, int(getattr(L.lib(), k.query)(M, N1, N2)))
        wsp, wsn = C.c_void_p(ws.data_ptr()), ws.numel()
    ev = _prof_begin()
    call(k.entry, a, b, c, M, N1, N2, *scalars, wsp, wsn, _stream())
    _prof_end(ev, f"{k.label} {N1}x{N2}x{M}", 2.0 * M * N1 * N2)


def _tn_batch(k, jobs):
    if not jobs:
        return
    M = jobs[0][0].shape[0]
    arr = (k.Job * len(jobs))()
    flops = 0.0
    for j, (A, B, Cacc, *scalars) in enumerate(jobs):
        if len(scalars) != len(k.scalars):
            raise L.VitsslError(f"{k.label}_batch: job {j}: expected (A, B, C{''.join(', ' + n for n in k.scalars)})")
        if A.shape[0] != M or B.shape[0] != M:
            raise L.VitsslError(f"{k.label}_batch: job {j}: row counts {A.shape[0]} / {B.shape[0]} differ from {M}")
        N1, N2 = A.shape[1], B.shape[1]
        q = arr[j]
        setattr(q, "A" + k.sfx, _chk(A, k.dtype, "A" + k.sfx).value)
        setattr(q, "B" + k.sfx, _chk(B, k.dtype, "B" + k.sfx).value)
        q.C, q.N1, q.N2 = _chk(Cacc, F32, "C", (N1, N2)).value, N1, N2
        for name, t in zip(k.scalars, scalars):
            setattr(q, name, _scalar(t, name).value)
        flops += 2.0 * M * N1 * N2
    ws = _tn_workspace(jobs[0][0].device, int(getattr(L.lib(), k.batch_query)(arr, len(jobs), M)))
    ev = _prof_begin()
    call(k.batch_entry, arr, len(jobs), M, C.c_void_p(ws.data_ptr()), ws.numel(), _stream())
    _prof_end(ev, f"{k.label} batch{len(jobs)}x{M}", flops)


def gemm_tn(A, B, Cacc, atomic=False):
    _tn_single(_TN_BF16, A, B, Cacc, (), atomic)


def gemm_fp8_tn(A8, B8, Cacc, alpha=None, alpha2=None, atomic=False):
    _tn_single(_TN_FP8, A8, B8, Cacc, (_scalar(alpha, "alpha"), _scalar(alpha2, "alpha2")), atomic)


def gemm_tn_batch(jobs):
    _tn_batch(_TN_BF16, jobs)


def gemm_fp8_tn_batch(jobs):
    _tn_batch(_TN_FP8, jobs)


def attn_fwd(qkv, out, lse, B, N, H, dh, probs=None, out_fp8=None):
    ev = _prof_begin()
    _attn_fwd(qkv, out, lse, B, N, H, dh, probs, out_fp8)
    _prof_end(ev, f"attn_fwd B{B} N{N} H{H}", 4.0 * B * H * N * N * dh)


def _attn_fwd(qkv, out, lse, B, N, H, dh, probs=None, out_fp8=None):
    if out_fp8 is not None:
        call("vitssl_attn_fwd_fp8", _chk(qkv, BF16, "qkv", (B * N, 3 * H * dh)), _chk(out, BF16, "out", (B * N, H * dh)),
             _chk(out_fp8, FP8, "out_fp8", (B * N, H * dh)), _chk(lse, F32, "lse", (B, H, N)),
             _opt(probs, F32, "probs", (B, H, N, N)), B, N, H, dh, _stream())
        return
    call("vitssl_attn_fwd", _chk(qkv, BF16, "qkv", (B * N, 3 * H * dh)), _chk(out, BF16, "out", (B * N, H * dh)),
         _chk(lse, F32, "lse", (B, H, N)), _opt(probs, F32, "probs", (B, H, N, N)), B, N, H, dh, _stream())


def attn_bwd(qkv, out, dout, lse, dqkv, delta_ws, B, N, H, dh, dqkv_fp8=None, scale=None, amax=None):
    ev = _prof_begin()
    if dqkv_fp8 is not None:
        call("vitssl_attn_bwd_fp8", _chk(qkv, BF16, "qkv", (B * N, 3 * H * dh)), _chk(out, BF16, "out", (B * N, H * dh)),
             _chk(dout, BF16, "dout", (B * N, H * dh)), _chk(lse, F32, "lse", (B, H, N)), _opt(dqkv, BF16, "dqkv", (B * N, 3 * H * dh)),
             _chk(dqkv_fp8, FP8, "dqkv_fp8", (B * N, 3 * H * dh)), _scalar(scale, "scale"), _scalar(amax, "amax"), B, N, H, dh, _stream())
    else:
        _attn_bwd(qkv, out, dout, lse, dqkv, delta_ws, B, N, H, dh)
    _prof_end(ev, f"attn_bwd B{B} N{N} H{H}", 8.0 * B * H * N * N * dh)


def _attn_bwd(qkv, out, dout, lse, dqkv, delta_ws, B, N, H, dh):
    call("vitssl_attn_bwd", _chk(qkv, BF16, "qkv", (B * N, 3 * H * dh)), _chk(out, BF16, "out", (B * N, H * dh)),
         _chk(dout, BF16, "dout", (B * N, H * dh)), _chk(lse, F32, "lse", (B, H, N)),
         _chk(dqkv, BF16, "dqkv", (B * N, 3 * H * dh)), _chk(delta_ws, F32, "delta_ws", (B, H, N)), B, N, H, dh, _stream())


HD_MIN, HD_MAX, HD_STEP = 8, 128, 8
HD_SUPPORTED = "head dims 8, 16, ..., 128 (multiples of 8; 64 runs the dh = 64 kernels)"


def attn_hd_fwd(qkv, out, lse, B, N, H, dh, probs=None):
    ev = _prof_begin()
    call("vitssl_attn_hd_fwd", _chk(qkv, BF16, "qkv", (B * N, 3 * H * dh)), _chk(out, BF16, "out", (B * N, H * dh)),
         _chk(lse, F32, "lse", (B, H, N)), _opt(probs, F32, "probs", (B, H, N, N)), B, N, H, dh, _stream())
    _prof_end(ev, f"attn_hd_fwd B{B} N{N} H{H} dh{dh}", 4.0 * B * H * N * N * dh)


def attn_hd_bwd(qkv, out, dout, lse, dqkv, delta_ws, B, N, H, dh):
    ev = _prof_begin()
    call("vitssl_attn_hd_bwd", _chk(qkv, BF16, "qkv", (B * N, 3 * H * dh)), _chk(out, BF16, "out", (B * N, H * dh)),
         _chk(dout, BF16, "dout", (B * N, H * dh)), _chk(lse, F32, "lse", (B, H, N)),
         _chk(dqkv, BF16, "dqkv", (B * N, 3 * H * dh)), _chk(delta_ws, F32, "delta_ws", (B, H, N)), B, N, H, dh, _stream())
    _prof_end(ev, f"attn_hd_bwd B{B} N{N} H{H} dh{dh}", 8.0 * B * H * N * N * dh)


def attn_family(dh):
    try:
        d = operator.index(dh)
    except TypeError:
        d = None
    if d == 64:
        return attn_fwd, attn_bwd
    if d is not None and HD_MIN <= d <= HD_MAX and d % HD_STEP == 0:
        return attn_hd_fwd, attn_hd_bwd
    raise L.VitsslError(f"head dim {dh} (embed_dim / num_heads) unsupported by the attention kernels: supported are {HD_SUPPORTED}")


def attn_fwd_any(qkv, out, lse, B, N, H, dh, probs=None):
    attn_family(dh)[0](qkv, out, lse, B, N, H, dh, probs=probs)


def attn_bwd_any(qkv, out, dout, lse, dqkv, delta_ws, B, N, H, dh):
    attn_family(dh)[1](qkv, out, dout, lse, dqkv, delta_ws, B, N, H, dh)


def patchify_bf16(img, patches, P):
    B, Cc, H, W = img.shape
    call("vitssl_patchify_bf16", _chk(img, F32, "img"), _chk(patches, BF16, "patches", (B * (H // P) * (W // P), Cc * P * P)),
         B, Cc, H, W, P, _stream())


def gather_patches_f32(img, idx, out, P):
    B, Cc, H, W = img.shape
    n = idx.numel()
    call("vitssl_gather_patches_f32", _chk(img, F32, "img"), _chk(idx, torch.int32, "idx"), _chk(out, F32, "out", (n, Cc * P * P)),
         n, Cc, H, W, P, _stream())


def gather_rows_bf16(x, idx, out):
    rows, cols = x.shape
    n = idx.numel()
    call("vitssl_gather_rows_bf16", _chk(x, F32, "x"), _chk(idx, torch.int32, "idx"), _chk(out, BF16, "out", (n, cols)), n, cols, _stream())


def scatter_rows_f32(src, inv, g):
    rows, cols = g.shape
    call("vitssl_scatter_rows_f32", _chk(src, BF16, "src"), _chk(inv, torch.int32, "inv", (rows,)), _chk(g, F32, "g"), rows, cols, _stream())


def gather_cls_f32(x, out, B, T, D):
    call("vitssl_gather_cls_f32", _chk(x, F32, "x", (B * T, D)), _chk(out, F32, "out", (B, D)), B, T, D, _stream())


def scatter_cls_f32(gcls, g, B, T, D):
    call("vitssl_scatter_cls_f32", _chk(gcls, F32, "gcls", (B, D)), _chk(g, F32, "g", (B * T, D)), B, T, D, _stream())


def embed_bwd(dtok, mask, dproj, dpos, dmask_token, dbias, dcls, B, tokens, tok_offset, D):
    T_out = tokens + tok_offset
    wsn = int(L.lib().vitssl_embed_bwd_workspace_floats(B, tokens, tok_offset, D))
    ws = _tn_workspace(dtok.device, wsn)
    call("vitssl_embed_bwd", _chk(dtok, F32, "dtok", (B * T_out, D)), _opt(mask, torch.uint8, "mask", (B * tokens,)),
         _chk(dproj, BF16, "dproj", (B * tokens, D)), _opt(dpos, F32, "dpos", (T_out, D)),
         _opt(dmask_token, F32, "dmask_token", (D,)), _opt(dbias, F32, "dbias", (D,)), _opt(dcls, F32, "dcls", (D,)),
         B, tokens, tok_offset, D, C.c_void_p(ws.data_ptr()), ws.numel(), _stream())


def l1_loss(pred, target, loss_sum, dpred=None, gscale=0.0):
    n = pred.numel()
    call("vitssl_l1_loss", _chk(pred, F32, "pred"), _chk(target, F32, "target", pred.shape), _chk(loss_sum, F32, "loss_sum", (1,)),
         _opt(dpred, BF16, "dpred", pred.shape), float(gscale), n, *_sum_ws(pred.device, n, 1), _stream())


def cross_entropy(logits, labels, loss_sum, dlogits=None, gscale=0.0):
    B, Cn = logits.shape
    call("vitssl_cross_entropy", _chk(logits, F32, "logits"), _chk(labels, torch.int64, "labels", (B,)),
         _chk(loss_sum, F32, "loss_sum", (1,)), _opt(dlogits, BF16, "dlogits", (B, Cn)), float(gscale), B, Cn, _stream())


def colsum_bf16(x, out):
    rows, cols = x.shape
    call("vitssl_colsum_bf16", _chk(x, BF16, "x"), _chk(out, F32, "out", (cols,)), rows, cols, *_sum_ws(x.device, rows, cols), _stream())


def cast_bf16(src, dst):
    call("vitssl_cast_bf16", _chk(src, F32, "src"), _chk(dst, BF16, "dst", src.shape), src.numel(), _stream())


def cast_transpose_bf16(src, dst, dst_t):
    R, Cn = src.shape
    call("vitssl_cast_transpose_bf16", _chk(src, F32, "src"), _opt(dst, BF16, "dst", (R, Cn)), _opt(dst_t, BF16, "dst_t", (Cn, R)),
         R, Cn, _stream())


class _JobTablePlan:
    Job = entry = dst_dtype = None

    def __init__(self):
        self.key = None
        self.jobs_dev = None
        self.starts_dev = None
        self.njobs = 0
        self.total = 0
        self.keep = None

    def _record(self, s, d, t):
        return (s.data_ptr(), 0 if d is None else d.data_ptr(), 0 if t is None else t.data_ptr(), s.shape[0], s.shape[1])

    def _check(self, s, d, t):
        R, Cn = s.shape
        _chk(s, F32, "src"); _opt(d, self.dst_dtype, "dst", (R, Cn)); _opt(t, self.dst_dtype, "dst_t", (Cn, R))

    def _rebuilt(self, dev):
        """per-table device state behind the job table (none here)"""

    def _extra(self):
        return ()

    def run(self, jobs):
        import numpy as np
        key = tuple(self._record(s, d, t) for s, d, t in jobs)
        if key != self.key:
            for s, d, t in jobs:
                self._check(s, d, t)
            dev = jobs[0][0].device
            rec = np.zeros(len(jobs), dtype=np.dtype(self.Job))
            starts = np.zeros(len(jobs) + 1, dtype=np.int32)
            for i, k in enumerate(key):
                rec[i] = k
                starts[i + 1] = starts[i] + ((k[3] + 63) // 64) * ((k[4] + 63) // 64)
            self.jobs_dev = torch.from_numpy(rec.view(np.uint8).copy()).to(dev)
            self.starts_dev = torch.from_numpy(starts).to(dev)
            self.njobs, self.total, self.key = len(jobs), int(starts[-1]), key
            self._rebuilt(dev)
        self.keep = jobs
        call(self.entry, C.c_void_p(self.jobs_dev.data_ptr()), C.c_void_p(self.starts_dev.data_ptr()), self.njobs, self.total,
             *self._extra(), _stream())


class CastPlan(_JobTablePlan):
    Job, entry, dst_dtype = L.CastJob, "vitssl_cast_transpose_batch", BF16


def _chk_ld(t, dtype, name, rows, cols):
    if t is None:
        raise L.VitsslError(f"{name}: tensor is None")
    if not t.is_cuda or t.device.index != torch.cuda.current_device():
        raise L.VitsslError(f"{name}: expected a tensor of the current CUDA (HIP) device, got {t.device}; there is no CPU fallback")
    if t.dtype != dtype:
        raise L.VitsslError(f"{name}: expected dtype {dtype}, got {t.dtype}")
    if tuple(t.shape) != (rows, cols):
        raise L.VitsslError(f"{name}: expected shape {(rows, cols)}, got {tuple(t.shape)}")
    ld = t.stride(0) if rows > 1 else max(t.stride(0), cols)
    if t.stride(1) != 1 or ld < cols:
        raise L.VitsslError(f"{name}: expected unit column stride and a row stride >= {cols}, got strides {tuple(t.stride())}")
    return C.c_void_p(t.data_ptr()), int(ld)


def patchify_ld_bf16(img, patches, P):
    B, Cc, H, W = img.shape
    if P <= 0 or H % P != 0 or W % P != 0:
        raise L.VitsslError(f"patchify_ld: image {H}x{W} not divisible by patch {P}")
    rows = B * (H // P) * (W // P)
    if patches is None or patches.dim() != 2 or patches.shape[1] < Cc * P * P:
        raise L.VitsslError(f"patchify_ld: expected patches [{rows}, ld >= {Cc * P * P}], got {None if patches is None else tuple(patches.shape)}")
    call("vitssl_patchify_ld_bf16", _chk(img, F32, "img"), _chk(patches, BF16, "patches", (rows, patches.shape[1])), B, Cc, H, W, P,
         patches.shape[1], _stream())


def gather_patches_any_f32(img, idx, out, P):
    B, Cc, H, W = img.shape
    n = idx.numel()
    call("vitssl_gather_patches_any_f32", _chk(img, F32, "img"), _chk(idx, torch.int32, "idx"), _chk(out, F32, "out", (n, Cc * P * P)),
         n, Cc, H, W, P, _stream())


def l1_loss_ld(pred, target, loss_sum, dpred=None, gscale=0.0):
    rows, cols = pred.shape
    pp, ld_p = _chk_ld(pred, F32, "pred", rows, cols)
    tp, ld_t = _chk_ld(target, F32, "target", rows, cols)
    ld_d = 0
    if dpred is not None:
        if dpred.dim() != 2 or dpred.shape[0] != rows or dpred.shape[1] < cols:
            raise L.VitsslError(f"l1_loss_ld: dpred must be [{rows}, ld_d >= {cols}], got {tuple(dpred.shape)}")
        ld_d = dpred.shape[1]
    call("vitssl_l1_loss_ld", pp, ld_p, tp, ld_t, _chk(loss_sum, F32, "loss_sum", (1,)), _opt(dpred, BF16, "dpred"), ld_d, float(gscale),
         rows, cols, *_sum_ws(pred.device, rows * cols, 1), _stream())


def accumulate_ld_f32(dst, src, cols=None):
    rows, c = dst.shape
    if src is None or src.dim() != 2 or src.shape[0] != rows or src.shape[1] < c:
        raise L.VitsslError(f"accumulate_ld: src must be [{rows}, ld >= {c}], got {None if src is None else tuple(src.shape)}")
    call("vitssl_accumulate_ld_f32", _chk(dst, F32, "dst"), _chk(src, F32, "src"), rows, c, src.shape[1], _stream())


class CastPlanLd(CastPlan):
    Job, entry = L.CastLdJob, "vitssl_cast_transpose_batch_ld"

    def _record(self, s, d, t):
        return super()._record(s, d, t) + (0 if d is None else d.shape[1], 0 if t is None else t.shape[1])

    def _check(self, s, d, t):
        R, Cn = s.shape
        _chk(s, F32, "src"); _opt(d, BF16, "dst"); _opt(t, BF16, "dst_t")
        if d is not None and (d.dim() != 2 or d.shape[0] < R or d.shape[1] < Cn):
            raise L.VitsslError(f"cast plan: dst {tuple(d.shape)} does not hold the [{R}, {Cn}] source")
        if t is not None and (t.dim() != 2 or t.shape[0] < Cn or t.shape[1] < R):
            raise L.VitsslError(f"cast plan: dst_t {tuple(t.shape)} does not hold the transposed [{R}, {Cn}] source")


class Fp8WeightPlan(_JobTablePlan):
    Job, entry, dst_dtype = L.Fp8WeightJob, "vitssl_fp8_quantize_weights", FP8

    def __init__(self):
        super().__init__()
        self.amax = self.alpha = None

    def _rebuilt(self, dev):
        self.amax = torch.zeros(self.njobs, dtype=F32, device=dev)
        self.alpha = torch.ones(self.njobs, dtype=F32, device=dev)

    def _extra(self):
        return C.c_void_p(self.amax.data_ptr()), C.c_void_p(self.alpha.data_ptr())


def adamw(p, g, m, v, lr, beta1, beta2, eps, wd, step, gscale=1.0):
    n = p.numel()
    ev = _prof_begin()
    call("vitssl_adamw", _chk(p, F32, "p"), _chk(g, F32, "g", p.shape), _chk(m, F32, "m", p.shape), _chk(v, F32, "v", p.shape),
         n, float(lr), float(beta1), float(beta2), float(eps), float(wd), int(step), float(gscale), _stream())
    _prof_end(ev, "adamw", 0.0, 28 * n)


class AdamWPlan:

    def __init__(self, segments, numel, device):
        segments = [(int(o), int(n), float(s), float(w)) for o, n, s, w in segments]
        l = L.lib()
        self.nseg, self.numel = len(segments), int(numel)
        nbytes = int(l.vitssl_optim_table_bytes(self.nseg))
        host = torch.zeros(max(nbytes, 8), dtype=torch.uint8)
        arr = (L.OptimSegment * max(self.nseg, 1))(*[L.OptimSegment(*s) for s in segments])
        call("vitssl_optim_table_build", arr, self.nseg, self.numel, C.c_void_p(host.data_ptr()), nbytes)
        self.elements = sum(s[1] for s in segments)
        self.table = host.to(device)
        self.workspace = torch.empty(int(l.vitssl_grad_sumsq_workspace_bytes(self.nseg)), dtype=torch.uint8, device=device)
        self.sumsq = torch.zeros(1, dtype=F32, device=device)
        self._rows, self.lamb_workspace, self.trust = arr, None, None

    def lamb_buffers(self):
        if self.trust is None:
            nbytes = int(L.lib().vitssl_lamb_workspace_bytes(self._rows, self.nseg))
            if nbytes <= 0:
                raise L.VitsslError(f"vitssl_lamb_workspace_bytes refused a table of {self.nseg} segments")
            self.lamb_workspace = torch.empty(nbytes, dtype=torch.uint8, device=self.table.device)
            self.trust = torch.ones(self.nseg, dtype=F32, device=self.table.device)
        return self.lamb_workspace, self.trust


def _flat(t, name, plan):
    if t.dim() != 1 or t.numel() != plan.numel:
        raise L.VitsslError(f"{name}: expected the flat buffer of {plan.numel} floats the plan was built for, got {tuple(t.shape)}")
    return _chk(t, F32, name)


def grad_sumsq(g, plan, out=None, workspace=None):
    out = plan.sumsq if out is None else out
    ws = plan.workspace if workspace is None else workspace
    ev = _prof_begin()
    call("vitssl_grad_sumsq", _flat(g, "g", plan), _chk(plan.table, torch.uint8, "table"), plan.nseg, _chk(out, F32, "out", (1,)),
         _chk(ws, torch.uint8, "workspace"), ws.numel(), _stream())
    _prof_end(ev, "grad_sumsq", 0.0, 4 * plan.elements)
    return out


def adamw_segments(p, g, m, v, plan, lr, beta1, beta2, eps, step, gscale=1.0, sumsq=None, max_norm=0.0):
    ev = _prof_begin()
    call("vitssl_adamw_segments", _flat(p, "p", plan), _flat(g, "g", plan), _flat(m, "m", plan), _flat(v, "v", plan),
         _chk(plan.table, torch.uint8, "table"), plan.nseg, float(lr), float(beta1), float(beta2), float(eps), int(step), float(gscale),
         _opt(sumsq, F32, "sumsq", (1,)), float(max_norm), _stream())
    _prof_end(ev, "adamw_segments", 0.0, 28 * plan.elements)


def lamb_segments(p, g, m, v, plan, lr, beta1, beta2, eps, step, gscale=1.0, sumsq=None, max_norm=0.0, always_adapt=False,
                  trust_clip=False, trust=None, workspace=None):
    ws0, trust0 = (None, None) if (trust is not None and workspace is not None) else plan.lamb_buffers()
    trust = trust0 if trust is None else trust
    ws = ws0 if workspace is None else workspace
    flags = (L.LAMB_ALWAYS_ADAPT if always_adapt else 0) | (L.LAMB_TRUST_CLIP if trust_clip else 0)
    ev = _prof_begin()
    call("vitssl_lamb_segments", _flat(p, "p", plan), _flat(g, "g", plan), _flat(m, "m", plan), _flat(v, "v", plan),
         _chk(plan.table, torch.uint8, "table"), plan.nseg, float(lr), float(beta1), float(beta2), float(eps), int(step), float(gscale),
         _opt(sumsq, F32, "sumsq", (1,)), float(max_norm), flags, _chk(trust, F32, "trust", (plan.nseg,)),
         _chk(ws, torch.uint8, "workspace"), ws.numel(), _stream())
    _prof_end(ev, "lamb_segments", 0.0, 40 * plan.elements)
    return trust


def ema(teacher, student, m):
    ev = _prof_begin()
    call("vitssl_ema", _chk(teacher, F32, "teacher"), _chk(student, F32, "student", teacher.shape), teacher.numel(), float(m), _stream())
    _prof_end(ev, "ema", 0.0, 12 * teacher.numel())


def rownorm_fwd(z, zn, inv_norm):
    rows, cols = z.shape
    call("vitssl_rownorm_fwd", _chk(z, F32, "z"), _chk(zn, BF16, "zn", (rows, cols)), _chk(inv_norm, F32, "inv_norm", (rows,)), rows, cols, _stream())


def rownorm_bwd(dzn, zn, inv_norm, dz):
    rows, cols = dzn.shape
    call("vitssl_rownorm_bwd", _chk(dzn, F32, "dzn"), _chk(zn, BF16, "zn", (rows, cols)), _chk(inv_norm, F32, "inv_norm", (rows,)),
         _chk(dz, BF16, "dz", (rows, cols)), rows, cols, _stream())


def weightnorm_fold(g, v, w_f32, inv_vnorm):
    K, D = v.shape
    call("vitssl_weightnorm_fold", _chk(g, F32, "g"), _chk(v, F32, "v"), _chk(w_f32, F32, "w", (K, D)), _chk(inv_vnorm, F32, "inv_vnorm", (K,)),
         K, D, _stream())


def weightnorm_bwd(dw, g, v, inv_vnorm, dg, dv):
    K, D = v.shape
    call("vitssl_weightnorm_bwd", _chk(dw, F32, "dw", (K, D)), _chk(g, F32, "g"), _chk(v, F32, "v"), _chk(inv_vnorm, F32, "inv_vnorm", (K,)),
         _chk(dg, F32, "dg"), _chk(dv, F32, "dv", (K, D)), K, D, _stream())


def dino_tws_floats(G, B, K):
    return int(L.lib().vitssl_dino_loss_workspace_floats(G, B, K))


def dino_loss(teacher, student, center, t_ws, loss_sum, dstudent, G, V, B, K, teacher_temp, student_temp, gscale=1.0):
    ev = _prof_begin()
    _dino_loss(teacher, student, center, t_ws, loss_sum, dstudent, G, V, B, K, teacher_temp, student_temp, gscale)
    _prof_end(ev, "dino_loss", 0.0, B * K * (4 * (G + V) + 8 + (2 * V if dstudent is not None else 0)))


def _dino_loss(teacher, student, center, t_ws, loss_sum, dstudent, G, V, B, K, teacher_temp, student_temp, gscale=1.0):
    call("vitssl_dino_loss", _chk(teacher, F32, "teacher", (G * B, K)), _chk(student, F32, "student", (V * B, K)),
         _chk(center, F32, "center"), _chk(t_ws, F32, "t_ws"), t_ws.numel(), _chk(loss_sum, F32, "loss_sum", (1,)),
         _opt(dstudent, BF16, "dstudent", (V * B, K)), G, V, B, K, float(teacher_temp), float(student_temp), float(gscale), _stream())


def colsum_f32(x, out):
    rows, cols = x.shape
    ev = _prof_begin()
    call("vitssl_colsum_f32", _chk(x, F32, "x"), _chk(out, F32, "out", (cols,)), rows, cols, _stream())
    _prof_end(ev, "center_colsum", 0.0, 4 * rows * cols)


def center_ema(center, colsum, momentum, inv_rows):
    K = colsum.numel()
    call("vitssl_center_ema", _chk(center, F32, "center"), _chk(colsum, F32, "colsum"), K, float(momentum), float(inv_rows), _stream())


def bicubic_resize_fwd(src, dst, gh0, gw0, gh, gw):
    D = src.shape[1]
    call("vitssl_bicubic_resize_fwd", _chk(src, F32, "src", (gh0 * gw0, D)), _chk(dst, F32, "dst", (gh * gw, D)),
         gh0, gw0, gh, gw, D, _stream())


def bicubic_resize_bwd(ddst, dsrc, gh0, gw0, gh, gw):
    D = ddst.shape[1]
    call("vitssl_bicubic_resize_bwd", _chk(ddst, F32, "ddst", (gh * gw, D)), _chk(dsrc, F32, "dsrc", (gh0 * gw0, D)),
         gh0, gw0, gh, gw, D, _stream())


AUG_IP, AUG_FP = 11, 10


def aug_resized_crop_u8(src, iparams, tmp, dst):
    B, H, W, Cc = src.shape
    S = dst.shape[1]
    if Cc != 3:
        raise L.VitsslError(f"aug_resized_crop: expected channel-last RGB [B,H,W,3], got {tuple(src.shape)}")
    call("vitssl_aug_resized_crop_u8", _chk(src, torch.uint8, "src"), _chk(iparams, torch.int32, "iparams", (B, AUG_IP)),
         _chk(tmp, torch.uint8, "tmp", (B, H, S, 3)), _chk(dst, torch.uint8, "dst", (B, S, S, 3)), B, H, W, S, _stream())


def aug_color_u8(img, iparams, fparams):
    B, S = img.shape[0], img.shape[1]
    call("vitssl_aug_color_u8", _chk(img, torch.uint8, "img", (B, S, S, 3)), _chk(iparams, torch.int32, "iparams", (B, AUG_IP)),
         _chk(fparams, F32, "fparams", (B, AUG_FP)), B, S, _stream())


def aug_blur_to_tensor(img, fparams, out, ksize=7):
    B, S = img.shape[0], img.shape[1]
    call("vitssl_aug_blur_to_tensor", _chk(img, torch.uint8, "img", (B, S, S, 3)), _chk(fparams, F32, "fparams", (B, AUG_FP)),
         _chk(out, F32, "out", (B, 3, S, S)), B, S, ksize, _stream())


TF_IP = 5


def tf_tile_rows(H, W, SH, SW):
    l = L.lib()
    tr = l.vitssl_debug_tf_tile_rows(int(H), int(W), int(SH), int(SW))
    if tr <= 0:
        raise L.VitsslError(f"vitssl_debug_tf_tile_rows failed ({tr}): {l.vitssl_last_error().decode()}")
    return tr


def tf_resized_crop_to_tensor(src, iparams, out):
    if src is None or src.dim() != 4 or src.shape[3] != 3:
        raise L.VitsslError(f"tf_resized_crop_to_tensor: expected channel-last RGB [B,H,W,3], got {None if src is None else tuple(src.shape)}")
    if out is None or out.dim() != 4:
        raise L.VitsslError(f"tf_resized_crop_to_tensor: expected out [B,3,SH,SW], got {None if out is None else tuple(out.shape)}")
    B, H, W, _ = src.shape
    SH, SW = out.shape[2], out.shape[3]
    call("vitssl_tf_resized_crop_to_tensor", _chk(src, torch.uint8, "src"), _chk(iparams, torch.int32, "iparams", (B, TF_IP)),
         _chk(out, F32, "out", (B, 3, SH, SW)), B, H, W, SH, SW, _stream())


F64 = torch.float64


def _vp(t):
    return C.c_void_p(t.data_ptr())


RECON_ACC = 4
DINO_STATS = 8


def recon_metrics(pred, target, acc, C, P):
    if pred is None or pred.dim() != 2 or pred.shape[1] != C * P * P:
        raise L.VitsslError(f"recon_metrics: expected pred [n, {C}*{P}*{P}], got {None if pred is None else tuple(pred.shape)}")
    n = pred.shape[0]
    a, b, c = _chk(pred, F32, "pred"), _chk(target, F32, "target", (n, C * P * P)), _chk(acc, F64, "acc", (RECON_ACC,))
    ws = _tn_workspace(pred.device, int(L.lib().vitssl_recon_metrics_workspace_floats(n, C, P)))
    call("vitssl_recon_metrics", a, b, c, n, C, P, _vp(ws), ws.numel(), _stream())


def dino_stats(teacher, student, center, out):
    if teacher is None or teacher.dim() != 3 or student is None or student.dim() != 3:
        raise L.VitsslError("dino_stats: expected teacher [G,B,K] and student [V,B,K], got "
                            f"{None if teacher is None else tuple(teacher.shape)} and {None if student is None else tuple(student.shape)}")
    G, B, K = teacher.shape
    V = student.shape[0]
    t, s = _chk(teacher, F32, "teacher"), _chk(student, F32, "student", (V, B, K))
    c, o = _opt(center, F32, "center", (K,)), _chk(out, F64, "out", (DINO_STATS,))
    ws = _tn_workspace(teacher.device, int(L.lib().vitssl_dino_stats_workspace_floats(G, V, B, K)))
    call("vitssl_dino_stats", t, s, c, o, G, V, B, K, _vp(ws), ws.numel(), _stream())


I64, I32 = torch.int64, torch.int32


def _classify(who, entry, sizing, between, logits, labels, C, loss_out, pred, counters, bad_labels, dlogits, dbias, label_smoothing,
              ignore_index, upstream, workspace, scalars=(), nullable=False):
    if logits is None or logits.dim() != 2 or not 2 <= int(C) <= logits.shape[1]:
        raise L.VitsslError(f"{who}: expected logits [B, ld] with 2 <= C = {C} <= ld, got {None if logits is None else tuple(logits.shape)}")
    B, ld = logits.shape
    ld_out = 0
    if dlogits is not None:
        if dlogits.dim() != 2 or dlogits.shape[0] != B or dlogits.shape[1] % 64 != 0 or dlogits.shape[1] < C:
            raise L.VitsslError(f"{who}: dlogits must be [{B}, ld_out] with ld_out % 64 == 0 and ld_out >= {C}, got {tuple(dlogits.shape)}")
        ld_out = dlogits.shape[1]
    z, y = _chk(logits, F32, "logits"), _chk(labels, I64, "labels", (B,))
    extra = [(_opt if nullable else _chk)(t, dtype, name, (B,)) for t, dtype, name in between]
    lo, pr = _chk(loss_out, F32, "loss_out", (2,)), _chk(pred, I64, "pred", (B,))
    ct, bl = _chk(counters, I64, "counters", (2,)), _chk(bad_labels, I32, "bad_labels", (1,))
    dl, db = _opt(dlogits, BF16, "dlogits"), _opt(dbias, F32, "dbias", (C,))
    need = int(getattr(L.lib(), sizing)(B, C))
    ws = _tn_workspace(logits.device, need) if workspace is None else workspace
    if workspace is not None:
        _chk(ws, F32, "workspace")
    call(entry, z, y, *extra, B, int(C), ld, float(label_smoothing), *scalars, int(ignore_index), float(upstream), lo, dl, ld_out, db,
         pr, ct, bl, _vp(ws), ws.numel(), _stream())


def classify_loss(logits, labels, C, loss_out, pred, counters, bad_labels, dlogits=None, dbias=None, label_smoothing=0.0,
                  ignore_index=-100, upstream=1.0, workspace=None):
    _classify("classify_loss", "vitssl_classify_loss", "vitssl_classify_loss_workspace_floats", (), logits, labels, C, loss_out, pred,
              counters, bad_labels, dlogits, dbias, label_smoothing, ignore_index, upstream, workspace)


MIX_IP = 6
MIX_COPY, MIX_BLEND, MIX_PASTE = 0, 1, 2


def mix_batch(x, out, iparams, lam):
    if x is None or x.dim() != 4:
        raise L.VitsslError(f"mix_batch: expected x [B,C,H,W], got {None if x is None else tuple(x.shape)}")
    B, Cn, H, W = x.shape
    call("vitssl_mix_batch", _chk(x, F32, "x"), _chk(out, F32, "out", (B, Cn, H, W)), _chk(iparams, I32, "iparams", (B, MIX_IP)),
         _chk(lam, F32, "lam", (B,)), B, Cn, H, W, _stream())


def classify_loss_mix(logits, labels, partner, lam, C, loss_out, pred, counters, bad_labels, dlogits=None, dbias=None,
                      label_smoothing=0.0, ignore_index=-100, upstream=1.0, workspace=None):
    _classify("classify_loss_mix", "vitssl_classify_loss_mix", "vitssl_classify_loss_mix_workspace_floats",
              ((partner, I32, "partner"), (lam, F32, "lam")), logits, labels, C, loss_out, pred, counters, bad_labels, dlogits, dbias,
              label_smoothing, ignore_index, upstream, workspace)


def classify_bce(logits, labels, C, loss_out, pred, counters, bad_labels, partner=None, lam=None, dlogits=None, dbias=None,
                 smoothing=0.0, target_threshold=None, sum_classes=False, ignore_index=-100, upstream=1.0, workspace=None):
    if (partner is None) != (lam is None):
        raise L.VitsslError("classify_bce: partner and lam are either both None (one label per row) or both given")
    thr = -1.0 if target_threshold is None else float(target_threshold)
    if not thr >= 0.0 and target_threshold is not None:
        raise L.VitsslError(f"classify_bce: target_threshold = {target_threshold!r} must be None or a number >= 0")
    _classify("classify_bce", "vitssl_classify_bce", "vitssl_classify_bce_workspace_floats",
              ((partner, I32, "partner"), (lam, F32, "lam")), logits, labels, C, loss_out, pred, counters, bad_labels, dlogits, dbias,
              smoothing, ignore_index, upstream, workspace, scalars=(thr, int(bool(sum_classes))), nullable=True)


def _mae_shape(who, B, N, K, D):
    B, N, K, D = int(B), int(N), int(K), int(D)
    if B <= 0 or N <= 0 or D <= 0 or D % 4 != 0:
        raise L.VitsslError(f"{who}: B={B}, N={N} must be positive and the width {D} a positive multiple of 4")
    if not 1 <= K <= N - 1:
        raise L.VitsslError(f"{who}: K={K} kept patches outside [1, N-1] with N={N}")
    return B, N, K, D


def mae_tokens_fwd(xk, keep, pos, cls, out, B, N, K):
    B, N, K, D = _mae_shape("mae_tokens_fwd", B, N, K, xk.shape[-1])
    call("vitssl_mae_tokens_fwd", _chk(xk, F32, "xk", (B * K, D)), _chk(keep, I32, "keep", (B, K)), _chk(pos, F32, "pos", (N + 1, D)),
         _chk(cls, F32, "cls", (D,)), _chk(out, F32, "out", (B * (K + 1), D)), B, N, K, D, _stream())


def mae_tokens_bwd(g, dproj, dbias, dcls, B, N, K):
    B, N, K, D = _mae_shape("mae_tokens_bwd", B, N, K, g.shape[-1])
    call("vitssl_mae_tokens_bwd", _chk(g, F32, "g", (B * (K + 1), D)), _chk(dproj, BF16, "dproj", (B * K, D)), _chk(dbias, F32, "dbias", (D,)),
         _chk(dcls, F32, "dcls", (D,)), B, N, K, D, *_sum_ws(g.device, B * (K + 1), D), _stream())


def mae_unshuffle_fwd(y, restore, mask_token, dpos, out, B, N, K):
    B, N, K, D = _mae_shape("mae_unshuffle_fwd", B, N, K, y.shape[-1])
    call("vitssl_mae_unshuffle_fwd", _chk(y, F32, "y", (B * (K + 1), D)), _chk(restore, I32, "restore", (B, N)),
         _chk(mask_token, F32, "mask_token", (D,)), _chk(dpos, F32, "dpos", (N + 1, D)), _chk(out, F32, "out", (B * (N + 1), D)),
         B, N, K, D, _stream())


def mae_unshuffle_bwd(g, restore, dy, dbias, dmask_token, B, N, K):
    B, N, K, D = _mae_shape("mae_unshuffle_bwd", B, N, K, g.shape[-1])
    call("vitssl_mae_unshuffle_bwd", _chk(g, F32, "g", (B * (N + 1), D)), _chk(restore, I32, "restore", (B, N)),
         _chk(dy, BF16, "dy", (B * (K + 1), D)), _chk(dbias, F32, "dbias", (D,)), _chk(dmask_token, F32, "dmask_token", (D,)),
         B, N, K, D, *_sum_ws(g.device, B * (N + 1), D), _stream())


def mae_loss(pred, target, loss_sum, dpred=None, gscale=0.0, norm_pix=True):
    if pred is None or pred.dim() != 2:
        raise L.VitsslError(f"mae_loss: pred must be a matrix, got {None if pred is None else tuple(pred.shape)}")
    rows, cols = pred.shape
    pp, ld = _chk_ld(pred, F32, "pred", rows, cols)
    Pdp = 0
    if dpred is not None:
        if dpred.dim() != 2 or dpred.shape[0] != rows or dpred.shape[1] < cols or dpred.shape[1] % 4 != 0:
            raise L.VitsslError(f"mae_loss: dpred must be [{rows}, Pdp >= {cols}] with Pdp % 4 == 0, got {tuple(dpred.shape)}")
        Pdp = dpred.shape[1]
    if norm_pix and cols < 2:
        raise L.VitsslError("mae_loss: norm_pix needs at least two columns (the unbiased variance of one value is undefined)")
    call("vitssl_mae_loss", pp, ld, _chk(target, F32, "target", (rows, cols)), _chk(loss_sum, F32, "loss_sum", (1,)),
         _opt(dpred, BF16, "dpred"), rows, cols, Pdp, int(bool(norm_pix)), float(gscale), *_sum_ws(pred.device, rows, cols), _stream())


def _mae_rows(entry, dtype, per, src, idx, out, scatter):
    if src is None or src.dim() != 2 or out is None or out.dim() != 2 or src.shape[1] != out.shape[1] or out.shape[1] % per != 0:
        raise L.VitsslError(f"{entry}: src / out must be matrices of one width that is a multiple of {per}, got "
                            f"{None if src is None else tuple(src.shape)} / {None if out is None else tuple(out.shape)}")
    rows, cols = out.shape
    if rows == 0 or (scatter and src.shape[0] == 0):
        raise L.VitsslError(f"{entry}: empty operand")
    call("vitssl_" + entry, _chk(src, dtype, "src"), _chk(idx, I32, "inv" if scatter else "idx", (rows,)), _chk(out, dtype, "out"),
         rows, cols, _stream())


def mae_gather_rows_bf16(src, idx, out):
    _mae_rows("mae_gather_rows_bf16", BF16, 8, src, idx, out, False)


def mae_gather_rows_f32(src, idx, out):
    _mae_rows("mae_gather_rows_f32", F32, 4, src, idx, out, False)


def mae_scatter_rows_f32(src, inv, g):
    _mae_rows("mae_scatter_rows_f32", F32, 4, src, inv, g, True)
```

Measured before the change: 7709 images/s.

## Store GELU pre-activation u in tile-ordered layout for wide stores and loads

```diff
diff --git a/__graft_entry__.py b/__graft_entry__.py
--- a/__graft_entry__.py
+++ b/__graft_entry__.py
@@ -31,7 +31,7 @@
             os.path.join(ROOT, "include", "vitssl_optim.h"), os.path.join(ROOT, "include", "vitssl_mixup.h"),
             os.path.join(ROOT, "include", "vitssl_droppath.h"), os.path.join(ROOT, "include", "vitssl_layerscale.h"),
             os.path.join(ROOT, "include", "vitssl_lamb.h"), os.path.join(ROOT, "include", "vitssl_bce.h"),
-            os.path.join(ROOT, "include_ext", "vitssl_mae.h")]
+            os.path.join(ROOT, "include_ext", "vitssl_mae.h"), os.path.join(ROOT, "include_nt", "vitssl_gprime.h")]
     objdir = os.path.join(CSRC, "build")
     os.makedirs(objdir, exist_ok=True)
 
diff --git a/include_nt/vitssl_gprime.h b/include_nt/vitssl_gprime.h
--- /dev/null
+++ b/include_nt/vitssl_gprime.h
@@ -0,0 +1,21 @@
+#ifndef VITSSL_GPRIME_H
+#define VITSSL_GPRIME_H
+
+#include <stdint.h>
+
+#include "../include/vitssl_hip.h"
+
+#ifdef __cplusplus
+extern "C" {
+#endif
+
+int64_t vitssl_gprime_bytes(int64_t M, int N);
+
+int vitssl_gprime_tile_order(int64_t M, int N);
+
+int vitssl_gemm_bf16_nt_gprime(const vitssl_gemm_t* g, void* stream);
+
+#ifdef __cplusplus
+}
+#endif
+#endif
diff --git a/vit-ssl_amd/csrc/gemm_nt.hip b/vit-ssl_amd/csrc/gemm_nt.hip
--- a/vit-ssl_amd/csrc/gemm_nt.hip
+++ b/vit-ssl_amd/csrc/gemm_nt.hip
@@ -1,3 +1,4 @@
+#include "../../include_nt/vitssl_gprime.h"
 #include "nt_epilogue.h"
 
 namespace {
@@ -15,6 +16,11 @@
   static constexpr int LDS_BYTES = 2 * BUF_BYTES;
   static constexpr int MIN_WAVES_PER_SIMD = 2;
   static constexpr int WG_PER_CU = (WAVES == 8) ? 1 : 2;
+  static constexpr bool GT = false;
+};
+template <typename CFG>
+struct NtTileOrdered : CFG {
+  static constexpr bool GT = true;
 };
 using NtBig = NtCfg<64, 2, 4>;
 using NtSmall = NtCfg<32, 2, 2>;
@@ -402,7 +408,7 @@
   wait_vmcnt<8>();
   raw_barrier();
 
-  constexpr int S = nt_epi_vmem_ops<EPI, MI, F8>();
+  constexpr int S = nt_epi_vmem_ops<EPI, MI, F8, CFG::GT>();
   constexpr int NW = 8;
   constexpr int NW_POST = (NW + S) > 63 ? 63 : (NW + S);
   int buf = 0;
@@ -508,7 +514,16 @@
     }
   }
   if constexpr (CFG::WAVES == 8 && CFG::BK == 64 && EPI != EPI_F32_SPLITK) {
-    if (p.k_chunk == 0 && (p.N & 7) == 0) return launch_pp<EPI, CFG>(p, s);
+    if (p.k_chunk == 0 && (p.N & 7) == 0) {
+      if constexpr (EPI == VITSSL_EPI_GELU || EPI == VITSSL_EPI_DGELU) {
+        if (p.gt) return launch_pp<EPI, NtTileOrdered<CFG>>(p, s);
+      }
+      return launch_pp<EPI, CFG>(p, s);
+    }
+  }
+  if (p.gt) {
+    vitssl_set_error("gemm_nt_gprime: the tile-ordered g' exists in the ping-pong loop only (VITSSL_NT_TILE=2 forces the other one)");
+    return VITSSL_ERR_ARG;
   }
   static VsEnvInt persist_env;
   const int knob = persist_env.get("VITSSL_NT_PERSIST", -1);
@@ -577,7 +592,7 @@
   if (mode == 3) return launch_cfg<EPI, NtBig192>(p, s);
   if (mode == 4) return launch_cfg<EPI, NtBig224>(p, s);
   const long long big_tiles = ceil_div64(p.M, 256) * ceil_div64(p.N, 256);
-  if (big_tiles < 64 && p.esz == 2) return launch_cfg<EPI, NtSmall>(p, s);
+  if (big_tiles < 64 && p.esz == 2) return p.gt ? launch_cfg<EPI, NtBig>(p, s) : launch_cfg<EPI, NtSmall>(p, s);
   const long long slots = cu_count();
   const long long tn = ceil_div64(p.N, 256);
   const double c256 = (double)ceil_div64(ceil_div64(p.M, 256) * tn, slots);
@@ -607,9 +622,14 @@
   return VITSSL_OK;
 }
 
+static int gprime_knob() {
+  static VsEnvInt knob;
+  return knob.get("VITSSL_GPRIME_MATRIX", 0);
+}
+
 static int gemm_nt_entry(const vitssl_gemm_t* g, int esz, const vitssl_fp8_gemm_t* q, void* stream, const vitssl_rowscale_t* rows = nullptr,
-                         const vitssl_colscale_t* cols = nullptr, void* branch = nullptr) {
-  const char* who = cols ? "gemm_nt_ls" : rows ? "gemm_nt_rows" : esz == 1 ? "gemm_fp8_nt" : "gemm_nt";
+                         const vitssl_colscale_t* cols = nullptr, void* branch = nullptr, bool gprime = false) {
+  const char* who = gprime ? "gemm_nt_gprime" : cols ? "gemm_nt_ls" : rows ? "gemm_nt_rows" : esz == 1 ? "gemm_fp8_nt" : "gemm_nt";
   VS_CHECK_ARG(g && g->A && g->B && (g->out0 || (esz == 1 && caller_epi(g->epilogue).q8_of == 0 && q && q->out_fp8)), "%s: null operand", who);
   VS_CHECK_ARG(g->M > 0 && g->N > 0 && g->K > 0, "%s: empty problem M=%lld N=%d K=%d", who, (long long)g->M, g->N, g->K);
   VS_CHECK_ARG(g->K % (128 / esz) == 0, "%s: K=%d must be a multiple of %d", who, g->K, 128 / esz);
@@ -630,6 +650,13 @@
     p.qamax = q->out_amax;
   }
   p.rows_per_group = 1;
+  if (gprime) {
+    VS_CHECK_ARG(g->epilogue == VITSSL_EPI_GELU || g->epilogue == VITSSL_EPI_DGELU,
+                 "%s: the tile-ordered g' belongs to VITSSL_EPI_GELU (out0) / VITSSL_EPI_DGELU (aux), got epilogue %d", who, g->epilogue);
+    VS_CHECK_ARG(g->N % 64 == 0, "%s: N=%d must be a multiple of 64 (one block of the image is 16 rows x 64 columns)", who, g->N);
+    VS_CHECK_ARG(nt_tile_override() != 2, "%s: VITSSL_NT_TILE=2 forces the two-phase loop, which has no tile-ordered g'", who);
+    p.gt = gprime_knob() > 0 ? 0 : 1;
+  }
 #ifdef VITSSL_NT_STAMPS
   p.stamps = g_nt_stamps;
 #endif
@@ -691,6 +718,18 @@
   return gemm_nt_entry(g, 2, nullptr, stream, rows, cols, branch_bf16);
 }
 
+extern "C" int64_t vitssl_gprime_bytes(int64_t M, int N) { return M > 0 && N > 0 ? ((M + 15) / 16 * 16) * (int64_t)N * 2 : 0; }
+
+extern "C" int vitssl_gprime_tile_order(int64_t M, int N) {
+  if (M <= 0 || N <= 0 || N % 64 != 0 || gprime_knob() > 0 || nt_tile_override() == 2) return 0;
+  if (gprime_knob() < 0) return 1;
+  return ceil_div64(M, 256) * ceil_div64(N, 256) >= 64;
+}
+
+extern "C" int vitssl_gemm_bf16_nt_gprime(const vitssl_gemm_t* g, void* stream) {
+  return gemm_nt_entry(g, 2, nullptr, stream, nullptr, nullptr, nullptr, true);
+}
+
 extern "C" int vitssl_gemm_fp8_nt(const vitssl_gemm_t* g, const vitssl_fp8_gemm_t* q, void* stream) {
   VS_CHECK_ARG(g && caller_epi(g->epilogue).fp8, "gemm_fp8_nt: fp8 operands are built for the BF16 / F32 / GELU / RESID / DGELU epilogues");
   VS_CHECK_ARG(!(q && q->out_fp8) || caller_epi(g->epilogue).q8_of >= 0, "gemm_fp8_nt: out_fp8 belongs to EPI_GELU / EPI_DGELU");
diff --git a/vit-ssl_amd/csrc/nt_epilogue.h b/vit-ssl_amd/csrc/nt_epilogue.h
--- a/vit-ssl_amd/csrc/nt_epilogue.h
+++ b/vit-ssl_amd/csrc/nt_epilogue.h
@@ -32,6 +32,7 @@
   float* qamax;
   const float* rowscale;
   unsigned rows_per_group;
+  int gt;
   const float* colscale;
 #ifdef VITSSL_NT_STAMPS
   unsigned long long* stamps;
@@ -74,16 +75,19 @@
   return nt_epi(EPI).resid ? (PREF ? 1 : (MI % 2 == 0 ? 2 : 1)) : EPI == VITSSL_EPI_DGELU ? (PREF ? 2 : (MI % 4 == 0 ? 4 : 2)) : 4;
 }
 
-template <int EPI, bool F8>
+constexpr int NT_GT_ROW_OPS = 2;
+template <int EPI, bool F8, bool GT = false>
 constexpr int nt_epi_row_ops(bool stores_only) {
   constexpr NtEpiFacts E = nt_epi(EPI);
+  static_assert(!GT || (!F8 && (EPI == VITSSL_EPI_GELU || EPI == VITSSL_EPI_DGELU)), "the tile-ordered g' belongs to GELU / dGELU with bf16 operands");
   if (!E.windowed) return 0;
-  const int out0 = (F8 && E.q8_of == 0) ? 1 : E.out0_esz;
+  const int out0 = (GT && EPI == VITSSL_EPI_GELU) ? NT_GT_ROW_OPS : (F8 && E.q8_of == 0) ? 1 : E.out0_esz;
   const int out1 = E.out1 != OUT1_REQUIRED ? 0 : (F8 && E.q8_of == 1) ? 1 : 2;
-  return (stores_only ? 0 : E.aux_esz) + out0 + out1;
-}
-template <int EPI, int MI, bool F8>
-constexpr int nt_epi_vmem_ops() { return nt_epi_row_ops<EPI, F8>(false) * MI; }
+  const int aux = (GT && EPI == VITSSL_EPI_DGELU) ? NT_GT_ROW_OPS : E.aux_esz;
+  return (stores_only ? 0 : aux) + out0 + out1;
+}
+template <int EPI, int MI, bool F8, bool GT = false>
+constexpr int nt_epi_vmem_ops() { return nt_epi_row_ops<EPI, F8, GT>(false) * MI; }
 template <int EPI>
 constexpr int nt_epi_tail_stores() { return nt_epi_row_ops<EPI, false>(true) * nt_row_group<EPI, 8, false>(); }
 template <int EPI, int MI>
@@ -98,6 +102,10 @@
          nt_counts_are<EPI_RESID_LS, MI>(8, 8, 8) && nt_counts_are<VITSSL_EPI_EMBED, MI>(0, 0, 0) && nt_counts_are<EPI_F32_SPLITK, MI>(0, 0, 0);
 }
 static_assert(nt_counts_are_as_written<6>() && nt_counts_are_as_written<7>() && nt_counts_are_as_written<8>(), "epilogue vmem counts");
+static_assert(nt_epi_vmem_ops<VITSSL_EPI_GELU, 8, false, true>() == 4 * 8 && nt_epi_vmem_ops<VITSSL_EPI_DGELU, 8, false, true>() == 4 * 8 &&
+                  nt_epi_vmem_ops<VITSSL_EPI_GELU, 7, false, true>() == nt_epi_vmem_ops<VITSSL_EPI_GELU, 7, false>() &&
+                  nt_epi_vmem_ops<VITSSL_EPI_DGELU, 6, false, true>() == nt_epi_vmem_ops<VITSSL_EPI_DGELU, 6, false>(),
+              "epilogue vmem counts, tile-ordered g'");
 
 
 constexpr int GLUT_E_LO = 127 - 14;
@@ -168,6 +176,9 @@
   constexpr int MI = CFG::MI;
   constexpr NtEpiFacts E = nt_epi(EPI);
   constexpr bool LS = EPI == EPI_RESID_LS;
+  constexpr bool GT = CFG::GT;
+  constexpr bool GT_OUT0 = GT && EPI == VITSSL_EPI_GELU, GT_AUX = GT && EPI == VITSSL_EPI_DGELU;
+  static_assert(!GT || (TLS && !Q8 && (GT_OUT0 || GT_AUX)), "the tile-ordered g': ping-pong kernel, bf16 operands, GELU / dGELU");
   int lane = lane_in;
   if (TLS) asm volatile("" : "+v"(lane));
   constexpr bool GLUT = EPI == VITSSL_EPI_GELU && GLUT_OFF >= 0;
@@ -189,6 +200,17 @@
     const unsigned rec = bytes > 0x80000000ull ? 0x80000000u : (unsigned)bytes;
     return __builtin_amdgcn_make_buffer_rsrc((void*)((const char*)base + m0 * p.N * elt), 0, (int)rec, 0x00020000);
   };
+  auto window_gt = [&](const void* base) {
+    const unsigned long long bytes = (unsigned long long)(((p.M + 15) & ~15ll) - m0) * (unsigned long long)p.N * 2ull;
+    const unsigned rec = bytes > 0x80000000ull ? 0x80000000u : (unsigned)bytes;
+    return __builtin_amdgcn_make_buffer_rsrc((void*)((const char*)base + m0 * p.N * 2), 0, (int)rec, 0x00020000);
+  };
+  unsigned gt_b = 0u;
+  if constexpr (GT) {
+    const int gt_n = n0 + wn * 64;
+    gt_b = gt_n < p.N ? (unsigned)(wm * MI) * ((unsigned)p.N * 32u) + (unsigned)(gt_n >> 6) * 2048u + (unsigned)lane * 16u : OOB;
+  }
+  auto off_gt = [&](int i) -> unsigned { return gt_b + (unsigned)i * ((unsigned)p.N * 32u); };
   const unsigned row_l = (unsigned)(wm * CFG::WROWS + (lane & 15));
   const unsigned un = (unsigned)p.N;
   const int odd = g4 & 1;
@@ -284,11 +306,11 @@
   if (q8) rsOut2 = window(p.out2, 1);
   const float qs = (Q8EPI && p.qscale) ? *p.qscale : 1.0f;
   float qmax = 0.f;
-  if constexpr (E.windowed) rsOut0 = window(p.out0, E.out0_esz);
+  if constexpr (E.windowed) rsOut0 = GT_OUT0 ? window_gt(p.out0) : window(p.out0, E.out0_esz);
   if constexpr (E.out1 != OUT1_NONE) {
     if (E.out1 == OUT1_REQUIRED || p.out1) rsOut1 = window(p.out1, 2);
   }
-  if constexpr (E.aux_esz != 0) rsAux = window(p.aux, E.aux_esz);
+  if constexpr (E.aux_esz != 0) rsAux = GT_AUX ? window_gt(p.aux) : window(p.aux, E.aux_esz);
 
   f32x4 bias4[2][2];
   f32x4 gam4[2][2];
@@ -354,7 +376,10 @@
 #pragma unroll
         for (int ii = 0; ii < RG; ++ii) {
           if (ii >= cnt) continue;
-          if (tls) {
+          if constexpr (GT_AUX) {
+#pragma unroll
+            for (int jp = 0; jp < 2; ++jp) raw[b][ii][jp] = __builtin_amdgcn_raw_buffer_load_b128(rsAux, off_gt(ig + ii), 1024 * jp, 0);
+          } else if (tls) {
             raw[b][ii][0] = __builtin_amdgcn_raw_buffer_load_b128(rsAux, off_line16(ig + ii, 0), 0, 0);
             raw[b][ii][1] = __builtin_amdgcn_raw_buffer_load_b128(rsAux, off_line16(ig + ii, 1), 0, 0);
           } else {
@@ -380,6 +405,11 @@
 #pragma unroll
           for (int jp = 0; jp < 2; ++jp) {
             if (ii >= cnt) continue;
+            if constexpr (GT_AUX) {
+              gpre[ii][jp][0] = u32x2{raw[gb][ii][jp][0], raw[gb][ii][jp][1]};
+              gpre[ii][jp][1] = u32x2{raw[gb][ii][jp][2], raw[gb][ii][jp][3]};
+              continue;
+            }
             if (tls) {
               if (jp == 0) {
                 win.put_lines_bf16(raw[gb][ii][0], raw[gb][ii][1]);
@@ -566,7 +596,11 @@
         }
       }
       if constexpr (E.windowed && E.out0_esz == 2) {
-        if (!(Q8 && E.q8_of == 0) || p.out0) store_bf16_row(rsOut0, i, out_a, IC<EPI == VITSSL_EPI_GELU ? 2 : 0>{});
+        if constexpr (GT_OUT0) {
+#pragma unroll
+          for (int jp = 0; jp < 2; ++jp)
+            __builtin_amdgcn_raw_buffer_store_b128(u32x4{out_a[jp][0][0], out_a[jp][0][1], out_a[jp][1][0], out_a[jp][1][1]}, rsOut0, off_gt(i), 1024 * jp, 2);
+        } else if (!(Q8 && E.q8_of == 0) || p.out0) store_bf16_row(rsOut0, i, out_a, IC<EPI == VITSSL_EPI_GELU ? 2 : 0>{});
       }
       if constexpr (E.out1 == OUT1_REQUIRED) {
         if (!(Q8 && E.q8_of == 1) || p.out1) store_bf16_row(rsOut1, i, out_b, IC<0>{});
diff --git a/vit-ssl_amd/vitssl_hip/_lib.py b/vit-ssl_amd/vitssl_hip/_lib.py
--- a/vit-ssl_amd/vitssl_hip/_lib.py
+++ b/vit-ssl_amd/vitssl_hip/_lib.py
@@ -10,6 +10,8 @@
                        "lamb", "bce")}
 _INCLUDE_EXT = os.path.normpath(os.path.join(_HERE, "..", "..", "include_ext"))
 EXT_HEADERS = {"mae": os.path.join(_INCLUDE_EXT, "vitssl_mae.h")}
+_INCLUDE_NT = os.path.normpath(os.path.join(_HERE, "..", "..", "include_nt"))
+NT_HEADERS = {"gprime": os.path.join(_INCLUDE_NT, "vitssl_gprime.h")}
 
 
 class VitsslError(RuntimeError):
@@ -225,6 +227,15 @@
 }
 EXT_REGISTRY = {key: {name: p if isinstance(p, tuple) else (C.c_int, p) for name, p in table.items()} for key, table in _EXT_ABI.items()}
 
+_NT_ABI = {
+    "gprime": {
+        "vitssl_gprime_bytes": _returns(_i64, _i64, _i),
+        "vitssl_gprime_tile_order": _returns(_i, _i64, _i),
+        "vitssl_gemm_bf16_nt_gprime": [_pGemm, _vp],
+    },
+}
+NT_REGISTRY = {key: {name: p if isinstance(p, tuple) else (C.c_int, p) for name, p in table.items()} for key, table in _NT_ABI.items()}
+
 DROPPATH_SITE_BIT = 0x80000000
 DROPPATH_MAX_SITES = 128
 LAMB_ALWAYS_ADAPT, LAMB_TRUST_CLIP = 1, 2
@@ -233,7 +244,7 @@
 
 
 def header_path(key):
-    return HEADERS[key] if key in HEADERS else EXT_HEADERS[key]
+    return HEADERS[key] if key in HEADERS else EXT_HEADERS[key] if key in EXT_HEADERS else NT_HEADERS[key]
 
 
 def header_text(key):
@@ -269,7 +280,7 @@
     if l.vitssl_version() != ABI_VERSION:
         raise VitsslError(f"{LIB_PATH} implements C-ABI version {l.vitssl_version()}, these bindings expect {ABI_VERSION}: "
                           "rebuild it (python __graft_entry__.py)")
-    for table in list(REGISTRY.values()) + list(EXT_REGISTRY.values()):
+    for table in list(REGISTRY.values()) + list(EXT_REGISTRY.values()) + list(NT_REGISTRY.values()):
         for name, (restype, argtypes) in table.items():
             fn = getattr(l, name)
             fn.restype, fn.argtypes = restype, argtypes
diff --git a/vit-ssl_amd/vitssl_hip/engine.py b/vit-ssl_amd/vitssl_hip/engine.py
--- a/vit-ssl_amd/vitssl_hip/engine.py
+++ b/vit-ssl_amd/vitssl_hip/engine.py
@@ -688,7 +688,8 @@
         dev = x.device
         g = self.ws.get
         probs = None
-        rec = {"B": B, "T": T, "seed": seed, "training": training, "blocks": []}
+        gt = not self.fp8 and dev.type == "cuda" and bool(L.lib().vitssl_gprime_tile_order(M, F))
+        rec = {"B": B, "T": T, "seed": seed, "training": training, "blocks": [], "gprime_tiles": gt}
         dp = None
         if training and self.drop_path is not None:
             dp = ops.droppath_table(self.drop_path_sites(), B, seed, g(f"{slot}.dp" if save else f"{slot}.tmp.dp", (2 * self.L, B), F32, dev))
@@ -707,7 +708,7 @@
             qkv = g(tag + "qkv", (M, 3 * D), BF16, dev)
             lse = g(tag + "lse", (B, H, T), F32, dev)
             xmid = g(tag + "xmid", (M, D), F32, dev)
-            u = g(tag + "u", (M, F), BF16, dev)
+            u = g(tag + "u", ((M + 15) // 16 * 16 if gt else M, F), BF16, dev)
             xout = g(f"{slot}.{i}.xout" if save else f"{slot}.tmp.xout{i & 1}", (M, D), F32, dev)
 
             if return_attn and i == self.L - 1:
@@ -718,7 +719,7 @@
             self._attn_fwd(qkv, att, att_op, lse, B, T, probs if i == self.L - 1 else None)
             self._gemm(att_op, i, "wo", xmid, L.EPI_RESID, aux=cur, drop=self._drop(i, 0, seed, training), **self._scaled(dp, T, i, 1, branch=ls1))
             self._ln_fwd(xmid, i, "layer_norm2", h2, mean2, rstd2)
-            self._gemm(h2, i, "w1", u, L.EPI_GELU, bias=b1, image=a, drop=self._drop(i, 1, seed, training))
+            self._gemm(h2, i, "w1", u, L.EPI_GELU, bias=b1, image=a, drop=self._drop(i, 1, seed, training), **({"gprime_tiles": True} if gt else {}))
             self._gemm(a, i, "w2", xout, L.EPI_RESID, bias=b2, aux=xmid, drop=self._drop(i, 2, seed, training), **self._scaled(dp, T, i, 2, branch=ls2))
             if save:
                 rec["blocks"].append(dict(xin=cur, h1=h1, mean1=mean1, rstd1=rstd1, qkv=qkv, att=att, att_op=att_op, lse=lse, xmid=xmid,
@@ -733,6 +734,7 @@
         st, D, H, F = self.store, self.D, self.H, self.F
         rec = self._saved[slot]
         B, T, seed, training, dp = rec["B"], rec["T"], rec["seed"], rec["training"], rec.get("dp")
+        gprime = {"gprime_tiles": True} if rec["gprime_tiles"] else {}
         M = B * T
         dev = g.device
         w = self.ws.get
@@ -765,7 +767,7 @@
             a_ = self.bp[i] + "self_attention."
             du, gm2, dqkv = grad(i, 1), grad(i, 2), grad(i, 3)
             self._dgrad(gm, i, "w2", du.x, L.EPI_DGELU, emits=du, aux=s["u"],
-                        colsum=gv(self._n(i, "feed_forward.linear_in.bias")))
+                        colsum=gv(self._n(i, "feed_forward.linear_in.bias")), **gprime)
             self._dgrad(du, i, "w1", dh_)
             self._ln_bwd((dh_, s["xmid"], s["mean2"], s["rstd2"], i, "layer_norm2"), g, gm2, None, self._drop(i, 0, seed, training),
                          **scaled(i, 1))
diff --git a/vit-ssl_amd/vitssl_hip/ops.py b/vit-ssl_amd/vitssl_hip/ops.py
--- a/vit-ssl_amd/vitssl_hip/ops.py
+++ b/vit-ssl_amd/vitssl_hip/ops.py
@@ -186,7 +186,15 @@
 _OUT0_DTYPE = {L.EPI_BF16: BF16, L.EPI_F32: F32, L.EPI_GELU: BF16, L.EPI_RESID: F32, L.EPI_DGELU: BF16, L.EPI_EMBED: F32}
 
 
-def _nt_desc(who, sfx, dtype, A, B, epilogue, bias, set_out0, aux, dgelu_aux, out1, colsum, drop, epilogues=None):
+def gprime_rows(M):
+    return (M + 15) // 16 * 16
+
+
+def gprime_tile_order(M, N):
+    return bool(L.lib().vitssl_gprime_tile_order(M, N))
+
+
+def _nt_desc(who, sfx, dtype, A, B, epilogue, bias, set_out0, aux, dgelu_aux, out1, colsum, drop, epilogues=None, gprime_tiles=False):
     M, K = A.shape
     N, K2 = B.shape
     if K != K2:
@@ -203,7 +211,7 @@
     if epilogue == L.EPI_RESID:
         g.aux = _chk(aux, F32, "aux(residual)", (M, N))
     elif epilogue == L.EPI_DGELU:
-        g.aux = _chk(aux, BF16, dgelu_aux, (M, N))
+        g.aux = _chk(aux, BF16, dgelu_aux, (gprime_rows(M) if gprime_tiles else M, N))
     g.out1 = _opt(out1, BF16, "out1", (M, N))
     g.colsum = _opt(colsum, F32, "colsum", (N,))
     if colsum is not None:
@@ -213,10 +221,13 @@
 
 
 def gemm_nt(A, B, out0, epilogue, bias=None, aux=None, out1=None, colsum=None, drop=NO_DROP, embed=None, rows=None, cols=None,
-            branch=None):
+            branch=None, gprime_tiles=False):
+    if gprime_tiles and epilogue not in (L.EPI_GELU, L.EPI_DGELU):
+        raise L.VitsslError(f"gemm_nt: gprime_tiles= belongs to EPI_GELU / EPI_DGELU, got epilogue {epilogue}")
+
     def set_out0(g, M, N):
         if epilogue != L.EPI_EMBED:
-            g.out0 = _chk(out0, _OUT0_DTYPE[epilogue], "out0", (M, N))
+            g.out0 = _chk(out0, _OUT0_DTYPE[epilogue], "out0", (gprime_rows(M) if gprime_tiles and epilogue == L.EPI_GELU else M, N))
             return
         if embed is None:
             raise L.VitsslError("gemm_nt: EPI_EMBED needs embed=(mask, mask_token, pos, tokens, out_tokens, tok_offset)")
@@ -231,9 +242,13 @@
         g.embed = e
         g.out0 = _chk(out0, F32, "out0", ((M // tokens) * out_tokens, N))
 
-    g, M, N, K = _nt_desc("gemm_nt", "", BF16, A, B, epilogue, bias, set_out0, aux, "aux(u)", out1, colsum, drop)
-    ev = _prof_begin()
-    if cols is not None:
+    g, M, N, K = _nt_desc("gemm_nt", "", BF16, A, B, epilogue, bias, set_out0, aux, "aux(u)", out1, colsum, drop, gprime_tiles=gprime_tiles)
+    ev = _prof_begin()
+    if gprime_tiles:
+        if cols is not None or rows is not None or branch is not None:
+            raise L.VitsslError("gemm_nt: gprime_tiles= does not combine with rows= / cols= / branch= (EPI_RESID forms)")
+        call("vitssl_gemm_bf16_nt_gprime", C.byref(g), _stream())
+    elif cols is not None:
         if epilogue != L.EPI_RESID:
             raise L.VitsslError(f"gemm_nt: cols= belongs to EPI_RESID, got epilogue {epilogue}")
         call("vitssl_gemm_bf16_nt_ls", C.byref(g), C.byref(_colscale(cols, N, "gemm_nt")),
@@ -250,7 +265,10 @@
 
 
 def gemm_fp8_nt(A8, B8, out0, epilogue, alpha=None, bias=None, aux=None, out1=None, out_fp8=None, drop=NO_DROP,
-                alpha2=None, colsum=None, out_scale=None, out_amax=None):
+                alpha2=None, colsum=None, out_scale=None, out_amax=None, gprime_tiles=False):
+    if gprime_tiles:
+        raise L.VitsslError("gemm_fp8_nt: the tile-ordered g' (gprime_tiles=) exists with bf16 operands only")
+
     def set_out0(g, M, N):
         if out0 is None and not (epilogue == L.EPI_DGELU and out_fp8 is not None):
             raise L.VitsslError("gemm_fp8_nt: out0 may only be omitted for EPI_DGELU with out_fp8")
```

Measured after the change: 7742 images/s (median of 6 runs). No clear change (+0.4%).
